# Koukyosyumei/MyZKP

Hardware: AMD Instinct MI355X
Metric: G1 MSM pairs/sec + NTT elems/sec at 2^20 and 2^24; bit-exact vs CPU (higher is better)
Workload: dtype u32x9 (29-bit limbs, 254-bit Montgomery); 1 GPU; KZG commit = BN254 G1 Pippenger MSM of 2^20 (scalar, point) pairs per GPU against a device-resident SRS (commit_kzg, kzg.rs:57-59); 17-bit signed windows (library default at this size), 15 window tables built once at upload; N GPUs = one MSM of N*2^20 pairs (BASELINE configs[2]/[3]); pairs_per_gpu=1048576, seed=332211571536, window_bits=17

## Files before the change

myzkp_amd/csrc/mzk_api.hip:

```cpp
#include <stdarg.h>
#include <stdlib.h>
#include <atomic>
#include "mzk_common.h"
#include "mzk_gl.h"

namespace mzk {

static thread_local char g_err[512] = "";
void set_error(const char* fmt, ...) {
  va_list ap;
  va_start(ap, fmt);
  vsnprintf(g_err, sizeof g_err, fmt, ap);
  va_end(ap);
}
void clear_error() { g_err[0] = 0; }
int hip_fail(hipError_t e, const char* what, const char* file, int line) {
  set_error("HIP error %d (%s) in %s at %s:%d", (int)e, hipGetErrorString(e), what, file, line);
  return MZK_E_HIP;
}

static std::atomic<uint64_t> g_owner{0};
static thread_local int t_depth = 0;
static thread_local char t_marker;
static uint64_t g_call_epoch = 1;
static size_t g_ws_budget = 0;
EntryGuard::EntryGuard() : ok(true), nested(false) {
  if (t_depth > 0) { t_depth++; nested = true; return; }
  uint64_t expected = 0;
  if (!g_owner.compare_exchange_strong(expected, (uint64_t)(uintptr_t)&t_marker, std::memory_order_acquire)) {
    ok = false;
    set_error("another host thread is inside the library: calls must come from one thread at a time (MZK_E_BUSY)");
    return;
  }
  t_depth = 1;
  g_call_epoch++;
}
EntryGuard::~EntryGuard() {
  if (!ok) return;
  if (--t_depth == 0) g_owner.store(0, std::memory_order_release);
}

static Context g_ctxs[MZK_MAX_CTX];
static int g_nctx = 0, g_cur = 0;
static int g_last_ordinal = 0;
static signed char g_peer[MZK_MAX_CTX][MZK_MAX_CTX];
int ctx_peer_enabled(int a, int b) { return (a >= 0 && b >= 0 && a < g_nctx && b < g_nctx) ? g_peer[a][b] : 0; }
static uint64_t g_gen_counter = 1;
Context& ctx() { return g_ctxs[g_cur]; }
int ctx_count() { return g_nctx; }
static std::atomic<int> g_ctx0_current_on{-1};
static void publish_ctx0() {
  g_ctx0_current_on.store((g_nctx > 0 && g_cur == 0 && g_ctxs[0].ready) ? g_ctxs[0].device : -1, std::memory_order_release);
}
int ctx_select(int index) {
  if (index < 0 || index >= g_nctx || !g_ctxs[index].ready) { set_error("context %d does not exist (%d initialised)", index, g_nctx); return MZK_E_ARG; }
  MZK_HIP(hipSetDevice(g_ctxs[index].device));
  g_cur = index;
  publish_ctx0();
  return MZK_OK;
}
CtxScope::CtxScope(int index) : prev_ctx(g_cur), prev_dev(-1), ok(false) {
  if (hipGetDevice(&prev_dev) != hipSuccess) prev_dev = -1;
  ok = ctx_select(index) == MZK_OK;
}
CtxScope::~CtxScope() {
  g_cur = prev_ctx;
  publish_ctx0();
  if (prev_dev >= 0) (void)hipSetDevice(prev_dev);
}

size_t ws_bytes_held() {
  size_t t = poly_bytes_held();
  for (const auto& b : ctx().ws) t += b.cap;
  return t;
}
size_t ws_trim_idle() {
  Context& c = ctx();
  const size_t poly_idle = poly_trim_idle();
  size_t idle = 0;
  for (const auto& b : c.ws) if (b.p && b.epoch != g_call_epoch) idle += b.cap;
  if (!idle) return poly_idle;
  (void)hipDeviceSynchronize();
  bool table_slot_freed = false;
  for (int k = 0; k < WS_COUNT; k++) {
    WsBuf& b = c.ws[k];
    if (b.p && b.epoch != g_call_epoch) {
      (void)hipFree(b.p);
      b.p = nullptr; b.cap = 0;
      table_slot_freed = table_slot_freed || k == WS_FB_TABLE16 || k == WS_FB_TABLE8 || k == WS_NTT_PRE || k == WS_NTT_PRE_M128;
    }
  }
  if (table_slot_freed) c.ws_gen = ++g_gen_counter;
  return idle + poly_idle;
}
int dev_alloc(void** out, size_t bytes, const char* what) {
  *out = nullptr;
  hipError_t e = hipMalloc(out, bytes);
  if (e == hipErrorOutOfMemory || e == hipErrorMemoryAllocation) {
    (void)hipGetLastError();
    if (ws_trim_idle()) e = hipMalloc(out, bytes);
  }
  if (e == hipSuccess) return MZK_OK;
  (void)hipGetLastError();
  *out = nullptr;
  if (e == hipErrorOutOfMemory || e == hipErrorMemoryAllocation) {
    set_error("%s: the device has no %zu bytes left (idle workspace already released)", what, bytes);
    return MZK_E_NOMEM;
  }
  return hip_fail(e, what, __FILE__, __LINE__);
}
int ws_get(WsSlot slot, size_t bytes, void** out) {
  WsBuf& b = ctx().ws[slot];
  b.epoch = g_call_epoch;
  if (bytes > b.cap) {
    if (b.p) {
      MZK_HIP(hipDeviceSynchronize());
      MZK_HIP(hipFree(b.p));
      b.p = nullptr; b.cap = 0;
    }
    size_t cap = bytes < 4096 ? 4096 : bytes;
    if (g_ws_budget && ws_bytes_held() + cap > g_ws_budget) (void)ws_trim_idle();
    MZK_TRY(dev_alloc(&b.p, cap, "workspace"));
    b.cap = cap;
  }
  *out = b.p;
  return MZK_OK;
}
uint64_t ws_generation() { return ctx().ws_gen; }
int d2h_sync(void* host, const void* dev, size_t bytes, hipStream_t s) {
  if (bytes == 0 || bytes > SMALL_D2H_MAX) {
    if (bytes) MZK_HIP(hipMemcpyAsync(host, dev, bytes, hipMemcpyDeviceToHost, s));
    MZK_HIP(hipStreamSynchronize(s));
    return MZK_OK;
  }
  Context& c = ctx();
  if (!c.bounce) MZK_HIP(hipHostMalloc(&c.bounce, SMALL_D2H_MAX, hipHostMallocPortable));
  MZK_HIP(hipMemcpyAsync(c.bounce, dev, bytes, hipMemcpyDeviceToHost, s));
  MZK_HIP(hipStreamSynchronize(s));
  memcpy(host, c.bounce, bytes);
  return MZK_OK;
}
void ws_release_all() {
  Context& c = ctx();
  c.ws_gen = ++g_gen_counter;
  for (auto& b : c.ws) {
    if (b.p) (void)hipFree(b.p);
    b.p = nullptr; b.cap = 0;
  }
}
WsGuard::WsGuard(hipStream_t s_) : s(s_) {
  Context& c = ctx();
  if (!c.ready) return;
  if (c.ws_used && c.ws_last != s) {
    if (!c.ws_event && hipEventCreateWithFlags(&c.ws_event, hipEventDisableTiming) != hipSuccess) c.ws_event = nullptr;
    if (c.ws_event && hipEventRecord(c.ws_event, c.ws_last) == hipSuccess) (void)hipStreamWaitEvent(s, c.ws_event, 0);
    else { (void)hipGetLastError(); (void)hipDeviceSynchronize(); }
  }
}
WsGuard::~WsGuard() {
  Context& c = ctx();
  if (!c.ready) return;
  c.ws_last = s;
  c.ws_used = true;
}

static bool g_prof_on = false;
static uint32_t g_prof_mask = 0xffffffffu;
struct ProfPair { hipEvent_t a, b; int phase; };
static std::vector<ProfPair> g_prof_pending;
static std::vector<hipEvent_t> g_prof_pool;
static hipEvent_t g_prof_open[MZK_PH_COUNT];
static double g_prof_ms[MZK_PH_COUNT];
static uint64_t g_prof_cnt[MZK_PH_COUNT];
static hipEvent_t prof_event() {
  if (!g_prof_pool.empty()) { hipEvent_t e = g_prof_pool.back(); g_prof_pool.pop_back(); return e; }
  hipEvent_t e = nullptr;
  (void)hipEventCreate(&e);
  return e;
}
void prof_begin(hipStream_t s, int phase) {
  if (!g_prof_on || !((g_prof_mask >> phase) & 1u) || ctx().index != 0) return;
  hipEvent_t e = prof_event();
  (void)hipEventRecord(e, s);
  g_prof_open[phase] = e;
}
void prof_end(hipStream_t s, int phase) {
  if (!g_prof_on || !g_prof_open[phase] || ctx().index != 0) return;
  hipEvent_t e = prof_event();
  (void)hipEventRecord(e, s);
  g_prof_pending.push_back({g_prof_open[phase], e, phase});
  g_prof_open[phase] = nullptr;
}
static void prof_drain() {
  (void)hipDeviceSynchronize();
  for (auto& pr : g_prof_pending) {
    float ms = 0.f;
    if (hipEventElapsedTime(&ms, pr.a, pr.b) == hipSuccess) { g_prof_ms[pr.phase] += ms; g_prof_cnt[pr.phase]++; }
    g_prof_pool.push_back(pr.a);
    g_prof_pool.push_back(pr.b);
  }
  g_prof_pending.clear();
}

int ensure_init() {
  if (g_nctx > 0 && ctx().ready) {
    int cur = -1;
    if (hipGetDevice(&cur) != hipSuccess || cur != ctx().device) MZK_HIP(hipSetDevice(ctx().device));
    return MZK_OK;
  }
  return mzk_init(g_last_ordinal);
}

static const HostField HF_FR = {4, {0x43e1f593f0000001ULL, 0x2833e84879b97091ULL, 0xb85045b68181585dULL, 0x30644e72e131a029ULL}, 29 * FrParams::L};
static const HostField HF_FQ = {4, {0x3c208c16d87cfd47ULL, 0x97816a916871ca8dULL, 0xb85045b68181585dULL, 0x30644e72e131a029ULL}, 29 * FqParams::L};
static const HostField HF_M128 = {2, {1ULL, 407ULL << 55, 0, 0}, 29 * M128Params::L};
const HostField* host_field(int fid) {
  switch (fid) {
    case MZK_FIELD_FR: return &HF_FR;
    case MZK_FIELD_M128: return &HF_M128;
    case MZK_FIELD_FQ: return &HF_FQ;
    default: return nullptr;
  }
}
int field_check(int fid, const char* who, bool fq_too) {
  if (fid == MZK_FIELD_FR || fid == MZK_FIELD_M128 || (fq_too && fid == MZK_FIELD_FQ)) return MZK_OK;
  set_error("%s: bad field id %d", who, fid);
  return MZK_E_ARG;
}
int field_check_ntt(int fid, const char* who) {
  if (fid == MZK_FIELD_FR || fid == MZK_FIELD_M128) return MZK_OK;
  set_error("%s: field id %d has no NTT on this path", who, fid);
  return MZK_E_ARG;
}
static int h_cmp(const uint64_t* a, const uint64_t* b, int n) {
  for (int i = n - 1; i >= 0; i--) if (a[i] != b[i]) return a[i] > b[i] ? 1 : -1;
  return 0;
}
bool h_is_canonical(const HostField* f, const uint64_t* a) { return h_cmp(a, f->p, f->nl) < 0; }
bool h_is_one(const HostField* f, const uint64_t* a) {
  if (a[0] != 1) return false;
  for (int i = 1; i < f->nl; i++) if (a[i]) return false;
  return true;
}
static void h_addmod(const HostField* f, uint64_t* r, const uint64_t* a, const uint64_t* b) {
  uint64_t t[4] = {0, 0, 0, 0};
  unsigned __int128 c = 0;
  for (int i = 0; i < f->nl; i++) { c += (unsigned __int128)a[i] + b[i]; t[i] = (uint64_t)c; c >>= 64; }
  if (c || h_cmp(t, f->p, f->nl) >= 0) {
    unsigned __int128 br = 0;
    for (int i = 0; i < f->nl; i++) {
      unsigned __int128 d = (unsigned __int128)t[i] - f->p[i] - (uint64_t)br;
      t[i] = (uint64_t)d; br = (d >> 64) & 1;
    }
  }
  for (int i = 0; i < f->nl; i++) r[i] = t[i];
}
static void h_mulmod_slow(const HostField* f, uint64_t* r, const uint64_t* a, const uint64_t* b) {
  uint64_t acc[4] = {0, 0, 0, 0}, aa[4] = {0, 0, 0, 0}, bb[4] = {0, 0, 0, 0};
  for (int i = 0; i < f->nl; i++) { aa[i] = a[i]; bb[i] = b[i]; }
  for (int bit = 64 * f->nl - 1; bit >= 0; bit--) {
    h_addmod(f, acc, acc, acc);
    if ((bb[bit / 64] >> (bit % 64)) & 1) h_addmod(f, acc, acc, aa);
  }
  for (int i = 0; i < f->nl; i++) r[i] = acc[i];
}
struct HostMont { bool ready; uint64_t n0; uint64_t r2[4]; };
static HostMont g_hmont[3];
static const HostMont* host_mont(const HostField* f) {
  HostMont* m = &g_hmont[f == &HF_FR ? 0 : (f == &HF_FQ ? 1 : 2)];
  if (!m->ready) {
    uint64_t inv = f->p[0];
    for (int i = 0; i < 6; i++) inv *= 2 - f->p[0] * inv;
    m->n0 = (uint64_t)0 - inv;
    uint64_t x[4] = {1, 0, 0, 0};
    for (int i = 0; i < 128 * f->nl; i++) h_addmod(f, x, x, x);
    for (int i = 0; i < 4; i++) m->r2[i] = x[i];
    m->ready = true;
  }
  return m;
}
static void h_montmul(const HostField* f, const HostMont* m, uint64_t* r, const uint64_t* a, const uint64_t* b) {
  const int n = f->nl;
  uint64_t t[6] = {0, 0, 0, 0, 0, 0};
  for (int i = 0; i < n; i++) {
    unsigned __int128 c = 0;
    for (int j = 0; j < n; j++) { c += (unsigned __int128)a[j] * b[i] + t[j]; t[j] = (uint64_t)c; c >>= 64; }
    c += t[n]; t[n] = (uint64_t)c; t[n + 1] = (uint64_t)(c >> 64);
    const uint64_t q = t[0] * m->n0;
    c = (unsigned __int128)q * f->p[0] + t[0];
    c >>= 64;
    for (int j = 1; j < n; j++) { c += (unsigned __int128)q * f->p[j] + t[j]; t[j - 1] = (uint64_t)c; c >>= 64; }
    c += t[n]; t[n - 1] = (uint64_t)c;
    t[n] = t[n + 1] + (uint64_t)(c >> 64);
  }
  if (t[n] || h_cmp(t, f->p, n) >= 0) {
    unsigned __int128 br = 0;
    for (int i = 0; i < n; i++) { unsigned __int128 d = (unsigned __int128)t[i] - f->p[i] - (uint64_t)br; t[i] = (uint64_t)d; br = (d >> 64) & 1; }
  }
  for (int i = 0; i < n; i++) r[i] = t[i];
}
void h_mulmod(const HostField* f, uint64_t* r, const uint64_t* a, const uint64_t* b) {
  const HostMont* m = host_mont(f);
  uint64_t t[4] = {0, 0, 0, 0};
  h_montmul(f, m, t, a, b);
  h_montmul(f, m, r, t, m->r2);
}
void h_powmod_u64(const HostField* f, uint64_t* r, const uint64_t* a, uint64_t e) {
  uint64_t res[4] = {1, 0, 0, 0}, base[4] = {0, 0, 0, 0};
  for (int i = 0; i < f->nl; i++) base[i] = a[i];
  while (e) {
    if (e & 1) h_mulmod(f, res, res, base);
    h_mulmod(f, base, base, base);
    e >>= 1;
  }
  for (int i = 0; i < f->nl; i++) r[i] = res[i];
}
void h_invmod(const HostField* f, uint64_t* r, const uint64_t* a) {
  uint64_t e[4] = {0, 0, 0, 0}, res[4] = {1, 0, 0, 0}, base[4] = {0, 0, 0, 0};
  for (int i = 0; i < f->nl; i++) { e[i] = f->p[i]; base[i] = a[i]; }
  {
    uint64_t borrow = 2;
    for (int i = 0; i < f->nl && borrow; i++) {
      const uint64_t old = e[i];
      e[i] = old - borrow;
      borrow = (old < borrow) ? 1 : 0;
    }
  }
  for (int bit = 0; bit < 64 * f->nl; bit++) {
    if ((e[bit / 64] >> (bit % 64)) & 1) h_mulmod(f, res, res, base);
    h_mulmod(f, base, base, base);
  }
  for (int i = 0; i < f->nl; i++) r[i] = res[i];
}
void h_ninv_pow2(const HostField* f, unsigned k, uint64_t* out) {
  uint64_t q[4] = {0, 0, 0, 0};
  for (int i = 0; i < f->nl; i++) q[i] = f->p[i];
  q[0] -= 1;
  for (unsigned s = 0; s < k; s++) {
    for (int i = 0; i < f->nl; i++) q[i] = (q[i] >> 1) | ((i + 1 < f->nl) ? (q[i + 1] << 63) : 0);
  }
  unsigned __int128 br = 0;
  for (int i = 0; i < f->nl; i++) {
    unsigned __int128 d = (unsigned __int128)f->p[i] - q[i] - (uint64_t)br;
    out[i] = (uint64_t)d; br = (d >> 64) & 1;
  }
}
void h_rmod(const HostField* f, uint64_t* out) {
  const uint64_t two[4] = {2, 0, 0, 0};
  h_powmod_u64(f, out, two, (uint64_t)f->mont_bits);
}

}

using namespace mzk;

extern "C" {

int mzk_abi_version(void) { return 2; }
const char* mzk_last_error(void) { return g_err; }

static int check_device(int device_ordinal, int* num_cu) {
  int count = 0;
  hipError_t e = hipGetDeviceCount(&count);
  if (e != hipSuccess || count <= 0) {
    set_error("no HIP device visible (hipGetDeviceCount: %s); this library has no CPU fallback",
              e == hipSuccess ? "0 devices" : hipGetErrorString(e));
    return MZK_E_NOGPU;
  }
  if (device_ordinal < 0 || device_ordinal >= count) { set_error("mzk_init: device %d out of range (%d visible)", device_ordinal, count); return MZK_E_ARG; }
  hipDeviceProp_t prop;
  MZK_HIP(hipGetDeviceProperties(&prop, device_ordinal));
  if (strncmp(prop.gcnArchName, "gfx950", 6) != 0) {
    set_error("device %d is %s; this library is built for gfx950 (MI355X) only", device_ordinal, prop.gcnArchName);
    return MZK_E_NOGPU;
  }
  *num_cu = prop.multiProcessorCount;
  return MZK_OK;
}

int mzk_init_devices(const int* device_ordinals, int n_devices) {
  mzk::EntryGuard entry;
  if (!entry.ok) return MZK_E_BUSY;
  if (!device_ordinals || n_devices < 1 || n_devices > MZK_MAX_CTX) { set_error("mzk_init_devices: need 1..%d device ordinals", MZK_MAX_CTX); return MZK_E_ARG; }
  bool same = g_nctx == n_devices;
  for (int i = 0; same && i < n_devices; i++) same = g_ctxs[i].ready && g_ctxs[i].device == device_ordinals[i];
  if (same) return ctx_select(0);
  int ncu[MZK_MAX_CTX];
  for (int i = 0; i < n_devices; i++) MZK_TRY(check_device(device_ordinals[i], &ncu[i]));
  if (g_nctx) mzk_shutdown();
  for (int i = 0; i < n_devices; i++) {
    Context& c = g_ctxs[i];
    c = Context();
    c.index = i;
    c.device = device_ordinals[i];
    c.num_cu = ncu[i];
    c.ws_gen = ++g_gen_counter;
    MZK_HIP(hipSetDevice(c.device));
    int dup = 0;
    for (int j = 0; j < i; j++) dup += g_ctxs[j].device == c.device;
    int prio_least = 0, prio_greatest = 0;
    (void)hipDeviceGetStreamPriorityRange(&prio_least, &prio_greatest);
    int prio = prio_least - dup;
    if (prio < prio_greatest) prio = prio_greatest;
    if (dup == 0) MZK_HIP(hipStreamCreateWithFlags(&c.stream, hipStreamNonBlocking));
    else MZK_HIP(hipStreamCreateWithPriority(&c.stream, hipStreamNonBlocking, prio));
    c.ready = true;
    g_nctx = i + 1;
  }
  g_last_ordinal = device_ordinals[0];
  for (int a = 0; a < n_devices; a++)
    for (int b = 0; b < n_devices; b++) {
      g_peer[a][b] = 1;
      const int da = g_ctxs[a].device, db = g_ctxs[b].device;
      if (da == db) continue;
      int can = 0;
      if (hipDeviceCanAccessPeer(&can, da, db) != hipSuccess) { (void)hipGetLastError(); can = 0; }
      if (can) {
        MZK_HIP(hipSetDevice(da));
        hipError_t e = hipDeviceEnablePeerAccess(db, 0);
        if (e == hipErrorPeerAccessAlreadyEnabled) (void)hipGetLastError();
        else if (e != hipSuccess) { (void)hipGetLastError(); can = 0; }
      }
      g_peer[a][b] = (signed char)can;
    }
  return ctx_select(0);
}
int mzk_init(int device_ordinal) {
  if (g_ctx0_current_on.load(std::memory_order_acquire) == device_ordinal) {
    int dev = -1;
    if (hipGetDevice(&dev) == hipSuccess && (dev == device_ordinal || hipSetDevice(device_ordinal) == hipSuccess)) return MZK_OK;
    (void)hipGetLastError();
  }
  mzk::EntryGuard entry;
  if (!entry.ok) return MZK_E_BUSY;
  if (g_nctx > 0 && g_ctxs[0].ready && g_ctxs[0].device == device_ordinal) return entry.nested ? MZK_OK : ctx_select(0);
  return mzk_init_devices(&device_ordinal, 1);
}
int mzk_ctx_count(void) { return g_nctx; }
int mzk_ctx_select(int index) {
  mzk::EntryGuard entry;
  if (!entry.ok) return MZK_E_BUSY;
  return ctx_select(index);
}
int mzk_ctx_peer_enabled(int a, int b) { return ctx_peer_enabled(a, b); }
int mzk_ctx_device(int index) { return (index >= 0 && index < g_nctx) ? g_ctxs[index].device : -1; }
void* mzk_ctx_stream(int index) { return (index >= 0 && index < g_nctx) ? (void*)g_ctxs[index].stream : nullptr; }

// ... 1141 lines not shown
```

myzkp_amd/csrc/mzk_common.h:

```cpp
#pragma once
#include <hip/hip_runtime.h>
#include <stdint.h>
#include <stddef.h>
#include <stdio.h>
#include <string.h>
#include <functional>
#include <string>
#include <vector>
#include "../../include/mzk.h"
#include "mzk_field.h"
#include "mzk_msm_plan.h"

namespace mzk {

#ifdef MZK_TUNING
#include <stdlib.h>
static inline int tune_int(const char* name, int dflt) { const char* v = getenv(name); return v ? atoi(v) : dflt; } static inline const char* tune_str(const char* name) { return getenv(name); }
#else
static inline constexpr int tune_int(const char*, int dflt) { return dflt; }
static inline constexpr const char* tune_str(const char*) { return nullptr; }
#endif

void set_error(const char* fmt, ...);
void clear_error();
size_t table_budget_bytes();
int hip_fail(hipError_t e, const char* what, const char* file, int line);
#define MZK_HIP(x)                                                        \
  do {                                                                    \
    hipError_t _e = (x);                                                  \
    if (_e != hipSuccess) return mzk::hip_fail(_e, #x, __FILE__, __LINE__); \
  } while (0)
#define MZK_TRY(x)        \
  do {                    \
    int _rc = (x);        \
    if (_rc != MZK_OK) return _rc; \
  } while (0)

constexpr int MZK_MAX_CTX = 16;
struct WsBuf { void* p = nullptr; size_t cap = 0; uint64_t epoch = 0; };
enum WsSlot { WS_NTT_TMP = 0, WS_NTT_IO_A, WS_NTT_IO_B, WS_MSM_POINTS, WS_MSM_SCALARS, WS_MSM_COUNTS, WS_MSM_OFFSETS,
              WS_MSM_CURSOR, WS_MSM_ENTRIES, WS_MSM_BUCKETS, WS_MSM_RED_A, WS_MSM_RED_B, WS_MSM_SCAN, WS_MSM_OUT, WS_MSM_SLOTS, WS_MSM_WGHIST, WS_BATCHINV, WS_XYZZ_TMP, WS_MERKLE_NODES, WS_FB_TABLE16, WS_FB_TABLE8, WS_NTT_PRE, WS_NTT_PRE_M128,
              WS_MISC_A, WS_MISC_B, WS_MISC_C, WS_MISC_D, WS_MISC_E, WS_MISC_F, WS_COUNT };
enum AttrFlag { ATTR_FINE_SCATTER4 = 0, ATTR_FINE_SCATTER8, ATTR_DIGITS_LDS, ATTR_SMALL_MSM, ATTR_NTT_LARGE_FR, ATTR_NTT_LARGE_M128, ATTR_NTT_LARGE_M128_2WG, ATTR_MANY_SORT1, ATTR_TAIL_ROW, ATTR_COARSE_STAGED4, ATTR_COARSE_STAGED8, ATTR_COUNT };
struct Context {
  bool ready = false;
  int index = 0;
  int device = -1;
  int num_cu = 256;
  hipStream_t stream = nullptr;
  WsBuf ws[WS_COUNT];
  uint64_t ws_gen = 1;
  hipEvent_t ws_event = nullptr;
  hipEvent_t fork_event = nullptr, join_event = nullptr;
  hipStream_t ws_last = nullptr;
  bool ws_used = false;
  bool attr_done[ATTR_COUNT] = {};
  hipStream_t xstream[MZK_MAX_CTX] = {};
  hipEvent_t xdone[MZK_MAX_CTX] = {};
  hipEvent_t xready = nullptr;
  void* bounce = nullptr;
};
constexpr size_t SMALL_D2H_MAX = 4096;
int d2h_sync(void* host, const void* dev, size_t bytes, hipStream_t s);
int ctx_peer_enabled(int a, int b);
struct EntryGuard {
  bool ok;
  bool nested;
  EntryGuard();
  ~EntryGuard();
};
#define MZK_ENTER()                        \
  mzk::EntryGuard _mzk_entry;              \
  if (!_mzk_entry.ok) return MZK_E_BUSY;   \
  MZK_TRY(mzk::ensure_init())
Context& ctx();
int ctx_count();
int ctx_select(int index);
int ensure_init();
struct CtxScope {
  int prev_ctx, prev_dev; bool ok;
  explicit CtxScope(int index);
  ~CtxScope();
};

int ws_get(WsSlot slot, size_t bytes, void** out);
void ws_release_all();
size_t ws_trim_idle();
size_t ws_bytes_held();
int dev_alloc(void** out, size_t bytes, const char* what);
size_t poly_bytes_held();
size_t poly_trim_idle();
uint64_t ws_generation();
struct WsGuard {
  hipStream_t s;
  explicit WsGuard(hipStream_t s_);
  ~WsGuard();
};

void prof_begin(hipStream_t s, int phase);
void prof_end(hipStream_t s, int phase);
struct ProfScope {
  hipStream_t s; int ph;
  ProfScope(hipStream_t s_, int ph_) : s(s_), ph(ph_) { prof_begin(s, ph); }
  ~ProfScope() { prof_end(s, ph); }
};

struct HostField {
  int nl;
  uint64_t p[4];
  int mont_bits;
};
const HostField* host_field(int fid);
bool h_is_canonical(const HostField* f, const uint64_t* a);
void h_mulmod(const HostField* f, uint64_t* r, const uint64_t* a, const uint64_t* b);
void h_powmod_u64(const HostField* f, uint64_t* r, const uint64_t* a, uint64_t e);
void h_invmod(const HostField* f, uint64_t* r, const uint64_t* a);
void h_ninv_pow2(const HostField* f, unsigned log2n, uint64_t* out);
bool h_is_one(const HostField* f, const uint64_t* a);
void h_rmod(const HostField* f, uint64_t* out);

static inline bool field_is_gl(int fid) { return fid == MZK_FIELD_M64 || fid == MZK_FIELD_M64X3; }
static inline int field_gl_comps(int fid) { return fid == MZK_FIELD_M64X3 ? 3 : 1; }
static inline int field_words(int fid) { return field_is_gl(fid) ? 2 * field_gl_comps(fid) : (fid == MZK_FIELD_M128 ? 4 : 8); }
static inline int field_limbs64(int fid) { return field_is_gl(fid) ? field_gl_comps(fid) : (fid == MZK_FIELD_M128 ? 2 : 4); }
static inline size_t field_bytes(int fid) { return 8 * (size_t)field_limbs64(fid); }
static inline unsigned field_max_log(int fid) { return fid == MZK_FIELD_FR ? 28 : 32; }

int field_check(int fid, const char* who, bool fq_too = false);
int field_check_ntt(int fid, const char* who);
template <class P_> struct FieldTag { typedef P_ P; };
template <class F> static inline int with_field(int fid, F&& f) {
  if (fid == MZK_FIELD_M128) return f(FieldTag<M128Params>());
  if (fid == MZK_FIELD_FR) return f(FieldTag<FrParams>());
  return field_check(fid, "with_field");
}
template <int NC_> struct GlTag { static constexpr int NC = NC_; };
template <class F> static inline int with_gl(int fid, F&& f) {
  if (fid == MZK_FIELD_M64) return f(GlTag<1>());
  if (fid == MZK_FIELD_M64X3) return f(GlTag<3>());
  return field_check(fid, "with_gl");
}
static inline int field_check_gl(int fid, const char* who) { return field_is_gl(fid) ? MZK_OK : field_check(fid, who); }
template <class F> static inline int with_field3(int fid, F&& f) {
  if (fid == MZK_FIELD_FR) return f(FieldTag<FrParams>());
  if (fid == MZK_FIELD_FQ) return f(FieldTag<FqParams>());
  if (fid == MZK_FIELD_M128) return f(FieldTag<M128Params>());
  return field_check(fid, "with_field", true);
}
#define MZK_FIELD_LAUNCH(fid, kernel, ...) \
  mzk::with_field(fid, [&](auto tag_) { typedef typename decltype(tag_)::P P; hipLaunchKernelGGL((kernel), __VA_ARGS__); return MZK_OK; })

int ntt_dev_impl(int fid, const uint64_t* root_host, const void* d_in, void* d_out, size_t n, int inverse,
                 const uint64_t* extra_scale_host, hipStream_t s);
int ntt_batch_dev_impl(int fid, const uint64_t* root_host, const void* d_in, void* d_out, size_t n, size_t batch, int inverse, hipStream_t s);
int coset_lde_dev_impl(int fid, const void* d_coef, size_t n_coef, const uint64_t* offset_host,
                       const uint64_t* generator_host, void* d_out, size_t order, hipStream_t s, size_t batch = 1);
int ntt_columns_dev_impl(int fid, const uint64_t* root_host, const void* d_in, void* d_out, size_t n_points, size_t cols, int inverse, hipStream_t s);
int transpose_elems_dev_impl(int fid, const void* d_in, void* d_out, size_t rows, size_t cols, hipStream_t s);
int poly_scale_dev_impl(int fid, const void* d_in, size_t n, const uint64_t* ratio_host, const uint64_t* lead_host, void* d_out, hipStream_t s);
int coset_divide_dev_impl(int fid, const void* d_lhs, size_t tl, const void* d_rhs, size_t tr, const uint64_t* offset_host,
                          const uint64_t* root_host, size_t order, void* d_out, hipStream_t s);
int rows_trimmed_len_dev(int fid, void* d_rows, size_t stride, const size_t* lens, size_t count, size_t clear_to, const void* d_extra, size_t extra_len,
                         WsSlot slot, size_t* out_lens, hipStream_t s);
struct CdRow { size_t row, tl; };
int coset_divide_rows_dev_impl(int fid, const void* d_lhs, size_t lhs_stride, const CdRow* rows, size_t nrows, const void* d_rhs, size_t tr,
                               const uint64_t* offset_host, const uint64_t* root_host, size_t order, void* d_out, size_t out_stride, hipStream_t s);
int pointwise_div_dev(int fid, const void* d_a, const void* d_b, void* d_out, size_t n, hipStream_t s);
int pointwise_div_shared_dev(int fid, const void* d_a, size_t a_stride, const void* d_b, void* d_out, size_t out_stride, size_t n, size_t regs, hipStream_t s);
int pointwise_mul_shared_dev(int fid, const void* d_a, size_t a_stride, const void* d_b, void* d_out, size_t out_stride, size_t n, size_t regs, hipStream_t s);
int pointwise_mul_dev(int fid, const void* d_a, const void* d_b, void* d_out, size_t n, hipStream_t s);
void ntt_release_plans();
int gl_param_check(int fid, const uint64_t* x, const char* who, const char* what, bool base_only);
int gl_ntt_dev_impl(int fid, const uint64_t* root_host, const void* d_in, void* d_out, size_t n, size_t batch, int inverse, hipStream_t s);
int gl_coset_lde_dev_impl(int fid, const void* d_coef, size_t n_coef, const uint64_t* offset_host, const uint64_t* generator_host, void* d_out,
                          size_t order, hipStream_t s, size_t batch);
int gl_fri_fold_dev(int fid, const void* d_cw, size_t n, const uint64_t* alpha, uint64_t half, uint64_t oinv, uint64_t winv, void* d_out, hipStream_t s);
void gl_release_plans();
void kzg_release_cache();
void poly_release_pool();
int fri_fold_dev_impl(int fid, const void* d_cw, size_t n, const uint64_t* alpha, const uint64_t* offset, const uint64_t* omega,
                      void* d_out, hipStream_t s);
struct FriFoldConsts { uint64_t half[4], oinv[4], winv[4], rmod[4]; };
int fri_fold_consts(int fid, const uint64_t* offset, const uint64_t* omega, FriFoldConsts* fc);
void fri_fold_consts_square(int fid, FriFoldConsts* fc);
int fri_fold_dev_consts(int fid, const void* d_cw, size_t n, const uint64_t* alpha, const FriFoldConsts& fc, void* d_out, hipStream_t s);
int fri_fold_dev_alpha(int fid, const void* d_cw, size_t n, const uint64_t* d_alpha, const FriFoldConsts& fc, void* d_out, hipStream_t s);
int kzg_batch_open_dev(const void* d_coef, size_t n, const uint64_t* us_host, size_t k, const void* d_points, int point_kind,
                       size_t table_stride, void* d_ys, void* d_w_xy, hipStream_t s);

static inline int msm_srs_window_bits(size_t n) {
  return n <= 1024 ? 8 : (n <= ((size_t)1 << 14) ? 10 : (n < ((size_t)1 << 19) ? 16 : (n < ((size_t)1 << 22) ? 17 : 20)));
}
static inline bool msm_srs_default_tables(size_t n) { return n > 0; }
struct MsmChunkCtx {
  int k, K;
  size_t i0;
  size_t n_total;
  size_t n_alloc;
};
struct MsmChunk { const void* d_scalars; size_t i0, n; hipEvent_t ready; };
int msm_chunked_impl(const MsmChunk* chunks, int K, const void* d_points, size_t n_total, int point_kind, size_t table_stride, void* d_out,
                     bool out_partial_xyzz, hipStream_t s, const std::function<int(int)>* before_chunk = nullptr);
bool msm_chunkable(size_t n_total, int point_kind, size_t table_stride);
int msm_dev_impl(const void* d_scalars, const void* d_points, size_t n, int point_kind, size_t table_stride, void* d_out,
                 bool out_partial_xyzz, hipStream_t s, const std::function<int()>* points_ready = nullptr, const MsmChunkCtx* cc = nullptr);

bool msm_many_supported(int window_bits);
int msm_generic_window_bits(size_t n);
int msm_many_dev_impl(const void* d_scalars, size_t n, size_t stride_elems, size_t count, const void* d_tables, int c, size_t table_stride, void* d_out,
                      hipStream_t s);
constexpr size_t MSM_DIRECT_MAX_N = (size_t)1 << 14;
size_t msm_direct_bytes(size_t n, int c);
int msm_build_direct(const void* d_points_mont, size_t n, int c, void* d_direct, hipStream_t s);
int msm_direct_many_dev_impl(const void* d_scalars, size_t n, size_t stride_elems, size_t count, const void* d_direct, int c, size_t table_stride, void* d_out,
                             hipStream_t s);

int xyzz_batch_to_affine(const void* d_xyzz, size_t count, void* d_out, bool out_mont, hipStream_t s);
int msm_build_tables(const void* d_points_mont, size_t n, void* d_tables, int window_bits, hipStream_t s);
int msm_fold_partials_impl(const void* d_partials, int count, void* d_out_xy, hipStream_t s);
int msm_prepare_points(const void* d_points_plain, size_t n, void* d_points_mont, void* d_phi, hipStream_t s);
int msm_phi_points(const void* d_points_mont, size_t n, void* d_phi, hipStream_t s);
int synth_field_impl(int fid, uint64_t seed, size_t n, void* d_out, hipStream_t s);
int synth_g1_impl(uint64_t seed, size_t n, void* d_out, hipStream_t s);
int selftest_inv_wave_impl(uint64_t seed, size_t n, uint64_t* mismatches_host, hipStream_t s);
int selftest_row_ec_impl(uint64_t seed, size_t n, int dbl_reps, uint64_t* mismatches_host, hipStream_t s);
int selftest_field_asm_impl(int fid, uint64_t seed, size_t n, uint64_t* mismatches_host, hipStream_t s);
int selftest_copy_impl(const void* d_src, void* d_dst, size_t bytes, hipStream_t s);
int selftest_field_probe_arity(int fid, int op, int form, int* limbs);
int selftest_field_probe_impl(int fid, int op, int form, size_t n, const uint32_t* in_host, uint32_t* out_host, hipStream_t s);
int selftest_g1_probe_check(int op, int form, int* a_words, int* b_words);
int selftest_g1_probe_impl(int op, int form, size_t n, const uint32_t* a_host, const uint32_t* b_host, const uint8_t* neg_host, uint32_t* out_host,
                           hipStream_t s);
int kzg_setup_g1_dev(const uint64_t* alpha_host, const uint64_t* g1_host, size_t first, size_t count, void* d_powers_xy, hipStream_t s);
int kzg_open_dev(const void* d_coef, size_t n, const uint64_t* u_host, const void* d_points, int point_kind, size_t table_stride,
                 void* d_y, void* d_w_xy, void* d_q, hipStream_t s);
struct SdJob { const void* src; size_t len; const uint64_t* u; const uint64_t* end; void* y; void* q; };
int synth_div_dev(const SdJob* jobs, const size_t* rounds, int nrounds, hipStream_t s);
int synth_div_field_dev(int fid, const SdJob* jobs, const size_t* rounds, int nrounds, hipStream_t s);
int poly_div_roots_check(int fid, const void* polys, size_t stride, const size_t* lens, size_t count, const uint64_t* roots, const size_t* root_offsets,
                         const void* out, const size_t* out_lens);
int poly_div_roots_dev_impl(int fid, const void* d_polys, size_t stride, const size_t* lens, size_t count, const uint64_t* roots, const size_t* root_offsets,
                            void* d_out, size_t* out_lens, hipStream_t s);

}

struct mzk_srs {
  void* d_points_mont;
  size_t n;
  bool has_tables;
  int window_bits;
  int ctx_index;
  int sets = 1;
  void* d_direct = nullptr;
  int direct_bits = 0;
  size_t direct_bytes = 0;
  mutable void* d_tables_wide = nullptr;
  mutable int wide_bits = 0;
  mutable size_t wide_bytes = 0;
  int kind() const { return has_tables ? (mzk::MSM_PTS_TABLES | (window_bits << 8) | (sets << 16)) : (int)mzk::MSM_PTS_MONT; }
  size_t table_rows() const { return has_tables ? (size_t)mzk::msm_table_rows(window_bits, sets) : 2; }
};

namespace mzk {
bool srs_many_capable(const mzk_srs* srs);
int msm_many_srs(const mzk_srs* srs, const void* d_scalars, size_t n, size_t stride_elems, size_t count, void* d_out, hipStream_t s,
                 size_t shift = 0);
bool kzg_open_many_supported(const mzk_srs* srs, size_t n);
int kzg_open_many_dev(const mzk_srs* srs, const void* d_coefs, size_t n, size_t count, const uint64_t* us_host, void* d_ys, void* d_ws_xy, hipStream_t s);
}
```

myzkp_amd/csrc/mzk_msm.hip:

```cpp
#include <stdlib.h>
#include <type_traits>
#include "mzk_common.h"
#include "mzk_ec.h"
#include "mzk_coop.h"
#include "mzk_row.h"
#include "mzk_glv.h"
#include "mzk_affine_wave.h"

namespace mzk {

static const MsmKnobs& msm_knobs() {
  static const MsmKnobs k = [] {
    const MsmKnobs d;
    return MsmKnobs{tune_int("MZK_GLV_C", d.glv_c), tune_int("MZK_SMALL_SCAN", d.small_scan), tune_int("MZK_SCAN_MAX_LOG", d.scan_max_log),
                    tune_int("MZK_ACC_SEG", d.acc_seg), tune_int("MZK_COARSE_LOG_20", d.coarse_log_20),
                    tune_int("MZK_COARSE_LOG_17", d.coarse_log_17), tune_int("MZK_PER_FINE", d.per_fine), tune_int("MZK_SORT_SCAN_FREE", d.sort_scan_free),
                    tune_int("MZK_COMBINE_WIDE_MIN_LOG", d.combine_wide_min_log)};
  }();
  return k;
}

int msm_generic_window_bits(size_t n) { return choose_shape_glv(n ? n : 1, msm_knobs().glv_c).c; }

__device__ __forceinline__ void load_words8(const u32* __restrict__ g, u32* w) {
  const uint4* p4 = reinterpret_cast<const uint4*>(g);
  uint4 a = p4[0], b = p4[1];
  w[0] = a.x; w[1] = a.y; w[2] = a.z; w[3] = a.w; w[4] = b.x; w[5] = b.y; w[6] = b.z; w[7] = b.w;
}
__device__ __forceinline__ void store_words8(u32* __restrict__ g, const u32* w) {
  uint4* p4 = reinterpret_cast<uint4*>(g);
  p4[0] = make_uint4(w[0], w[1], w[2], w[3]);
  p4[1] = make_uint4(w[4], w[5], w[6], w[7]);
}
__device__ __forceinline__ Xyzz xyzz_gload(const u32* __restrict__ g, size_t idx) {
  u32 w[32];
#pragma unroll
  for (int q = 0; q < 4; q++) load_words8(g + idx * 32 + 8 * q, w + 8 * q);
  return xyzz_load(w);
}
__device__ __forceinline__ void xyzz_gstore(u32* __restrict__ g, size_t idx, const Xyzz& p) {
  u32 w[32];
  xyzz_store(p, w);
#pragma unroll
  for (int q = 0; q < 4; q++) store_words8(g + idx * 32 + 8 * q, w + 8 * q);
}

static_assert(SLOT_WORDS == 4 * FqParams::L, "a slot is the four raw coordinates");
__device__ __forceinline__ void xyzz_gstore_raw(u32* __restrict__ g, size_t idx, const Xyzz& p) {
  u32 w[SLOT_WORDS];
  const bool inf = xyzz_is_inf(p);
#pragma unroll
  for (int i = 0; i < FqParams::L; i++) {
    w[i] = inf ? 0u : p.X.l[i]; w[9 + i] = inf ? 0u : p.Y.l[i]; w[18 + i] = inf ? 0u : p.ZZ.l[i]; w[27 + i] = inf ? 0u : p.ZZZ.l[i];
  }
  uint4* p4 = reinterpret_cast<uint4*>(g + idx * SLOT_WORDS);
#pragma unroll
  for (int q = 0; q < SLOT_WORDS / 4; q++) p4[q] = make_uint4(w[4 * q], w[4 * q + 1], w[4 * q + 2], w[4 * q + 3]);
}
__device__ __forceinline__ Xyzz xyzz_gload_raw(const u32* __restrict__ g, size_t idx) {
  u32 w[SLOT_WORDS];
  const uint4* p4 = reinterpret_cast<const uint4*>(g + idx * SLOT_WORDS);
#pragma unroll
  for (int q = 0; q < SLOT_WORDS / 4; q++) { const uint4 v = p4[q]; w[4 * q] = v.x; w[4 * q + 1] = v.y; w[4 * q + 2] = v.z; w[4 * q + 3] = v.w; }
  Xyzz p;
#pragma unroll
  for (int i = 0; i < FqParams::L; i++) { p.X.l[i] = w[i]; p.Y.l[i] = w[9 + i]; p.ZZ.l[i] = w[18 + i]; p.ZZZ.l[i] = w[27 + i]; }
  return p;
}
__device__ __forceinline__ Xyzz xyzz_gload_raw_quad(const u32* __restrict__ g, size_t idx, int lane) {
  Fq mine;
  const u32* src = g + idx * SLOT_WORDS + 9 * lane;
#pragma unroll
  for (int i = 0; i < FqParams::L; i++) mine.l[i] = src[i];
  Xyzz p;
  p.X = quad_bcast<0>(mine);
  p.Y = quad_bcast<1>(mine);
  p.ZZ = quad_bcast<2>(mine);
  p.ZZZ = quad_bcast<3>(mine);
  return p;
}

__global__ void k_prepare_points(const u32* __restrict__ in, u32* __restrict__ out, size_t n, u32* __restrict__ phi_out) {
  const size_t i = (size_t)blockIdx.x * blockDim.x + threadIdx.x;
  if (i >= n) return;
  u32 w[16];
  load_words8(in + i * 16, w);
  load_words8(in + i * 16 + 8, w + 8);
  Affine a;
  const bool inf = affine_words_is_inf(w);
  if (!inf) {
    a = affine_load_plain(w);
    affine_store_mont(a, w);
  }
  store_words8(out + i * 16, w);
  store_words8(out + i * 16 + 8, w + 8);
  if (phi_out) {
    if (!inf) {
      Fq beta;
#pragma unroll
      for (int k = 0; k < FqParams::L; k++) beta.l[k] = GlvParams::BETA_MONT[k];
      a.x = fe_reduce<FqParams>(fe_mul<FqParams>(a.x, beta));
      affine_store_mont(a, w);
    }
    store_words8(phi_out + i * 16, w);
    store_words8(phi_out + i * 16 + 8, w + 8);
  }
}
__global__ void k_phi_points(const u32* __restrict__ in_mont, size_t n, u32* __restrict__ phi_out) {
  const size_t i = (size_t)blockIdx.x * blockDim.x + threadIdx.x;
  if (i >= n) return;
  u32 w[16];
  load_words8(in_mont + i * 16, w);
  load_words8(in_mont + i * 16 + 8, w + 8);
  if (!affine_words_is_inf(w)) {
    Affine a = affine_load_mont(w);
    Fq beta;
#pragma unroll
    for (int k = 0; k < FqParams::L; k++) beta.l[k] = GlvParams::BETA_MONT[k];
    a.x = fe_reduce<FqParams>(fe_mul<FqParams>(a.x, beta));
    affine_store_mont(a, w);
  }
  store_words8(phi_out + i * 16, w);
  store_words8(phi_out + i * 16 + 8, w + 8);
}

__global__ void k_points_to_plain(const u32* __restrict__ in_mont, size_t n, u32* __restrict__ out) {
  const size_t i = (size_t)blockIdx.x * blockDim.x + threadIdx.x;
  if (i >= n) return;
  u32 w[16];
  load_words8(in_mont + i * 16, w);
  load_words8(in_mont + i * 16 + 8, w + 8);
  if (!affine_words_is_inf(w)) affine_store_plain(affine_load_mont(w), w);
  store_words8(out + i * 16, w);
  store_words8(out + i * 16 + 8, w + 8);
}

__device__ __forceinline__ void load_scalar_canonical(const u32* __restrict__ scalars, size_t i, u32* w) {
  load_words8(scalars + i * 8, w);
  if (w[7] >= 0x30644e72u) {
    Fe<FrParams> x = fe_reduce<FrParams>(fe_unpack<FrParams>(w));
    fe_pack<FrParams>(x, w);
  }
}
__device__ __forceinline__ u32 raw_window(const u32* w, int win, int c) {
  const int bit = win * c;
  if (bit >= 256) return 0;
  const int k = bit >> 5, s = bit & 31;
  u64 v = w[k];
  if (k + 1 < 8) v |= (u64)w[k + 1] << 32;
  return (u32)(v >> s) & ((1u << c) - 1u);
}
__device__ __forceinline__ int slots_per_scalar(const DigitLayout& L) { return L.glv ? 2 * L.nwin : L.nwin; }
template <class Emit>
__device__ __forceinline__ void walk_digits(const u32* w, const DigitLayout& L, size_t i, Emit emit) {
  const int c = L.c;
  const u32 half = 1u << (c - 1);
  if (!L.glv) {
    u32 carry = 0;
    for (int win = 0; win < L.nwin; win++) {
      u32 raw = raw_window(w, win, c) + carry;
      u32 neg = 0, mag = raw;
      carry = 0;
      if (raw > half) { mag = (1u << c) - raw; neg = 1; carry = 1; }
      if (mag != 0) {
        const u32 key = (L.merged ? ((u32)(win % L.sets) << (c - 1)) : ((u32)win << (c - 1))) + (mag - 1);
        const u32 payload = (L.merged ? (u32)((size_t)(win / L.sets) * L.table_stride + i) : (u32)i) | (neg << 31);
        emit(win, key, payload);
      }
    }
    return;
  }
  u32 m[2][8], sg[2];
#pragma unroll
  for (int h = 0; h < 2; h++)
#pragma unroll
    for (int j = 4; j < 8; j++) m[h][j] = 0;
  glv_split(w, m[0], &sg[0], m[1], &sg[1]);
#pragma unroll
  for (int h = 0; h < 2; h++) {
    u32 carry = 0;
    for (int win = 0; win < L.nwin; win++) {
      u32 raw = raw_window(m[h], win, c) + carry;
      u32 neg = 0, mag = raw;
      carry = 0;
      if (raw > half) { mag = (1u << c) - raw; neg = 1; carry = 1; }
      if (mag != 0) {
        const u32 key = ((u32)win << (c - 1)) + (mag - 1);
        const u32 payload = (u32)(i + (h ? L.phi_offset : 0)) | ((neg ^ sg[h]) << 31);
        emit(h * L.nwin + win, key, payload);
      }
    }
  }
}

constexpr u32 digit_bias_word(int C, int k) {
  const int nwin = 254 / C + 1;
  const unsigned long long hm1 = (1ull << (C - 1)) - 1;
  unsigned long long acc = 0;
  for (int w = 0; w < nwin; w++) {
    const int sh = w * C - 32 * k;
    if (sh >= 0 && sh < 32) acc |= (hm1 << sh) & 0xffffffffull;
    else if (sh < 0 && sh > -32) acc |= hm1 >> (-sh);
  }
  return (u32)acc;
}
template <int C, class Emit>
__device__ __forceinline__ void walk_digits_merged(const u32* w, size_t table_stride, size_t i, Emit emit) {
  constexpr int NWIN = 254 / C + 1;
  constexpr u32 HALF = 1u << (C - 1), MASKC = (1u << C) - 1u;
  u32 t[9];
  u64 cy = 0;
#pragma unroll
  for (int k = 0; k < 8; k++) { cy += (u64)w[k] + digit_bias_word(C, k); t[k] = (u32)cy; cy >>= 32; }
  t[8] = (u32)cy + digit_bias_word(C, 8);
#pragma unroll
  for (int win = 0; win < NWIN; win++) {
    const int bit = win * C, k = bit >> 5, sft = bit & 31;
    const u64 pair = (u64)t[k] | ((k + 1 < 9) ? ((u64)t[k + 1] << 32) : 0ull);
    const u32 v = (u32)(pair >> sft) & MASKC;
    if (v == HALF - 1u) continue;
    const bool neg = v < HALF - 1u;
    const u32 mag = neg ? (HALF - 1u) - v : v - (HALF - 1u);
    emit(win, mag - 1u, (u32)((size_t)win * table_stride + i) | ((u32)neg << 31));
  }
}

template <int NT>
__device__ __forceinline__ u32 block_excl_scan(u32 v, u32* sc, u32* total) {
  constexpr int NW = NT / 64;
  static_assert(NT % 64 == 0 && NW <= 64, "whole waves, at most 64 of them");
  const int lane = threadIdx.x & 63, wave = threadIdx.x >> 6;
  u32 incl = v;
#pragma unroll
  for (int off = 1; off < 64; off <<= 1) { const u32 t = (u32)__shfl_up((int)incl, off, 64); if (lane >= off) incl += t; }
  if (lane == 63) sc[wave] = incl;
  __syncthreads();
  if (wave == 0) {
    u32 t = (lane < NW) ? sc[lane] : 0u;
#pragma unroll
    for (int off = 1; off < NW; off <<= 1) { const u32 u = (u32)__shfl_up((int)t, off, 64); if (lane >= off) t += u; }
    if (lane < NW) sc[lane] = t;
  }
  __syncthreads();
  if (total) *total = sc[NW - 1];
  return (wave ? sc[wave - 1] : 0u) + incl - v;
}

__device__ __forceinline__ u32 counter_inc_agg(u32* __restrict__ ctr, u32 key) {
  const u32 k0 = (u32)__builtin_amdgcn_readfirstlane((int)key);
  const u64 same = __builtin_amdgcn_ballot_w64(key == k0);
  if (__builtin_popcountll(same) >= 16) {
    u32 r;
    if (key == k0) {
      const u32 lane_id = __builtin_amdgcn_mbcnt_hi(~0u, __builtin_amdgcn_mbcnt_lo(~0u, 0u));
      const u32 rank = (u32)__builtin_popcountll(same & (((u64)1 << lane_id) - 1));
      u32 base = 0;
      if (rank == 0) base = atomicAdd(&ctr[k0], (u32)__builtin_popcountll(same));
      base = (u32)__builtin_amdgcn_readlane((int)base, __builtin_ctzll(same));
      r = base + rank;
    } else {
      r = atomicAdd(&ctr[key], 1u);
    }
    return r;
  }
  return atomicAdd(&ctr[key], 1u);
}
constexpr u32 NO_RANK = 0xffffffffu;

__global__ __launch_bounds__(256) void k_digits_count(const u32* __restrict__ scalars, size_t n, DigitLayout L, u32* __restrict__ counts,
                                                       u32* __restrict__ ranks) {
  const size_t i = (size_t)blockIdx.x * blockDim.x + threadIdx.x;
  if (i >= n) return;
  u32 w[8];
  load_scalar_canonical(scalars, i, w);
  walk_digits(w, L, i, [&](int slot, u32 key, u32) { ranks[(size_t)slot * n + i] = counter_inc_agg(counts, key); });
}
__global__ __launch_bounds__(256) void k_digits_scatter(const u32* __restrict__ scalars, size_t n, DigitLayout L, const u32* __restrict__ offsets,
                                                         const u32* __restrict__ ranks, u32* __restrict__ entries) {
  const size_t i = (size_t)blockIdx.x * blockDim.x + threadIdx.x;
  if (i >= n) return;
  u32 w[8];
  load_scalar_canonical(scalars, i, w);
  walk_digits(w, L, i, [&](int slot, u32 key, u32 payload) { entries[offsets[key] + ranks[(size_t)slot * n + i]] = payload; });
}

constexpr int LDS_SORT_THREADS = 1024;
__global__ __launch_bounds__(LDS_SORT_THREADS) void k_digits_count_lds(const u32* __restrict__ scalars, size_t n, size_t per_wg, DigitLayout L,
                                                                      u32* __restrict__ wg_hist, u32* __restrict__ ranks) {
  extern __shared__ u32 hist[];
  const int NBK = 1 << (L.c - 1);
  for (int b = threadIdx.x; b < NBK; b += LDS_SORT_THREADS) hist[b] = 0;
  __syncthreads();
  const size_t lo = (size_t)blockIdx.x * per_wg;
  const size_t hi = (lo + per_wg < n) ? lo + per_wg : n;
  const int c = L.c;
  const u32 half = 1u << (c - 1);
  for (size_t i = lo + threadIdx.x; i < hi; i += LDS_SORT_THREADS) {
    u32 w[8];
    load_scalar_canonical(scalars, i, w);
    u32 carry = 0;
    for (int win = 0; win < L.nwin; win++) {
      u32 raw = raw_window(w, win, c) + carry;
      u32 mag = raw;
      carry = 0;
      if (raw > half) { mag = (1u << c) - raw; carry = 1; }
      u32 rank = NO_RANK;
      if (mag != 0) rank = atomicAdd(&hist[mag - 1], 1u);
      ranks[(size_t)win * n + i] = rank;
    }
  }
  __syncthreads();
  u32* row = wg_hist + (size_t)blockIdx.x * NBK;
  for (int b = threadIdx.x; b < NBK; b += LDS_SORT_THREADS) row[b] = hist[b];
}
__global__ __launch_bounds__(256) void k_wg_hist_prefix(u32* __restrict__ wg_hist, int nwg, int nbk, u32* __restrict__ counts) {
  const int b = blockIdx.x * blockDim.x + threadIdx.x;
  if (b >= nbk) return;
  u32 run = 0;
  for (int g = 0; g < nwg; g++) {
    const u32 v = wg_hist[(size_t)g * nbk + b];
    wg_hist[(size_t)g * nbk + b] = run;
    run += v;
  }
  counts[b] = run;
}
__global__ __launch_bounds__(LDS_SORT_THREADS) void k_digits_scatter_lds(const u32* __restrict__ scalars, size_t n, size_t per_wg, DigitLayout L,
                                                                        const u32* __restrict__ offsets, const u32* __restrict__ wg_hist,
                                                                        const u32* __restrict__ ranks, u32* __restrict__ entries) {
  extern __shared__ u32 base[];
  const int NBK = 1 << (L.c - 1);
  const u32* row = wg_hist + (size_t)blockIdx.x * NBK;
  for (int b = threadIdx.x; b < NBK; b += LDS_SORT_THREADS) base[b] = offsets[b] + row[b];
  __syncthreads();
  const size_t lo = (size_t)blockIdx.x * per_wg;
  const size_t hi = (lo + per_wg < n) ? lo + per_wg : n;
  const int c = L.c;
  const u32 half = 1u << (c - 1);
  for (size_t i = lo + threadIdx.x; i < hi; i += LDS_SORT_THREADS) {
    u32 w[8];
    load_scalar_canonical(scalars, i, w);
    u32 carry = 0;
    for (int win = 0; win < L.nwin; win++) {
      u32 raw = raw_window(w, win, c) + carry;
      u32 neg = 0, mag = raw;
      carry = 0;
      if (raw > half) { mag = (1u << c) - raw; neg = 1; carry = 1; }
      if (mag != 0) {
        const u32 rank = ranks[(size_t)win * n + i];
        const u32 ref = (u32)((size_t)win * L.table_stride + i);
        entries[base[mag - 1] + rank] = ref | (neg << 31);
      }
    }
  }
}

constexpr int SORT2_THREADS = 1024;
template <int C, int CL = COARSE_LOG>
__global__ __launch_bounds__(SORT2_THREADS) void k_coarse_count(const u32* __restrict__ scalars, size_t n, DigitLayout L, int key_shift,
                                                                 u32* __restrict__ binhist, int nwg, u32* __restrict__ bin_tot, u32* __restrict__ zero_ptr,
                                                                 size_t zero_words) {
  constexpr int BINS = 1 << CL;
  static_assert(BINS <= SORT2_THREADS, "one lane per bin");
  __shared__ u32 hist[BINS];
  if (threadIdx.x < BINS) hist[threadIdx.x] = 0;
  if (zero_ptr) {
    const size_t per = (zero_words + gridDim.x - 1) / gridDim.x;
    const size_t z0 = (size_t)blockIdx.x * per, z1 = (z0 + per < zero_words) ? z0 + per : zero_words;
    for (size_t z = z0 + threadIdx.x; z < z1; z += SORT2_THREADS) zero_ptr[z] = 0;
  }
  __syncthreads();
  const size_t lo = (size_t)blockIdx.x * COARSE_PER_WG;
  const size_t hi = (lo + COARSE_PER_WG < n) ? lo + COARSE_PER_WG : n;
  u32 w[COARSE_PER_WG / SORT2_THREADS][8];
#pragma unroll
  for (int k = 0; k < COARSE_PER_WG / SORT2_THREADS; k++) {
    const size_t i = lo + threadIdx.x + (size_t)k * SORT2_THREADS;
    if (i < hi) load_scalar_canonical(scalars, i, w[k]);
  }
#pragma unroll
  for (int k = 0; k < COARSE_PER_WG / SORT2_THREADS; k++) {
    const size_t i = lo + threadIdx.x + (size_t)k * SORT2_THREADS;
    if (i < hi) {
      auto emit = [&](int, u32 key, u32) { counter_inc_agg(hist, key >> key_shift); };
      if constexpr (C != 0) walk_digits_merged<C>(w[k], L.table_stride, i, emit);
      else walk_digits(w[k], L, i, emit);
    }
  }
  __syncthreads();
  if (threadIdx.x < BINS) {
    const u32 v = hist[threadIdx.x];
    binhist[(size_t)threadIdx.x * nwg + blockIdx.x] = v;
    if (bin_tot && v) atomicAdd(&bin_tot[threadIdx.x], v);
  }
}
template <int BINS>
__device__ __forceinline__ void bin_starts(const u32* __restrict__ bin_tot, u32* start, u32* __restrict__ start_out) {
  constexpr int PER = BINS / 64;
  static_assert(BINS % 64 == 0, "whole lanes");
  const int tid = threadIdx.x;
  if (tid < 64) {
    u32 c[PER], sum = 0;
#pragma unroll
    for (int q = 0; q < PER; q++) { c[q] = bin_tot[PER * tid + q]; sum += c[q]; }
    u32 incl = sum;
#pragma unroll
    for (int d = 1; d < 64; d <<= 1) {
      const u32 up = (u32)__shfl_up((int)incl, d, 64);
      if (tid >= d) incl += up;
    }
    u32 run = incl - sum;
#pragma unroll
    for (int q = 0; q < PER; q++) { start[PER * tid + q] = run; run += c[q]; }
    if (tid == 63) start[BINS] = incl;
  }
  __syncthreads();
  if (start_out && blockIdx.x == 0) for (int b = tid; b <= BINS; b += blockDim.x) start_out[b] = start[b];
}
struct Rec8 {
  typedef uint2 T;
  static __device__ __forceinline__ T make(u32 payload, u32 fine, int) { return make_uint2(payload, fine); }
  static __device__ __forceinline__ u32 fine(const T& r, u32, int) { return r.y; }
  static __device__ __forceinline__ u32 payload(const T& r, int) { return r.x; }
};
struct Rec4 {
  typedef u32 T;
  static __device__ __forceinline__ T make(u32 payload, u32 fine, int fb) { return ((payload & 0x7fffffffu) << (fb + 1)) | (fine << 1) | (payload >> 31); }
  static __device__ __forceinline__ u32 fine(const T& r, u32 fmask, int) { return (r >> 1) & fmask; }
  static __device__ __forceinline__ u32 payload(const T& r, int fb) { return (r >> (fb + 1)) | ((r & 1u) << 31); }
};
template <class REC, int C, int CL = COARSE_LOG>
__global__ __launch_bounds__(SORT2_THREADS) void k_coarse_scatter(const u32* __restrict__ scalars, size_t n, DigitLayout L, int key_shift,
                                                                   u32 fine_mask, int fb, const u32* __restrict__ binbase, int nwg,
                                                                   typename REC::T* __restrict__ tmp, const u32* __restrict__ bin_tot,
                                                                   u32* __restrict__ bin_cur, u32* __restrict__ bin_start_out) {
  constexpr int COARSE_BINS = 1 << CL;
  static_assert(COARSE_BINS <= SORT2_THREADS, "one lane per bin");
  __shared__ u32 cursor[COARSE_BINS];
  __shared__ u32 bscan[COARSE_BINS + 1];
  if (bin_tot) {
    bin_starts<COARSE_BINS>(bin_tot, bscan, bin_start_out);
    if (threadIdx.x < COARSE_BINS) {
      const u32 mine = binbase[(size_t)threadIdx.x * nwg + blockIdx.x];
      cursor[threadIdx.x] = bscan[threadIdx.x] + (mine ? atomicAdd(&bin_cur[threadIdx.x], mine) : 0u);
    }
  } else if (threadIdx.x < COARSE_BINS) {
    cursor[threadIdx.x] = binbase[(size_t)threadIdx.x * nwg + blockIdx.x];
  }
  __syncthreads();
  const size_t lo = (size_t)blockIdx.x * COARSE_PER_WG;
  const size_t hi = (lo + COARSE_PER_WG < n) ? lo + COARSE_PER_WG : n;
  u32 w[COARSE_PER_WG / SORT2_THREADS][8];
#pragma unroll
  for (int k = 0; k < COARSE_PER_WG / SORT2_THREADS; k++) {
    const size_t i = lo + threadIdx.x + (size_t)k * SORT2_THREADS;
    if (i < hi) load_scalar_canonical(scalars, i, w[k]);
  }
#pragma unroll
  for (int k = 0; k < COARSE_PER_WG / SORT2_THREADS; k++) {
    const size_t i = lo + threadIdx.x + (size_t)k * SORT2_THREADS;
    if (i < hi) {
      auto emit = [&](int, u32 key, u32 payload) {
        const u32 pos = counter_inc_agg(cursor, key >> key_shift);
        tmp[pos] = REC::make(payload, key & fine_mask, fb);
      };
      if constexpr (C != 0) walk_digits_merged<C>(w[k], L.table_stride, i, emit);
      else walk_digits(w[k], L, i, emit);
    }
  }
}
constexpr int stage_records(int C, int CL) { return (CL > 8 ? (254 / C + 1) : 16) * SORT2_THREADS; }
constexpr size_t stage_lds_bytes(int C, int CL, size_t rec_bytes) {
  return (size_t)stage_records(C, CL) * (rec_bytes + (CL > 8 ? 2 : 1)) + (size_t)(4 * (1 << CL) + 1) * 4;
}
template <class REC, int C, int CL = COARSE_LOG>
__global__ __launch_bounds__(SORT2_THREADS) void k_coarse_scatter_staged(const u32* __restrict__ scalars, size_t n, size_t table_stride, int key_shift,
                                                                          u32 fine_mask, int fb, const u32* __restrict__ binbase, int nwg,
                                                                          typename REC::T* __restrict__ tmp, const u32* __restrict__ bin_tot,
                                                                          u32* __restrict__ bin_cur, u32* __restrict__ bin_start_out) {
  typedef typename REC::T R;
  constexpr int COARSE_BINS = 1 << CL;
  constexpr int STAGE_RECORDS = stage_records(C, CL);
  constexpr int PER_LANE = COARSE_BINS / 64;
  typedef typename std::conditional<(CL > 8), unsigned short, unsigned char>::type BinTag;
  static_assert(stage_lds_bytes(C, CL, sizeof(R)) <= (size_t)160 * 1024, "staging must fit the LDS");
  extern __shared__ __attribute__((aligned(16))) u32 lds_stage[];
  R* stage = reinterpret_cast<R*>(lds_stage);
  BinTag* stage_bin = reinterpret_cast<BinTag*>(stage + STAGE_RECORDS);
  u32* cursor = reinterpret_cast<u32*>(stage_bin + STAGE_RECORDS);
  u32* hist = cursor + COARSE_BINS;
  u32* loff = hist + COARSE_BINS;
  u32* gpos = loff + COARSE_BINS + 1;
  static_assert(COARSE_BINS % 64 == 0 && COARSE_BINS <= SORT2_THREADS, "one wave scans PER_LANE bins per lane; one lane per bin elsewhere");
  const int tid = threadIdx.x;
  if (bin_tot) bin_starts<COARSE_BINS>(bin_tot, loff, bin_start_out);
  if (tid < COARSE_BINS) cursor[tid] = bin_tot ? loff[tid] : binbase[(size_t)tid * nwg + blockIdx.x];
  const size_t lo = (size_t)blockIdx.x * COARSE_PER_WG;
  const size_t hi = (lo + COARSE_PER_WG < n) ? lo + COARSE_PER_WG : n;
  u32 w[COARSE_PER_WG / SORT2_THREADS][8];
#pragma unroll
  for (int k = 0; k < COARSE_PER_WG / SORT2_THREADS; k++) {
    const size_t i = lo + tid + (size_t)k * SORT2_THREADS;
    if (i < hi) load_scalar_canonical(scalars, i, w[k]);
  }
#pragma unroll 1
  for (int k = 0; k < COARSE_PER_WG / SORT2_THREADS; k++) {
    const size_t i = lo + tid + (size_t)k * SORT2_THREADS;
    if (tid < COARSE_BINS) hist[tid] = 0;
    __syncthreads();
    if (i < hi) walk_digits_merged<C>(w[k], table_stride, i, [&](int, u32 key, u32) { counter_inc_agg(hist, key >> key_shift); });
    __syncthreads();
    if (tid < 64) {
      u32 c[PER_LANE], sum = 0;
#pragma unroll
      for (int q = 0; q < PER_LANE; q++) { c[q] = hist[PER_LANE * tid + q]; sum += c[q]; }
      u32 incl = sum;
#pragma unroll
      for (int d = 1; d < 64; d <<= 1) {
        const u32 up = (u32)__shfl_up((int)incl, d, 64);
        if (tid >= d) incl += up;
      }
      u32 run = incl - sum;
#pragma unroll
      for (int q = 0; q < PER_LANE; q++) { loff[PER_LANE * tid + q] = run; run += c[q]; }
      if (tid == 63) loff[COARSE_BINS] = incl;
    }
    __syncthreads();
    if (tid < COARSE_BINS) {
      const u32 cnt = hist[tid];
      if (bin_tot) {
        gpos[tid] = cursor[tid] + (cnt ? atomicAdd(&bin_cur[tid], cnt) : 0u);
      } else {
        gpos[tid] = cursor[tid];
        cursor[tid] += cnt;
      }
      hist[tid] = loff[tid];
    }
    __syncthreads();
    if (i < hi) walk_digits_merged<C>(w[k], table_stride, i, [&](int, u32 key, u32 payload) {
      const u32 bin = key >> key_shift;
      const u32 pos = counter_inc_agg(hist, bin);
      stage[pos] = REC::make(payload, key & fine_mask, fb);
      stage_bin[pos] = (BinTag)bin;
    });
    __syncthreads();
    const u32 total = loff[COARSE_BINS];
    for (u32 p = tid; p < total; p += SORT2_THREADS) {
      const u32 b = stage_bin[p];
      tmp[gpos[b] + (p - loff[b])] = stage[p];
    }
    __syncthreads();
  }
}
struct FineSlice { int bin, s, Sb; u32 lo, hi, start; bool active; };
__device__ __forceinline__ FineSlice fine_plan(const u32* __restrict__ binbase, int nwg, int bins, int S, u32 cap, u32* sc, u32* res) {
  const int tid = threadIdx.x;
  u32 start = 0, len = 0, Sb = 0;
  if (tid < bins) {
    start = binbase[(size_t)tid * nwg];
    len = binbase[(size_t)(tid + 1) * nwg] - start;
    Sb = (len + cap - 1) / cap;
    if (Sb < (u32)S) Sb = (u32)S;
  }
  if (tid == 0) res[0] = 0xffffffffu;
  const int lane = tid & 63, wave = tid >> 6;
  u32 v = Sb;
#pragma unroll
  for (int off = 1; off < 64; off <<= 1) { const u32 t = __shfl_up(v, off, 64); if (lane >= off) v += t; }
  if (lane == 63) sc[wave] = v;
  __syncthreads();
  if (wave == 0) {
    u32 t = (lane < SORT2_THREADS / 64) ? sc[lane] : 0u;
#pragma unroll
    for (int off = 1; off < SORT2_THREADS / 64; off <<= 1) { const u32 u = __shfl_up(t, off, 64); if (lane >= off) t += u; }
    if (lane < SORT2_THREADS / 64) sc[lane] = t;
  }
  __syncthreads();
  const u32 w = blockIdx.x, incl = v + (wave ? sc[wave - 1] : 0u), excl = incl - Sb;
  if (tid < bins && excl <= w && w < incl) { res[0] = (u32)tid; res[1] = w - excl; res[2] = Sb; res[3] = start; res[4] = len; res[5] = excl; }
  __syncthreads();
  FineSlice r;
  r.active = res[0] != 0xffffffffu;
  r.bin = (int)res[0]; r.s = (int)res[1]; r.Sb = (int)res[2];
  const u64 L = res[4];
  r.start = res[3];
  r.lo = res[3] + (u32)(L * (u64)r.s / (u64)r.Sb);
  r.hi = res[3] + (u32)(L * (u64)(r.s + 1) / (u64)r.Sb);
  return r;
}
constexpr int FINE_UNROLL = 8;
template <class REC>
__global__ __launch_bounds__(SORT2_THREADS) void k_fine_count(const typename REC::T* __restrict__ tmp, const u32* __restrict__ binbase, int nwg, int F,
                                                               int S, int fb, u32* __restrict__ finehist, int bins, u32 cap, u32* __restrict__ bucket_tot) {
  __shared__ u32 hist[FINE_MAX];
  __shared__ u32 sc[SORT2_THREADS];
  const FineSlice p = fine_plan(binbase, nwg, bins, S, cap, sc, hist);
  __syncthreads();
  if (!p.active) {
    for (int f = threadIdx.x; f < F; f += SORT2_THREADS) finehist[(size_t)blockIdx.x * F + f] = 0;
    return;
  }
  for (int f = threadIdx.x; f < F; f += SORT2_THREADS) hist[f] = 0;
  __syncthreads();
  const u32 lo = p.lo, hi = p.hi;
  for (u32 base = lo + threadIdx.x; base < hi; base += FINE_UNROLL * SORT2_THREADS) {
    u32 f[FINE_UNROLL];
#pragma unroll
    for (int k = 0; k < FINE_UNROLL; k++) {
      const u32 e = base + k * SORT2_THREADS;
      f[k] = (e < hi) ? REC::fine(tmp[e], (u32)F - 1u, fb) : 0xffffffffu;
    }
#pragma unroll
    for (int k = 0; k < FINE_UNROLL; k++) if (f[k] != 0xffffffffu) counter_inc_agg(hist, f[k]);
  }
  __syncthreads();
  const size_t hbase = (size_t)F * (blockIdx.x - (u32)p.s);
  for (int f = threadIdx.x; f < F; f += SORT2_THREADS) {
    const u32 v = hist[f];
    finehist[hbase + (size_t)f * p.Sb + p.s] = v;
    if (bucket_tot && v) atomicAdd(&bucket_tot[(size_t)p.bin * F + f], v);
  }
}
template <class REC>
__global__ __launch_bounds__(SORT2_THREADS) void k_fine_scatter_direct(const typename REC::T* __restrict__ tmp, const u32* __restrict__ binbase, int nwg, int F,
                                                                 int S, int fb, const u32* __restrict__ finebase, u32* __restrict__ offsets,
                                                                 u32* __restrict__ entries, size_t nbuckets, int bins, u32 cap) {
  __shared__ u32 cursor[FINE_MAX];
  __shared__ u32 sc[SORT2_THREADS];
  const FineSlice p = fine_plan(binbase, nwg, bins, S, cap, sc, cursor);
  __syncthreads();
  if (blockIdx.x == 0 && threadIdx.x == 0) offsets[nbuckets] = finebase[(size_t)F * gridDim.x];
  if (!p.active) return;
  const size_t hbase = (size_t)F * (blockIdx.x - (u32)p.s);
  for (int f = threadIdx.x; f < F; f += SORT2_THREADS) {
    const u32 base = finebase[hbase + (size_t)f * p.Sb + p.s];
    cursor[f] = base;
    if (p.s == 0) offsets[(size_t)p.bin * F + f] = base;
  }
  __syncthreads();
  const u32 lo = p.lo, hi = p.hi;
  for (u32 base = lo + threadIdx.x; base < hi; base += FINE_UNROLL * SORT2_THREADS) {
    typename REC::T r[FINE_UNROLL];
#pragma unroll
    for (int k = 0; k < FINE_UNROLL; k++) {
      const u32 e = base + k * SORT2_THREADS;
      if (e < hi) r[k] = tmp[e];
    }
#pragma unroll
    for (int k = 0; k < FINE_UNROLL; k++)
      if (base + k * SORT2_THREADS < hi) entries[counter_inc_agg(cursor, REC::fine(r[k], (u32)F - 1u, fb))] = REC::payload(r[k], fb);
  }
}

#ifndef MZK_STAGE_CAP
#define MZK_STAGE_CAP 8192
#endif
constexpr int STAGE_CAP = MZK_STAGE_CAP;
constexpr int STAGE_PER_LANE = STAGE_CAP / SORT2_THREADS;
template <class REC>
__global__ __launch_bounds__(SORT2_THREADS) void k_fine_scatter(const typename REC::T* __restrict__ tmp, const u32* __restrict__ binbase, int nwg, int F,
                                                                 int S, int fb, const u32* __restrict__ finebase, u32* __restrict__ offsets,
                                                                 u32* __restrict__ entries, size_t nbuckets, int bins, u32 cap, const u32* __restrict__ bucket_tot,
                                                                 u32* __restrict__ bucket_cur) {
  extern __shared__ u32 lds_fs[];
  u32* gbase = lds_fs;
  u32* cnt = gbase + F;
  u32* lpre = cnt + F;
  u32* scan = lpre + F;
  u32* spay = scan + SORT2_THREADS;
  unsigned short* skey = reinterpret_cast<unsigned short*>(spay + STAGE_CAP);
  const int tid = threadIdx.x;
  const FineSlice p = fine_plan(binbase, nwg, bins, S, cap, scan, gbase);
  __syncthreads();
  if (blockIdx.x == 0 && tid == 0) offsets[nbuckets] = bucket_tot ? binbase[(size_t)bins * nwg] : finebase[(size_t)F * gridDim.x];
  if (!p.active) return;
  const size_t hbase = (size_t)F * (blockIdx.x - (u32)p.s);
  if (bucket_tot) {
    const int per2 = (F + SORT2_THREADS - 1) / SORT2_THREADS;
    u32 local = 0;
    for (int q = 0; q < per2; q++) { const int f = tid * per2 + q; if (f < F) { const u32 v = bucket_tot[(size_t)p.bin * F + f]; cnt[f] = v; local += v; } }
    u32 run = p.start + block_excl_scan<SORT2_THREADS>(local, scan, nullptr);
    for (int q = 0; q < per2; q++) {
      const int f = tid * per2 + q;
      if (f < F) {
        const u32 v = cnt[f];
        const u32 mine = finebase[hbase + (size_t)f * p.Sb + p.s];
        gbase[f] = run + (mine ? atomicAdd(&bucket_cur[(size_t)p.bin * F + f], mine) : 0u);
        if (p.s == 0) offsets[(size_t)p.bin * F + f] = run;
        run += v;
      }
    }
    __syncthreads();
  } else {
    for (int f = tid; f < F; f += SORT2_THREADS) {
      const u32 base = finebase[hbase + (size_t)f * p.Sb + p.s];
      gbase[f] = base;
      if (p.s == 0) offsets[(size_t)p.bin * F + f] = base;
    }
  }
  const u32 lo = p.lo, hi = p.hi;
  const int per = (F + SORT2_THREADS - 1) / SORT2_THREADS;
  for (u32 chunk = lo; chunk < hi; chunk += STAGE_CAP) {
    const u32 cend = (hi - chunk > (u32)STAGE_CAP) ? chunk + STAGE_CAP : hi;
    for (int f = tid; f < F; f += SORT2_THREADS) cnt[f] = 0;
    __syncthreads();
    typename REC::T r[STAGE_PER_LANE];
    u32 rk[STAGE_PER_LANE];
    const u32 fmask = (u32)F - 1u;
#pragma unroll
    for (int k = 0; k < STAGE_PER_LANE; k++) {
      const u32 e = chunk + tid + k * SORT2_THREADS;
      if (e < cend) r[k] = tmp[e];
    }
#pragma unroll
    for (int k = 0; k < STAGE_PER_LANE; k++) rk[k] = (chunk + tid + k * SORT2_THREADS < cend) ? counter_inc_agg(cnt, REC::fine(r[k], fmask, fb)) : 0u;
    __syncthreads();
    u32 local = 0;
    for (int q = 0; q < per; q++) { const int f = tid * per + q; if (f < F) local += cnt[f]; }
    u32 run = block_excl_scan<SORT2_THREADS>(local, scan, nullptr);
    for (int q = 0; q < per; q++) { const int f = tid * per + q; if (f < F) { lpre[f] = run; run += cnt[f]; } }
    __syncthreads();
#pragma unroll
    for (int k = 0; k < STAGE_PER_LANE; k++) {
      if (chunk + tid + k * SORT2_THREADS < cend) {
        const u32 fk = REC::fine(r[k], fmask, fb);
        const u32 pos = lpre[fk] + rk[k];
        spay[pos] = REC::payload(r[k], fb);
        skey[pos] = (unsigned short)fk;
      }
    }
    __syncthreads();
    const u32 m = cend - chunk;
    for (u32 j = tid; j < m; j += SORT2_THREADS) {
      const u32 f = skey[j];
      entries[gbase[f] + (j - lpre[f])] = spay[j];
    }
    __syncthreads();
    for (int f = tid; f < F; f += SORT2_THREADS) gbase[f] += cnt[f];
    __syncthreads();
  }
}

__global__ __launch_bounds__(256) void k_scan_local(const u32* __restrict__ in, u32* __restrict__ out, u32* __restrict__ block_sums, size_t n) {
  __shared__ u32 sh[256];
  const size_t base = (size_t)blockIdx.x * SCAN_BLOCK + (size_t)threadIdx.x * SCAN_ITEMS;
  u32 v[SCAN_ITEMS], sum = 0;
#pragma unroll
  for (int k = 0; k < SCAN_ITEMS; k++) {
    v[k] = (base + k < n) ? in[base + k] : 0u;
    sum += v[k];
  }
  u32 block_total;
  u32 excl = block_excl_scan<256>(sum, sh, &block_total);
  if (threadIdx.x == 255) block_sums[blockIdx.x] = block_total;
#pragma unroll
  for (int k = 0; k < SCAN_ITEMS; k++) {
    if (base + k < n) out[base + k] = excl;
    excl += v[k];
  }
}
__global__ __launch_bounds__(256) void k_scan_finish(u32* __restrict__ offsets, const u32* __restrict__ block_sums, size_t nblocks, size_t n) {
  __shared__ u32 part[4];
  static_assert(SCAN_BLOCK % 256 == 0, "one block index per workgroup");
  const size_t i = (size_t)blockIdx.x * blockDim.x + threadIdx.x;
  const size_t first = (size_t)blockIdx.x * blockDim.x;
  const bool total_wg = first >= n;
  const size_t blk = total_wg ? nblocks : first / SCAN_BLOCK;
  u32 acc = 0;
  for (size_t j = threadIdx.x; j < blk; j += 256) acc += block_sums[j];
#pragma unroll
  for (int d = 32; d >= 1; d >>= 1) acc += (u32)__shfl_xor((int)acc, d, 64);
  if ((threadIdx.x & 63) == 0) part[threadIdx.x >> 6] = acc;
  __syncthreads();
  const u32 pre = part[0] + part[1] + part[2] + part[3];
  if (total_wg) { if (threadIdx.x == 0) offsets[n] = pre; }
  else if (i < n) offsets[i] = offsets[i] + pre;
}

__global__ __launch_bounds__(256) void k_scan_add(u32* __restrict__ offsets, const u32* __restrict__ prefix, size_t nblocks, size_t n) {
  const size_t i = (size_t)blockIdx.x * blockDim.x + threadIdx.x;
  if (i < n) offsets[i] += prefix[i / SCAN_BLOCK];
  else if (i == n) offsets[n] = prefix[nblocks];
}
static int launch_exclusive_scan(const u32* in, u32* out, size_t n, u32* scratch, hipStream_t s) {
  const size_t sb = (n + SCAN_BLOCK - 1) / SCAN_BLOCK;
  hipLaunchKernelGGL(k_scan_local, dim3((unsigned)sb), dim3(256), 0, s, in, out, scratch, n);
  if (sb <= SCAN_DIRECT_BLOCKS) {
    hipLaunchKernelGGL(k_scan_finish, dim3((unsigned)((n + 255) / 256 + 1)), dim3(256), 0, s, out, (const u32*)scratch, sb, n);
  } else {
    MZK_TRY(launch_exclusive_scan((const u32*)scratch, scratch, sb, scratch + sb + 2, s));
    hipLaunchKernelGGL(k_scan_add, dim3((unsigned)(n / 256 + 1)), dim3(256), 0, s, out, (const u32*)scratch, sb, n);
  }
  MZK_HIP(hipGetLastError());
  return MZK_OK;
}

constexpr u32 SEG_MIN = 8;
__device__ __forceinline__ u32 segment_length(u32 seg_host, u32 t_max, u32 total_entries) {
  if (t_max == 0) return seg_host;
  const u32 v = (total_entries + t_max - 1) / t_max;
  return v < SEG_MIN ? SEG_MIN : v;
}
template <bool SENT = false>
__global__ __launch_bounds__(256, 3) void k_seg_accumulate(const u32* __restrict__ points_mont, const u32* __restrict__ offsets,
                                                         const u32* __restrict__ entries, u32* __restrict__ slots, size_t nbuckets,
                                                         u32 seg_host, u32 t_max) {
  const size_t t = (size_t)blockIdx.x * blockDim.x + threadIdx.x;
  const u32 total_entries = offsets[nbuckets];
  u32 e0, e1;
  if (!seg_span(t, segment_length(seg_host, t_max, total_entries), total_entries, &e0, &e1)) return;
  const auto offset_at = [&](size_t b) __attribute__((always_inline)) { return offsets[b]; };
  Xyzz acc = xyzz_inf();
  u32 w[16];
  Affine pt;
  bool skip = false;
  seg_walk<SENT>(
      e0, e1, seg_first_bucket(offset_at, nbuckets, e0), nbuckets, [&](u32 e) __attribute__((always_inline)) { return entries[e]; }, offset_at,
      [&](u32 ref) __attribute__((always_inline)) {
        const size_t idx = ref & 0x7fffffffu;
        load_words8(points_mont + idx * 16, w);
        load_words8(points_mont + idx * 16 + 8, w + 8);
      },
      [&](u32 ent) __attribute__((always_inline)) {
#pragma unroll
        for (int k = 0; k < 16; k++) asm volatile("" : "+v"(w[k]));
        skip = affine_words_is_inf(w) || (SENT && ent == MANY_SENTINEL);
        pt = affine_load_mont(w);
      },
      [&](size_t b) __attribute__((always_inline)) {
        xyzz_gstore_raw(slots, t + b, acc);
        acc = xyzz_inf();
      },
      [&](u32, u32 ent, size_t) __attribute__((always_inline)) {
        if (!skip) acc = xyzz_madd_signed_with<FeAsm>(acc, pt, (ent >> 31) != 0);
      });
}
constexpr u32 HEAVY_SLOTS_SORT1 = 16;
__device__ __forceinline__ u32 bucket_end(const u32* __restrict__ offsets, const u32* __restrict__ tails, int lg_nb, size_t b) {
  if (tails && (b & (((size_t)1 << lg_nb) - 1)) == (((size_t)1 << lg_nb) - 1)) return tails[b >> lg_nb];
  return offsets[b + 1];
}
__device__ __forceinline__ bool defer_heavy(size_t b, size_t s0, size_t s1, u32 o1, u32* __restrict__ heavy, bool leader, u32 threshold = HEAVY_SLOTS) {
  if (s1 - s0 + 1 <= threshold) return false;
  if (leader) { const u32 i = atomicAdd(&heavy[0], 1u); heavy[HEAVY_HDR + 2 * i] = (u32)b; heavy[HEAVY_HDR + 2 * i + 1] = o1; }
  return true;
}
__global__ __launch_bounds__(128) void k_seg_combine_wide(const u32* __restrict__ slots, const u32* __restrict__ offsets,
                                                           u32* __restrict__ buckets, size_t nbuckets, u32 seg_host, u32* __restrict__ heavy, u32 t_max) {
  const size_t b = (size_t)blockIdx.x * blockDim.x + threadIdx.x;
  if (b >= nbuckets) return;
  const u32 seg = segment_length(seg_host, t_max, offsets[nbuckets]);
  if (b == 0) heavy[1] = seg;
  const u32 o0 = offsets[b], o1 = offsets[b + 1];
  Xyzz acc = xyzz_inf();
  if (o1 > o0) {
    const size_t s0 = (size_t)(o0 / seg) + b, s1 = (size_t)((o1 - 1) / seg) + b;
    if (defer_heavy(b, s0, s1, o1, heavy, true)) return;
    for (size_t sl = s0; sl <= s1; sl++) acc = xyzz_add_with<FeAsm>(acc, xyzz_gload_raw(slots, sl));
  }
  xyzz_gstore(buckets, b, acc);
}
__global__ __launch_bounds__(128) void k_seg_combine(const u32* __restrict__ slots, const u32* __restrict__ offsets, u32* __restrict__ buckets,
                                                      size_t nbuckets, u32 seg_host, u32* __restrict__ heavy, const u32* __restrict__ tails, int lg_nb, u32 t_max) {
  const size_t tid = (size_t)blockIdx.x * blockDim.x + threadIdx.x;
  const size_t b = tid / 4;
  const int lane = (int)(tid & 3);
  if (b >= nbuckets) return;
  const u32 seg = segment_length(seg_host, t_max, offsets[nbuckets]);
  if (tid == 0) heavy[1] = seg;
  const u32 o0 = offsets[b], o1 = bucket_end(offsets, tails, lg_nb, b);
  Xyzz acc = xyzz_inf();
  if (o1 > o0) {
    const size_t s0 = (size_t)(o0 / seg) + b, s1 = (size_t)((o1 - 1) / seg) + b;
    if (defer_heavy(b, s0, s1, o1, heavy, lane == 0, tails ? HEAVY_SLOTS_SORT1 : HEAVY_SLOTS)) return;
    acc = xyzz_gload_raw_quad(slots, s0, lane);
    for (size_t sl = s0 + 1; sl <= s1; sl++) acc = xyzz_add_quad(acc, xyzz_gload_raw_quad(slots, sl, lane), lane);
  }
  xyzz_gstore_quad(buckets, b, acc, lane);
}
constexpr int HEAVY_THREADS = 256;
constexpr int HEAVY_QUADS = HEAVY_THREADS / 4;
__device__ __forceinline__ void heavy_tree(u32* sh, const Xyzz& acc, int quad, int lane) {
  xyzz_gstore_quad(sh, quad, acc, lane);
  __syncthreads();
  for (int off = HEAVY_QUADS / 2; off >= 1; off >>= 1) {
    if (quad < off) {
      const Xyzz x = xyzz_gload_quad(sh, quad, lane), y = xyzz_gload_quad(sh, quad + off, lane);
      xyzz_gstore_quad(sh, quad, xyzz_add_quad(x, y, lane), lane);
    }
    __syncthreads();
  }
}
__global__ __launch_bounds__(HEAVY_THREADS) void k_seg_combine_heavy(const u32* __restrict__ slots, const u32* __restrict__ offsets,
                                                                      u32* __restrict__ buckets, u32* __restrict__ heavy, size_t max_heavy) {
  __shared__ __attribute__((aligned(16))) u32 sh[HEAVY_QUADS * 32];
  __shared__ u32 last_arrival;
  const u32 count = heavy[0];
  if (count == 0) return;
  const u32 seg = heavy[1];
  const int lane = threadIdx.x & 3, quad = threadIdx.x >> 2;
  const u32* list = heavy + HEAVY_HDR;
  if (2 * count > gridDim.x) {
    for (u32 h = blockIdx.x; h < count; h += gridDim.x) {
      const size_t b = list[2 * h];
      const u32 o0 = offsets[b], o1 = list[2 * h + 1];
      const size_t s0 = (size_t)(o0 / seg) + b, s1 = (size_t)((o1 - 1) / seg) + b;
      Xyzz acc = xyzz_inf();
      for (size_t sl = s0 + quad; sl <= s1; sl += HEAVY_QUADS) acc = xyzz_add_quad(acc, xyzz_gload_raw_quad(slots, sl, lane), lane);
      heavy_tree(sh, acc, quad, lane);
      if (quad == 0) xyzz_gstore_quad(buckets, b, xyzz_gload_quad(sh, 0, lane), lane);
      __syncthreads();
    }
    return;
  }
  const u32 G = gridDim.x / count;
  const u32 h = blockIdx.x / G, part = blockIdx.x % G;
  if (h >= count) return;
  u32* scratch = heavy + heavy_list_words(max_heavy);
  const size_t b = list[2 * h];
  const u32 o0 = offsets[b], o1 = list[2 * h + 1];
  const size_t s0 = (size_t)(o0 / seg) + b, s1 = (size_t)((o1 - 1) / seg) + b;
  if (s1 - s0 + 1 <= 16 * HEAVY_QUADS) {
    if (part != 0) return;
    Xyzz acc = xyzz_inf();
    for (size_t sl = s0 + quad; sl <= s1; sl += HEAVY_QUADS) acc = xyzz_add_quad(acc, xyzz_gload_raw_quad(slots, sl, lane), lane);
    heavy_tree(sh, acc, quad, lane);
    if (quad == 0) xyzz_gstore_quad(buckets, b, xyzz_gload_quad(sh, 0, lane), lane);
    return;
  }
  const size_t per = (s1 - s0 + G) / G;
  const size_t lo = s0 + (size_t)part * per;
  size_t hi = lo + per - 1;
  if (hi > s1) hi = s1;
  Xyzz acc = xyzz_inf();
  for (size_t sl = lo + quad; sl <= hi; sl += HEAVY_QUADS) acc = xyzz_add_quad(acc, xyzz_gload_raw_quad(slots, sl, lane), lane);
  heavy_tree(sh, acc, quad, lane);
  if (quad == 0) xyzz_gstore_quad(scratch, (size_t)h * G + part, xyzz_gload_quad(sh, 0, lane), lane);
  __threadfence();
  __syncthreads();
  if (threadIdx.x == 0) last_arrival = (atomicAdd(&heavy[2 + h], 1u) == G - 1) ? 1u : 0u;
  __syncthreads();
  if (!last_arrival) return;
  __threadfence();
  acc = xyzz_inf();
  for (u32 q = quad; q < G; q += HEAVY_QUADS) acc = xyzz_add_quad(acc, xyzz_gload_quad(scratch, (size_t)h * G + q, lane), lane);
  heavy_tree(sh, acc, quad, lane);
  if (quad == 0) xyzz_gstore_quad(buckets, b, xyzz_gload_quad(sh, 0, lane), lane);
}

__device__ __forceinline__ void halve_op(u32* __restrict__ buf, int lgB, int t, size_t id, int lane) {
  const int lgh = lgB - t - 1;
  const size_t a = id >> lgh, j = id & (((size_t)1 << lgh) - 1);
  const size_t base = (a == 0) ? 0 : ((size_t)1 << (lgB - a));
  const size_t idx = base + j;
  const Xyzz x = xyzz_gload_quad(buf, idx, lane), y = xyzz_gload_quad(buf, idx + ((size_t)1 << lgh), lane);
  xyzz_gstore_quad(buf, idx, xyzz_add_quad(x, y, lane), lane);
}
__global__ __launch_bounds__(128) void k_halve_step_wide(u32* __restrict__ buckets, int lgB, int t) {
  const size_t id = (size_t)blockIdx.x * blockDim.x + threadIdx.x;
  const size_t total = (size_t)(t + 1) << (lgB - t - 1);
  if (id >= total) return;
  u32* buf = buckets + ((size_t)blockIdx.y << lgB) * 32;
  const int lgh = lgB - t - 1;
  const size_t a = id >> lgh, j = id & (((size_t)1 << lgh) - 1);
  const size_t idx = ((a == 0) ? 0 : ((size_t)1 << (lgB - a))) + j;
  xyzz_gstore(buf, idx, xyzz_add_with<FeAsm>(xyzz_gload(buf, idx), xyzz_gload(buf, idx + ((size_t)1 << lgh))));
}
__global__ __launch_bounds__(128) void k_halve_step(u32* __restrict__ buckets, int lgB, int t) {
  const size_t tid = (size_t)blockIdx.x * blockDim.x + threadIdx.x;
  const size_t id = tid >> 2;
  const size_t total = (size_t)(t + 1) << (lgB - t - 1);
  if (id >= total) return;
  halve_op(buckets + ((size_t)blockIdx.y << lgB) * 32, lgB, t, id, (int)(tid & 3));
}
constexpr int HMULTI_THREADS = 512;
constexpr int HMULTI_QUADS = HMULTI_THREADS / 4;
constexpr int HMULTI_MAX_S = 8;
__global__ __launch_bounds__(HMULTI_THREADS) void k_halve_multi(u32* __restrict__ buckets, int lgB, int t0, int s) {
  extern __shared__ __attribute__((aligned(16))) u32 lds_hm[];
  const int lgs = lgB - t0 - s;
  const int a = (int)(blockIdx.x >> lgs);
  const size_t j0 = blockIdx.x & (((size_t)1 << lgs) - 1);
  u32* buf = buckets + ((size_t)blockIdx.y << lgB) * 32;
  const size_t base = ((a == 0) ? 0 : ((size_t)1 << (lgB - a))) + j0;
  const int ql = threadIdx.x & 3, quad = threadIdx.x >> 2;
  uint4* l4 = reinterpret_cast<uint4*>(lds_hm);
  uint4* g4 = reinterpret_cast<uint4*>(buf);
  for (int i = threadIdx.x; i < (8 << s); i += HMULTI_THREADS) l4[i] = g4[(base + ((size_t)(i >> 3) << lgs)) * 8 + (i & 7)];
  __syncthreads();
  for (int tl = 0; tl < s; tl++) {
    const int lgh = s - tl - 1;
    const int total = ((a == 0) ? (tl + 1) : 1) << lgh;
    for (int id = quad; id < total; id += HMULTI_QUADS) {
      const int aa = id >> lgh, j = id & ((1 << lgh) - 1);
      const int lo = ((aa == 0) ? 0 : (1 << (s - aa))) + j;
      const Xyzz x = xyzz_gload_quad(lds_hm, (size_t)lo, ql), y = xyzz_gload_quad(lds_hm, (size_t)(lo + (1 << lgh)), ql);
      xyzz_gstore_quad(lds_hm, (size_t)lo, xyzz_add_quad(x, y, ql), ql);
    }
    __syncthreads();
  }
  const int nlive = (a == 0) ? s + 1 : 1;
  for (int i = threadIdx.x; i < 8 * nlive; i += HMULTI_THREADS) {
    const int e = i >> 3, k = (e == 0) ? 0 : (1 << (e - 1));
    g4[(base + ((size_t)k << lgs)) * 8 + (i & 7)] = l4[k * 8 + (i & 7)];
  }
}

constexpr int SMALL_SORT_THREADS = 1024;
__global__ __launch_bounds__(SMALL_SORT_THREADS) void k_small_sort(const u32* __restrict__ scalars, size_t n, DigitLayout L, int NB,
                                                                    u32* __restrict__ offsets, u32* __restrict__ entries) {
  extern __shared__ u32 sh_small[];
  u32* hist = sh_small;
  u32* scan = sh_small + NB;
  const int tid = threadIdx.x;
  for (int b = tid; b < NB; b += SMALL_SORT_THREADS) hist[b] = 0;
  __syncthreads();
  for (size_t i = tid; i < n; i += SMALL_SORT_THREADS) {
    u32 w[8];
    load_scalar_canonical(scalars, i, w);
    walk_digits(w, L, i, [&](int, u32 key, u32) { atomicAdd(&hist[key], 1u); });
  }
  __syncthreads();
  const int per = (NB + SMALL_SORT_THREADS - 1) / SMALL_SORT_THREADS;
  u32 local = 0;
  for (int q = 0; q < per; q++) { const int b = tid * per + q; if (b < NB) local += hist[b]; }
  u32 all_entries;
  u32 run = block_excl_scan<SMALL_SORT_THREADS>(local, scan, &all_entries);
  for (int q = 0; q < per; q++) {
    const int b = tid * per + q;
    if (b < NB) { const u32 c = hist[b]; hist[b] = run; offsets[b] = run; run += c; }
  }
  if (tid == SMALL_SORT_THREADS - 1) offsets[NB] = all_entries;
  __syncthreads();
  for (size_t i = tid; i < n; i += SMALL_SORT_THREADS) {
    u32 w[8];
    load_scalar_canonical(scalars, i, w);
    walk_digits(w, L, i, [&](int, u32 key, u32 payload) { entries[atomicAdd(&hist[key], 1u)] = payload; });
  }
}
template <int T>
__device__ __forceinline__ void small_tree_store(u32* sh, const Xyzz& acc, u32 cnt, size_t b, u32* __restrict__ buckets) {
  const int lane = threadIdx.x;
  if (cnt > T) cnt = T;
  if (cnt <= 1) {
    if (lane == 0) xyzz_gstore(buckets, b, acc);
    return;
  }
  u32 width = 2;
  while (width < cnt) width <<= 1;
  if ((u32)lane < width) xyzz_gstore(sh, lane, acc);
  __syncthreads();
  const int quad = lane >> 2, ql = lane & 3;
  const rowop::Lane ln = rowop::lane_init();
  for (u32 m = width; m > 1; m >>= 1) {
    if (m / 2 <= (u32)(T / 64)) {
      for (u32 i = (u32)(lane >> 6); i < m / 2; i += T / 64) {
        const rowop::Pt x = rowop::load(sh + i * 32, ln), y = rowop::load(sh + (i + m / 2) * 32, ln);
        rowop::store(sh + i * 32, rowop::add(x, y, ln), ln);
      }
    } else {
      for (u32 i = quad; i < m / 2; i += T / 4) {
        const Xyzz x = xyzz_gload_quad(sh, i, ql), y = xyzz_gload_quad(sh, i + m / 2, ql);
        xyzz_gstore_quad(sh, i, xyzz_add_quad(x, y, ql), ql);
      }
    }
    __syncthreads();
  }
  if (lane < 32) buckets[b * 32 + lane] = sh[lane];
}

template <int T>
__global__ __launch_bounds__(T) void k_small_accumulate(const u32* __restrict__ points_mont, const u32* __restrict__ offsets,
                                                         const u32* __restrict__ entries, u32* __restrict__ buckets) {
  __shared__ __attribute__((aligned(16))) u32 sh[T * 32];
  const size_t b = blockIdx.x;
  const int lane = threadIdx.x;
  const u32 o0 = offsets[b], o1 = offsets[b + 1];
  Xyzz acc = xyzz_inf();
  for (u32 e = o0 + lane; e < o1; e += T) {
    const u32 ent = entries[e];
    u32 w[16];
    const size_t idx = ent & 0x7fffffffu;
    load_words8(points_mont + idx * 16, w);
    load_words8(points_mont + idx * 16 + 8, w + 8);
    if (affine_words_is_inf(w)) continue;
    acc = xyzz_madd_signed_with<FeCpp>(acc, affine_load_mont(w), (ent >> 31) != 0);
  }
  small_tree_store<T>(sh, acc, o1 - o0, b, buckets);
}
constexpr int SMALL_LIST_CAP = 4096;
template <int T, int C>
__global__ __launch_bounds__(T) void k_small_accumulate_scan(const u32* __restrict__ scalars, size_t n, size_t table_stride, const u32* __restrict__ points_mont,
                                                              u32* __restrict__ buckets) {
  constexpr int NWIN = 254 / C + 1;
  constexpr u32 HALF = 1u << (C - 1), MASKC = (1u << C) - 1u;
  __shared__ __attribute__((aligned(16))) u32 sh[T * 32];
  __shared__ u32 list[SMALL_LIST_CAP];
  __shared__ u32 count;
  const size_t b = blockIdx.x;
  const int lane = threadIdx.x;
  if (lane == 0) count = 0;
  __syncthreads();
  Xyzz acc = xyzz_inf();
  auto add_entry = [&](u32 ent) {
    u32 w[16];
    const size_t idx = ent & 0x7fffffffu;
    load_words8(points_mont + idx * 16, w);
    load_words8(points_mont + idx * 16 + 8, w + 8);
    if (affine_words_is_inf(w)) return;
    acc = xyzz_madd_signed_with<FeCpp>(acc, affine_load_mont(w), (ent >> 31) != 0);
  };
  const u32 vpos = (u32)b + HALF, vneg = HALF - 2u - (u32)b;
  for (size_t i = lane; i < n; i += T) {
    u32 w[8], t[9];
    load_scalar_canonical(scalars, i, w);
    u64 cy = 0;
#pragma unroll
    for (int k = 0; k < 8; k++) { cy += (u64)w[k] + digit_bias_word(C, k); t[k] = (u32)cy; cy >>= 32; }
    t[8] = (u32)cy + digit_bias_word(C, 8);
    u32 hits = 0;
    u32 negs = 0;
#pragma unroll
    for (int win = 0; win < NWIN; win++) {
      const int bit = win * C, k = bit >> 5, sft = bit & 31;
      const u64 pair = (u64)t[k] | ((k + 1 < 9) ? ((u64)t[k + 1] << 32) : 0ull);
      const u32 v = (u32)(pair >> sft) & MASKC;
      hits |= (v == vpos || v == vneg) ? (1u << win) : 0u;
      negs |= (v == vneg) ? (1u << win) : 0u;
    }
    while (hits) {
      const int win = __builtin_ctz(hits);
      hits &= hits - 1;
      const u32 payload = (u32)((size_t)win * table_stride + i) | (((negs >> win) & 1u) << 31);
      const u32 pos = atomicAdd(&count, 1u);
      if (pos < (u32)SMALL_LIST_CAP) list[pos] = payload;
      else add_entry(payload);
    }
  }
  __syncthreads();
  const u32 total = count;
  const u32 listed = total < (u32)SMALL_LIST_CAP ? total : (u32)SMALL_LIST_CAP;
  for (u32 e = lane; e < listed; e += T) add_entry(list[e]);
  small_tree_store<T>(sh, acc, total > (u32)SMALL_LIST_CAP ? (u32)T : total, b, buckets);
}
static_assert(254 / 8 + 1 <= 32, "window hit masks are 32 bits");

int launch_reduce_tail_row(u32* buckets, int lgB, int t_start, int sets, u32* out, int finish_affine, hipStream_t s);
int launch_window_combine_row(const u32* wsum, int nwin, int c, int out_xyzz, u32* out, hipStream_t s);
int launch_fold_partials_row(const u32* partials, int count, u32* out, hipStream_t s);
static size_t row_tail_max_ops() {
  static const size_t v = (size_t)tune_int("MZK_TAIL_MAX_OPS", 64);
  return v < 1 ? 1 : v;
}

static int launch_halving_steps(u32* buckets, int lgB, int sets, size_t tail_max, int* t_next, hipStream_t s) {
  int t = 0;
  while (t < lgB && ((size_t)(t + 1) << (lgB - t - 1)) > tail_max) {
    const size_t total = (size_t)(t + 1) << (lgB - t - 1);
    if (total * (size_t)sets >= ((size_t)1 << 16)) {
      hipLaunchKernelGGL(k_halve_step_wide, dim3((unsigned)((total + 127) / 128), (unsigned)sets), dim3(128), 0, s, buckets, lgB, t);
      t++;
      continue;
    }
    const int st = (lgB - t < HMULTI_MAX_S) ? lgB - t : HMULTI_MAX_S;
    const size_t multi_wgs = ((size_t)(t + 1) << (lgB - t - st)) * (size_t)sets;
    if (multi_wgs > (size_t)ctx().num_cu) {
      hipLaunchKernelGGL(k_halve_step, dim3((unsigned)((4 * total + 127) / 128), (unsigned)sets), dim3(128), 0, s, buckets, lgB, t);
      t++;
    } else {
      hipLaunchKernelGGL(k_halve_multi, dim3((unsigned)((size_t)(t + 1) << (lgB - t - st)), (unsigned)sets), dim3(HMULTI_THREADS), ((size_t)128 << st), s, buckets, lgB, t, st);
      t += st;
    }
  }
  MZK_HIP(hipGetLastError());
  *t_next = t;
  return MZK_OK;
}

static int reduce_bucket_sets(u32* buckets, int lgB, int sets, bool merged, int horner_c, u32* wsum, u32* d_out, bool out_partial_xyzz, hipStream_t s) {
  prof_begin(s, MZK_PH_MSM_REDUCE);
  int t_start = 0;
  MZK_TRY(launch_halving_steps(buckets, lgB, sets, row_tail_max_ops(), &t_start, s));
  if (merged) {
    MZK_TRY(launch_reduce_tail_row(buckets, lgB, t_start, 1, d_out, out_partial_xyzz ? 0 : 1, s));
    MZK_HIP(hipGetLastError());
    prof_end(s, MZK_PH_MSM_REDUCE);
    return MZK_OK;
  }
  MZK_TRY(launch_reduce_tail_row(buckets, lgB, t_start, sets, wsum, 0, s));
  MZK_HIP(hipGetLastError());
  prof_end(s, MZK_PH_MSM_REDUCE);
  prof_begin(s, MZK_PH_MSM_COMBINE);
  MZK_TRY(launch_window_combine_row((const u32*)wsum, sets, horner_c, out_partial_xyzz ? 1 : 0, d_out, s));
  prof_end(s, MZK_PH_MSM_COMBINE);
  return MZK_OK;
}

int msm_prepare_points(const void* d_points_plain, size_t n, void* d_points_mont, void* d_phi, hipStream_t s) {
  if (n == 0) return MZK_OK;
  hipLaunchKernelGGL(k_prepare_points, dim3((unsigned)((n + 255) / 256)), dim3(256), 0, s, (const u32*)d_points_plain,
                     (u32*)d_points_mont, n, (u32*)d_phi);
  MZK_HIP(hipGetLastError());
  return MZK_OK;
}
int msm_points_to_plain(const void* d_points_mont, size_t n, void* d_points_plain, hipStream_t s) {
  if (n == 0) return MZK_OK;
  hipLaunchKernelGGL(k_points_to_plain, dim3((unsigned)((n + 255) / 256)), dim3(256), 0, s, (const u32*)d_points_mont, n, (u32*)d_points_plain);
  MZK_HIP(hipGetLastError());
  return MZK_OK;
}
int msm_phi_points(const void* d_points_mont, size_t n, void* d_phi, hipStream_t s) {
  if (n == 0) return MZK_OK;
  hipLaunchKernelGGL(k_phi_points, dim3((unsigned)((n + 255) / 256)), dim3(256), 0, s, (const u32*)d_points_mont, n, (u32*)d_phi);
  MZK_HIP(hipGetLastError());
  return MZK_OK;
}

__global__ __launch_bounds__(128) void k_srs_state_init(const u32* __restrict__ pts_mont, size_t n, u32* __restrict__ state) {
  const size_t i = (size_t)blockIdx.x * blockDim.x + threadIdx.x;
  if (i >= n) return;
  u32 w[16];
  load_words8(pts_mont + i * 16, w);
  load_words8(pts_mont + i * 16 + 8, w + 8);
  Xyzz p = affine_words_is_inf(w) ? xyzz_inf() : xyzz_from_affine(affine_load_mont(w));
  xyzz_gstore(state, i, p);
}
__global__ __launch_bounds__(128) void k_srs_window_step(u32* __restrict__ state, size_t n, int c) {
  const size_t i = (size_t)blockIdx.x * blockDim.x + threadIdx.x;
  if (i >= n) return;
  Xyzz p = xyzz_gload(state, i);
  for (int d = 0; d < c; d++) p = xyzz_dbl_with<FeAsm>(p);
  xyzz_gstore(state, i, p);
}
int msm_build_tables(const void* d_points_mont, size_t n, void* d_tables, int window_bits, hipStream_t s) {
  if (n == 0) return MZK_OK;
  u32* state;
  MZK_TRY(ws_get(WS_XYZZ_TMP, n * 128, (void**)&state));
  const unsigned blocks = (unsigned)((n + 127) / 128);
  MZK_HIP(hipMemcpyAsync(d_tables, d_points_mont, n * 64, hipMemcpyDeviceToDevice, s));
  hipLaunchKernelGGL(k_srs_state_init, dim3(blocks), dim3(128), 0, s, (const u32*)d_points_mont, n, state);
  for (int win = 1; win < msm_table_windows(window_bits); win++) {
    hipLaunchKernelGGL(k_srs_window_step, dim3(blocks), dim3(128), 0, s, state, n, window_bits);
    MZK_TRY(xyzz_batch_to_affine(state, n, (u32*)d_tables + (size_t)win * n * 16, true, s));
  }
  MZK_HIP(hipGetLastError());
  return MZK_OK;
}

struct SortBufs {
  const u32* scalars; u32* binhist; void* tmp; u32* finehist; u32* scan3; u32* offsets; u32* entries;
  u32 *bin_tot, *bin_cur, *bin_start, *bucket_tot, *bucket_cur;
};
template <class REC>
static int sort_records(const MsmPlan& P, const SortBufs& a, hipStream_t s) {
  typedef typename REC::T R;
  const unsigned bins = 1u << P.cl;
#define MZK_STAGED(C, CLOG) hipLaunchKernelGGL((k_coarse_scatter_staged<REC, C, CLOG>), dim3(P.nwg), dim3(SORT2_THREADS), lds, s, a.scalars, P.n, P.L.table_stride, \
                                               P.key_shift, P.fine_mask, P.fb, (const u32*)a.binhist, P.nwg, (R*)a.tmp, (const u32*)a.bin_tot, a.bin_cur, a.bin_start)
#define MZK_DIRECT(C, CLOG) hipLaunchKernelGGL((k_coarse_scatter<REC, C, CLOG>), dim3(P.nwg), dim3(SORT2_THREADS), 0, s, a.scalars, P.n, P.L, P.key_shift, P.fine_mask, \
                                               P.fb, (const u32*)a.binhist, P.nwg, (R*)a.tmp, (const u32*)a.bin_tot, a.bin_cur, a.bin_start)
  if (P.scatter_staged) {
    const size_t lds = stage_lds_bytes(P.coarse_c, P.cl, sizeof(R));
    bool& attr = ctx().attr_done[sizeof(R) == 4 ? ATTR_COARSE_STAGED4 : ATTR_COARSE_STAGED8];
    if (!attr) {
      MZK_HIP(hipFuncSetAttribute((const void*)k_coarse_scatter_staged<REC, 16>, hipFuncAttributeMaxDynamicSharedMemorySize, 160 * 1024));
      MZK_HIP(hipFuncSetAttribute((const void*)k_coarse_scatter_staged<REC, 17>, hipFuncAttributeMaxDynamicSharedMemorySize, 160 * 1024));
      MZK_HIP(hipFuncSetAttribute((const void*)k_coarse_scatter_staged<REC, 20>, hipFuncAttributeMaxDynamicSharedMemorySize, 160 * 1024));
      MZK_HIP(hipFuncSetAttribute((const void*)k_coarse_scatter_staged<REC, 20, 10>, hipFuncAttributeMaxDynamicSharedMemorySize, 160 * 1024));
      MZK_HIP(hipFuncSetAttribute((const void*)k_coarse_scatter_staged<REC, 17, 9>, hipFuncAttributeMaxDynamicSharedMemorySize, 160 * 1024));
      attr = true;
    }
    if (P.coarse_c == 17 && P.cl == 9) MZK_STAGED(17, 9);
    else if (P.coarse_c == 20 && P.cl == 10) MZK_STAGED(20, 10);
    else if (P.coarse_c == 20) MZK_STAGED(20, COARSE_LOG);
    else if (P.coarse_c == 17) MZK_STAGED(17, COARSE_LOG);
    else MZK_STAGED(16, COARSE_LOG);
  }
  else if (P.cl == 10) MZK_DIRECT(0, 10);
  else MZK_DIRECT(0, COARSE_LOG);
#undef MZK_STAGED
#undef MZK_DIRECT
  const u32* bounds = a.bin_tot ? (const u32*)a.bin_start : (const u32*)a.binhist;
  const int bstride = a.bin_tot ? 1 : P.nwg;
  hipLaunchKernelGGL((k_fine_count<REC>), dim3(P.fine_wgs), dim3(SORT2_THREADS), 0, s, (const R*)a.tmp, bounds, bstride, P.F, P.S,
                     P.fb, a.finehist, (int)bins, P.slice_cap, a.bucket_tot);
  if (!P.fine_free) MZK_TRY(launch_exclusive_scan((const u32*)a.finehist, a.finehist, P.own.n_fine, a.scan3, s));
  if (P.F <= STAGE_F_MAX) {
    const size_t lds = ((size_t)3 * P.F + SORT2_THREADS + STAGE_CAP) * 4 + (size_t)STAGE_CAP * 2;
    bool& staged_attr = ctx().attr_done[sizeof(R) == 4 ? ATTR_FINE_SCATTER4 : ATTR_FINE_SCATTER8];
    if (!staged_attr) {
      MZK_HIP(hipFuncSetAttribute((const void*)k_fine_scatter<REC>, hipFuncAttributeMaxDynamicSharedMemorySize, 160 * 1024));
      staged_attr = true;
    }
    hipLaunchKernelGGL((k_fine_scatter<REC>), dim3(P.fine_wgs), dim3(SORT2_THREADS), lds, s, (const R*)a.tmp, bounds, bstride, P.F,
                       P.S, P.fb, (const u32*)a.finehist, a.offsets, a.entries, P.NBtot, (int)bins, P.slice_cap, (const u32*)a.bucket_tot, a.bucket_cur);
  } else {
    hipLaunchKernelGGL((k_fine_scatter_direct<REC>), dim3(P.fine_wgs), dim3(SORT2_THREADS), 0, s, (const R*)a.tmp, bounds, bstride,
                       P.F, P.S, P.fb, (const u32*)a.finehist, a.offsets, a.entries, P.NBtot, (int)bins, P.slice_cap);
  }
  MZK_HIP(hipGetLastError());
  return MZK_OK;
}

int msm_dev_impl(const void* d_scalars, const void* d_points, size_t n, int point_kind, size_t table_stride, void* d_out,
                 bool out_partial_xyzz, hipStream_t s, const std::function<int()>* points_ready, const MsmChunkCtx* cc) {
  if (!d_out || ((!d_scalars || !d_points) && n)) { set_error("msm: null pointer"); return MZK_E_ARG; }
  if (cc && (n < SMALL_MAX_N || n > cc->n_alloc)) { set_error("msm: chunk of %zu pairs (chunks hold 4097 .. %zu)", n, cc->n_alloc); return MZK_E_ARG; }
  if (n == 0) {
    if (points_ready) MZK_TRY((*points_ready)());
    MZK_HIP(hipMemsetAsync(d_out, 0, out_partial_xyzz ? 128 : 64, s));
    return MZK_OK;
  }
  const size_t n_shape = cc ? cc->n_total : n, i0 = cc ? cc->i0 : 0;
  const MsmPlan P = msm_plan(n, n_shape, cc ? cc->n_alloc : n, point_kind, table_stride, ctx().num_cu, cc ? cc->K : 0, msm_knobs());
  if (P.err != MZK_OK) { set_error("%s", P.msg); return P.err; }
  u32 *pm = nullptr, *counts = nullptr, *offsets = nullptr, *ranks = nullptr, *entries = nullptr, *scan = nullptr, *buckets = nullptr,
      *slots = nullptr, *wghist = nullptr, *wsum = nullptr;
  const struct { WsSlot slot; size_t bytes; u32** p; size_t words; } req[] = {
      {WS_MSM_POINTS, P.ws.points, &pm, 0}, {WS_MSM_COUNTS, P.ws.counts, &counts, 0}, {WS_MSM_OFFSETS, P.ws.offsets, &offsets, P.NBtot + 1},
      {WS_MSM_CURSOR, P.ws.cursor, &ranks, 0}, {WS_MSM_ENTRIES, P.ws.entries, &entries, P.alloc.E}, {WS_MSM_SCAN, P.ws.scan, &scan, 0},
      {WS_MSM_BUCKETS, P.ws.buckets, &buckets, P.NB * 32}, {WS_MSM_SLOTS, P.ws.slots, &slots, P.slot_region_words},
      {WS_MSM_WGHIST, P.ws.wghist, &wghist, 0}, {WS_MSM_OUT, P.ws.out, &wsum, 0}};
  for (const auto& r : req)
    if (r.bytes) { MZK_TRY(ws_get(r.slot, r.bytes, (void**)r.p)); *r.p += (cc ? cc->k : 0) * r.words; }
  const u32* pts = (pm ? pm : (const u32*)d_points) + i0 * 16;
  bool prepared = false;
  auto prepare = [&]() -> int {
    if (prepared) return MZK_OK;
    prepared = true;
    if (points_ready) MZK_TRY((*points_ready)());
    if (!pm) return MZK_OK;
    prof_begin(s, MZK_PH_MSM_PREPARE);
    MZK_TRY(msm_prepare_points((const u32*)d_points + i0 * 16, n, pm + i0 * 16, pm + (n_shape + i0) * 16, s));
    prof_end(s, MZK_PH_MSM_PREPARE);
    return MZK_OK;
  };
  if (P.path == MsmPath::SmallScan) {
    MZK_TRY(prepare());
    prof_begin(s, MZK_PH_MSM_ACCUMULATE);
#define MZK_SCAN_CASE(C) case C: hipLaunchKernelGGL((k_small_accumulate_scan<256, C>), dim3((unsigned)P.NB), dim3(256), 0, s, (const u32*)d_scalars, n, P.L.table_stride, pts, buckets); break;
    switch (P.L.c) { MZK_SCAN_CASE(8) MZK_SCAN_CASE(10) MZK_SCAN_CASE(11) MZK_SCAN_CASE(12) MZK_SCAN_CASE(13) }
#undef MZK_SCAN_CASE
    prof_end(s, MZK_PH_MSM_ACCUMULATE);
  } else if (P.path == MsmPath::SmallSort) {
    MZK_TRY(prepare());
    prof_begin(s, MZK_PH_MSM_SORT);
    hipLaunchKernelGGL(k_small_sort, dim3(1), dim3(SMALL_SORT_THREADS), (P.NB + SMALL_SORT_THREADS) * 4, s, (const u32*)d_scalars, n, P.L, (int)P.NB, offsets, entries);
    prof_end(s, MZK_PH_MSM_SORT);
    prof_begin(s, MZK_PH_MSM_ACCUMULATE);
    if (P.small_wide)
      hipLaunchKernelGGL(k_small_accumulate<256>, dim3((unsigned)P.NB), dim3(256), 0, s, pts, (const u32*)offsets, (const u32*)entries, buckets);
    else
      hipLaunchKernelGGL(k_small_accumulate<64>, dim3((unsigned)P.NB), dim3(64), 0, s, pts, (const u32*)offsets, (const u32*)entries, buckets);
    prof_end(s, MZK_PH_MSM_ACCUMULATE);
  } else {
    u32* heavy = slots + P.nslots * SLOT_WORDS;
    prof_begin(s, MZK_PH_MSM_SORT);
    MZK_HIP(hipMemsetAsync(heavy, 0, (size_t)HEAVY_HDR * 4, s));
    if (P.path == MsmPath::TwoLevel) {
      u32* finehist = wghist + P.alloc.n_coarse + 1;
      const SortBufs sb{(const u32*)d_scalars, wghist, ranks, finehist, scan + scan_scratch_words(P.alloc.n_coarse) + 2, offsets, entries,
                        P.coarse_free ? heavy + SORT_CTR_AT : nullptr, P.coarse_free ? heavy + SORT_CTR_AT + SORT_CTR_BINS : nullptr,
                        P.coarse_free ? finehist + P.alloc.n_fine + 1 : nullptr, P.fine_free ? counts : nullptr, P.fine_free ? counts + P.NBtot : nullptr};
#define MZK_CCOUNT(C, CLOG) hipLaunchKernelGGL((k_coarse_count<C, CLOG>), dim3(P.nwg), dim3(SORT2_THREADS), 0, s, (const u32*)d_scalars, n, P.L, P.key_shift, wghist, \
                                               P.nwg, sb.bin_tot, sb.bucket_tot, P.fine_free ? 2 * P.NBtot : (size_t)0)
      if (P.coarse_c == 20 && P.cl == 10) MZK_CCOUNT(20, 10);
      else if (P.coarse_c == 17 && P.cl == 9) MZK_CCOUNT(17, 9);
      else if (P.cl == 10) MZK_CCOUNT(0, 10);
      else if (P.coarse_c == 20) MZK_CCOUNT(20, COARSE_LOG);
      else if (P.coarse_c == 17) MZK_CCOUNT(17, COARSE_LOG);
      else if (P.coarse_c == 16) MZK_CCOUNT(16, COARSE_LOG);
      else MZK_CCOUNT(0, COARSE_LOG);
#undef MZK_CCOUNT
      if (!P.coarse_free) MZK_TRY(launch_exclusive_scan((const u32*)wghist, wghist, P.own.n_coarse, scan, s));
      MZK_TRY(P.compact ? sort_records<Rec4>(P, sb, s) : sort_records<Rec8>(P, sb, s));
    } else if (P.path == MsmPath::LdsOnePass) {
      const size_t lds = P.NB * 4;
      bool& lds_attr_set = ctx().attr_done[ATTR_DIGITS_LDS];
      if (!lds_attr_set) {
        MZK_HIP(hipFuncSetAttribute((const void*)k_digits_count_lds, hipFuncAttributeMaxDynamicSharedMemorySize, 160 * 1024));
        MZK_HIP(hipFuncSetAttribute((const void*)k_digits_scatter_lds, hipFuncAttributeMaxDynamicSharedMemorySize, 160 * 1024));
        lds_attr_set = true;
      }
      hipLaunchKernelGGL(k_digits_count_lds, dim3(P.nwg), dim3(LDS_SORT_THREADS), lds, s, (const u32*)d_scalars, n, P.per_wg, P.L, wghist, ranks);
      hipLaunchKernelGGL(k_wg_hist_prefix, dim3((unsigned)((P.NB + 255) / 256)), dim3(256), 0, s, wghist, P.nwg, (int)P.NB, counts);
      MZK_TRY(launch_exclusive_scan((const u32*)counts, offsets, P.NB, scan, s));
      hipLaunchKernelGGL(k_digits_scatter_lds, dim3(P.nwg), dim3(LDS_SORT_THREADS), lds, s, (const u32*)d_scalars, n, P.per_wg, P.L, (const u32*)offsets,
                         (const u32*)wghist, (const u32*)ranks, entries);
    } else {
      const unsigned nblk = (unsigned)((n + 255) / 256);
      MZK_HIP(hipMemsetAsync(counts, 0, P.NB * 4, s));
      hipLaunchKernelGGL(k_digits_count, dim3(nblk), dim3(256), 0, s, (const u32*)d_scalars, n, P.L, counts, ranks);
      MZK_TRY(launch_exclusive_scan((const u32*)counts, offsets, P.NB, scan, s));
      hipLaunchKernelGGL(k_digits_scatter, dim3(nblk), dim3(256), 0, s, (const u32*)d_scalars, n, P.L, offsets, ranks, entries);
    }
    MZK_HIP(hipGetLastError());
    prof_end(s, MZK_PH_MSM_SORT);
    MZK_TRY(prepare());
    prof_begin(s, MZK_PH_MSM_ACCUMULATE);
    hipLaunchKernelGGL(k_seg_accumulate<false>, dim3((unsigned)((P.T + 255) / 256)), dim3(256), 0, s, pts, offsets, entries, slots, P.NB, P.seg, P.t_max);
    prof_end(s, MZK_PH_MSM_ACCUMULATE);
    prof_begin(s, MZK_PH_MSM_SEG_COMBINE);
    if (P.combine_wide)
      hipLaunchKernelGGL(k_seg_combine_wide, dim3((unsigned)((P.NB + 127) / 128)), dim3(128), 0, s, slots, offsets, buckets, P.NB, P.seg, heavy, P.t_max);
    else
      hipLaunchKernelGGL(k_seg_combine, dim3((unsigned)((4 * P.NB + 127) / 128)), dim3(128), 0, s, slots, offsets, buckets, P.NB, P.seg, heavy, (const u32*)nullptr, 0, P.t_max);
    hipLaunchKernelGGL(k_seg_combine_heavy, dim3(HEAVY_GRID), dim3(HEAVY_THREADS), 0, s, (const u32*)slots, (const u32*)offsets, buckets, heavy, P.max_heavy);
    MZK_HIP(hipGetLastError());
    prof_end(s, MZK_PH_MSM_SEG_COMBINE);
    if (cc) return MZK_OK;
  }
  MZK_TRY(reduce_bucket_sets(buckets, P.lgB, P.red_windows, P.one_set, P.horner_c, wsum, (u32*)d_out, out_partial_xyzz, s));
  MZK_HIP(hipGetLastError());
  return MZK_OK;
}

__global__ __launch_bounds__(128) void k_fold_bucket_sets(u32* __restrict__ buckets, size_t NB, int K) {
  const size_t b = (size_t)blockIdx.x * blockDim.x + threadIdx.x;
  if (b >= NB) return;
  Xyzz acc = xyzz_gload(buckets, b);
  for (int k = 1; k < K; k++) acc = xyzz_add_with<FeAsm>(acc, xyzz_gload(buckets, (size_t)k * NB + b));
  xyzz_gstore(buckets, b, acc);
}
bool msm_chunkable(size_t n_total, int point_kind, size_t table_stride) { return msm_chunkable(n_total, point_kind, table_stride, msm_knobs()); }
int msm_chunked_impl(const MsmChunk* chunks, int K, const void* d_points, size_t n_total, int point_kind, size_t table_stride, void* d_out,
                     bool out_partial_xyzz, hipStream_t s, const std::function<int(int)>* before_chunk) {
  if (!chunks || K < 1 || K > 8 || !d_out || !d_points) { set_error("msm_chunked: bad argument"); return MZK_E_ARG; }
  size_t n_alloc = 0, covered = 0;
  for (int k = 0; k < K; k++) {
    if (chunks[k].i0 != covered) { set_error("msm_chunked: chunks must be consecutive"); return MZK_E_ARG; }
    covered += chunks[k].n;
    n_alloc = chunks[k].n > n_alloc ? chunks[k].n : n_alloc;
  }
  if (covered != n_total || !msm_chunkable(n_total, point_kind, table_stride)) { set_error("msm_chunked: chunks do not cover a chunkable problem"); return MZK_E_ARG; }
  for (int k = 0; k < K; k++) {
    if (before_chunk) MZK_TRY((*before_chunk)(k));
    if (chunks[k].ready) MZK_HIP(hipStreamWaitEvent(s, chunks[k].ready, 0));
    const MsmChunkCtx cc{k, K, chunks[k].i0, n_total, n_alloc};
    MZK_TRY(msm_dev_impl(chunks[k].d_scalars, d_points, chunks[k].n, point_kind, table_stride, d_out, out_partial_xyzz, s, nullptr, &cc));
  }
  const MsmPlan P = msm_plan(n_alloc, n_total, n_alloc, point_kind, table_stride, ctx().num_cu, K, msm_knobs());
  u32 *buckets, *wsum;
  MZK_TRY(ws_get(WS_MSM_BUCKETS, P.ws.buckets, (void**)&buckets));
  MZK_TRY(ws_get(WS_MSM_OUT, (size_t)MAX_WINDOWS * 128, (void**)&wsum));
  if (K > 1) {
    prof_begin(s, MZK_PH_MSM_SEG_COMBINE);
    hipLaunchKernelGGL(k_fold_bucket_sets, dim3((unsigned)((P.NB + 127) / 128)), dim3(128), 0, s, buckets, P.NB, K);
    MZK_HIP(hipGetLastError());
    prof_end(s, MZK_PH_MSM_SEG_COMBINE);
  }
  MZK_TRY(reduce_bucket_sets(buckets, P.lgB, P.red_windows, P.one_set, P.horner_c, wsum, (u32*)d_out, out_partial_xyzz, s));
  MZK_HIP(hipGetLastError());
  return MZK_OK;
}

constexpr int MANY_CHUNK = 1024;
constexpr int MANY_THREADS = 256;
constexpr int MANY_PER_LANE = MANY_CHUNK / MANY_THREADS;
template <int C>
__global__ __launch_bounds__(MANY_THREADS) void k_many_count(const u32* __restrict__ scalars, size_t n, size_t stride_words, int nch, u32* __restrict__ cnt) {
  constexpr int NB = 1 << (C - 1);
  __shared__ u32 hist[NB];
  const size_t j = blockIdx.x / (unsigned)nch;
  const int ch = (int)(blockIdx.x % (unsigned)nch);
  for (int b = threadIdx.x; b < NB; b += MANY_THREADS) hist[b] = 0;
  __syncthreads();
  const u32* sc = scalars + j * stride_words;
  const size_t lo = (size_t)ch * MANY_CHUNK;
  const size_t hi = (lo + MANY_CHUNK < n) ? lo + MANY_CHUNK : n;
  u32 w[MANY_PER_LANE][8];
#pragma unroll
  for (int k = 0; k < MANY_PER_LANE; k++) {
    const size_t i = lo + threadIdx.x + (size_t)k * MANY_THREADS;
    if (i < hi) load_scalar_canonical(sc, i, w[k]);
  }
#pragma unroll
  for (int k = 0; k < MANY_PER_LANE; k++) {
    const size_t i = lo + threadIdx.x + (size_t)k * MANY_THREADS;
    if (i < hi) walk_digits_merged<C>(w[k], 0, i, [&](int, u32 key, u32) { counter_inc_agg(hist, key); });
  }
  __syncthreads();
  for (int b = threadIdx.x; b < NB; b += MANY_THREADS) cnt[(j * NB + b) * (size_t)nch + ch] = hist[b];
}
template <int C>
__global__ __launch_bounds__(MANY_THREADS) void k_many_scatter(const u32* __restrict__ scalars, size_t n, size_t stride_words, int nch, size_t table_stride,
                                                                const u32* __restrict__ offs, u32* __restrict__ compact, size_t nbuckets,
                                                                u32* __restrict__ entries) {
  constexpr int NB = 1 << (C - 1);
  __shared__ u32 cursor[NB];
  const size_t j = blockIdx.x / (unsigned)nch;
  const int ch = (int)(blockIdx.x % (unsigned)nch);
  for (int b = threadIdx.x; b < NB; b += MANY_THREADS) {
    const u32 o = offs[(j * NB + b) * (size_t)nch + ch];
    cursor[b] = o;
    if (compact != nullptr && ch == 0) compact[j * NB + b] = o;
  }
  if (compact != nullptr && blockIdx.x == 0 && threadIdx.x == 0) compact[nbuckets] = offs[nbuckets * (size_t)nch];
  __syncthreads();
  const u32* sc = scalars + j * stride_words;
  const size_t lo = (size_t)ch * MANY_CHUNK;
  const size_t hi = (lo + MANY_CHUNK < n) ? lo + MANY_CHUNK : n;
  u32 w[MANY_PER_LANE][8];
#pragma unroll
  for (int k = 0; k < MANY_PER_LANE; k++) {
    const size_t i = lo + threadIdx.x + (size_t)k * MANY_THREADS;
    if (i < hi) load_scalar_canonical(sc, i, w[k]);
  }
#pragma unroll
  for (int k = 0; k < MANY_PER_LANE; k++) {
    const size_t i = lo + threadIdx.x + (size_t)k * MANY_THREADS;
    if (i < hi) walk_digits_merged<C>(w[k], table_stride, i, [&](int, u32 key, u32 payload) { entries[counter_inc_agg(cursor, key)] = payload; });
  }
}

constexpr int SORT1_THREADS = 1024;
constexpr int SORT1_PER_LANE = MANY_CHUNK / SORT1_THREADS;
template <int C>
__global__ __launch_bounds__(SORT1_THREADS) void k_many_sort1(const u32* __restrict__ scalars, size_t n, size_t stride_words, size_t table_stride, u32 cap,
                                                              u32* __restrict__ offsets, size_t npoly, u32* __restrict__ entries, u32* __restrict__ tails) {
  constexpr int NB = 1 << (C - 1);
  constexpr int PER = (NB + SORT1_THREADS - 1) / SORT1_THREADS;
  __shared__ u32 hist[NB];
  __shared__ u32 scan[SORT1_THREADS];
  extern __shared__ u32 stage[];
  const size_t j = blockIdx.x;
  const int tid = threadIdx.x;
  for (int b = tid; b < NB; b += SORT1_THREADS) hist[b] = 0;
  __syncthreads();
  const u32* sc = scalars + j * stride_words;
  u32 w[SORT1_PER_LANE][8];
#pragma unroll
  for (int k = 0; k < SORT1_PER_LANE; k++) {
    const size_t i = tid + (size_t)k * SORT1_THREADS;
    if (i < n) load_scalar_canonical(sc, i, w[k]);
  }
#pragma unroll
  for (int k = 0; k < SORT1_PER_LANE; k++) {
    const size_t i = tid + (size_t)k * SORT1_THREADS;
    if (i < n) walk_digits_merged<C>(w[k], 0, i, [&](int, u32 key, u32) { counter_inc_agg(hist, key); });
  }
  __syncthreads();
  u32 local = 0;
#pragma unroll
  for (int q = 0; q < PER; q++) { const int b = tid * PER + q; if (b < NB) local += hist[b]; }
  u32 total;
  u32 run = block_excl_scan<SORT1_THREADS>(local, scan, &total);
  const u32 base = (u32)(j * cap);
#pragma unroll
  for (int q = 0; q < PER; q++) {
    const int b = tid * PER + q;
    if (b < NB) { const u32 c = hist[b]; hist[b] = run; offsets[j * NB + b] = base + run; run += c; }
  }
  if (j + 1 == npoly && tid == 0) offsets[npoly * NB] = (u32)(npoly * cap);
  if (tid == 0) tails[j] = base + total;
  __syncthreads();
#pragma unroll
  for (int k = 0; k < SORT1_PER_LANE; k++) {
    const size_t i = tid + (size_t)k * SORT1_THREADS;
    if (i < n) walk_digits_merged<C>(w[k], table_stride, i, [&](int, u32 key, u32 payload) { stage[counter_inc_agg(hist, key)] = payload; });
  }
  __syncthreads();
  for (u32 e = tid; e < cap; e += SORT1_THREADS) entries[base + e] = (e < total) ? stage[e] : MANY_SENTINEL;
}

bool msm_many_supported(int window_bits) { return window_bits == 8 || (window_bits >= 10 && window_bits <= 13); }

int msm_many_dev_impl(const void* d_scalars, size_t n, size_t stride_elems, size_t count, const void* d_tables, int c, size_t table_stride, void* d_out,
                      hipStream_t s) {
  if (count == 0) return MZK_OK;
  if (!d_out || ((!d_scalars || !d_tables) && n)) { set_error("msm_many: null pointer"); return MZK_E_ARG; }
  if (!msm_many_supported(c)) { set_error("msm_many: window width %d has no grid-batched path", c); return MZK_E_ARG; }
  if (n == 0) {
    MZK_HIP(hipMemsetAsync(d_out, 0, count * 64, s));
    return MZK_OK;
  }
  const int nwin = msm_table_windows(c), lgB = c - 1;
  const size_t NB = (size_t)1 << lgB;
  if ((size_t)nwin * table_stride > ((size_t)1 << 31)) { set_error("msm_many: table rows exceed the 31-bit point references"); return MZK_E_ARG; }
  const int nch = (int)((n + MANY_CHUNK - 1) / MANY_CHUNK);
  size_t per_pass = ((size_t)1 << 21) / NB;
  const size_t by_coefs = (((size_t)1 << 22) + n - 1) / n;
  if (by_coefs < per_pass) per_pass = by_coefs;
  if (per_pass < 1) per_pass = 1;
  for (size_t first = 0; first < count; first += per_pass) {
    const size_t cnt = (count - first < per_pass) ? count - first : per_pass;
    const u32* sc = (const u32*)d_scalars + first * stride_elems * 8;
    u32* out = (u32*)d_out + first * 16;
    const size_t NBtot = cnt * NB, ncnt = NBtot * (size_t)nch;
    const size_t E_max = cnt * n * (size_t)nwin;
    const size_t resident_lanes = (size_t)ctx().num_cu * 4 * 4 * 64;
    size_t seg_sz = (E_max + resident_lanes - 1) / resident_lanes;
    if (seg_sz < 16) seg_sz = 16;
    const u32 seg = (u32)seg_sz;
    const size_t T = (E_max + seg_sz - 1) / seg_sz;
    const size_t nslots = T + NBtot + 1;
    const size_t max_heavy = (T + NBtot) / HEAVY_SLOTS_SORT1 + 1;
    const size_t heavy_words = heavy_total_words(max_heavy);
    u32 *offs, *compact, *entries, *scan_tmp, *buckets, *slots;
    MZK_TRY(ws_get(WS_MSM_COUNTS, (ncnt + 1) * 4, (void**)&offs));
    MZK_TRY(ws_get(WS_MSM_ENTRIES, E_max * 4, (void**)&entries));
    MZK_TRY(ws_get(WS_MSM_SCAN, scan_scratch_words(ncnt) * 4, (void**)&scan_tmp));
    MZK_TRY(ws_get(WS_MSM_BUCKETS, NBtot * 128, (void**)&buckets));
    MZK_TRY(ws_get(WS_MSM_SLOTS, nslots * SLOT_WORDS * 4 + heavy_words * 4, (void**)&slots));
    compact = offs;
    u32* tails = nullptr;
    if (nch > 1) MZK_TRY(ws_get(WS_MSM_OFFSETS, (NBtot + 1) * 4, (void**)&compact));
    else MZK_TRY(ws_get(WS_MSM_OFFSETS, cnt * 4, (void**)&tails));
    u32* heavy = slots + nslots * SLOT_WORDS;
    prof_begin(s, MZK_PH_MSM_SORT);
    MZK_HIP(hipMemsetAsync(heavy, 0, (size_t)HEAVY_HDR * 4, s));
    const unsigned nwg = (unsigned)(cnt * (size_t)nch);
    const bool one_kernel_sort = nch == 1;
    if (one_kernel_sort) {
      bool& done = ctx().attr_done[ATTR_MANY_SORT1];
      if (!done) {
        MZK_HIP(hipFuncSetAttribute((const void*)k_many_sort1<8>, hipFuncAttributeMaxDynamicSharedMemorySize, 140 * 1024));
        MZK_HIP(hipFuncSetAttribute((const void*)k_many_sort1<10>, hipFuncAttributeMaxDynamicSharedMemorySize, 140 * 1024));
        MZK_HIP(hipFuncSetAttribute((const void*)k_many_sort1<11>, hipFuncAttributeMaxDynamicSharedMemorySize, 140 * 1024));
        MZK_HIP(hipFuncSetAttribute((const void*)k_many_sort1<12>, hipFuncAttributeMaxDynamicSharedMemorySize, 140 * 1024));
        MZK_HIP(hipFuncSetAttribute((const void*)k_many_sort1<13>, hipFuncAttributeMaxDynamicSharedMemorySize, 140 * 1024));
        done = true;
      }
    }
#define MZK_MANY_CASE(C) case C:                                                                                                                    \
      if (one_kernel_sort) {                                                                                                                         \
        hipLaunchKernelGGL((k_many_sort1<C>), dim3(nwg), dim3(SORT1_THREADS), n * (size_t)nwin * 4, s, sc, n, stride_elems * 8, table_stride,       \
                           (u32)(n * (size_t)nwin), offs, cnt, entries, tails);                                                                           \
        break;                                                                                                                                       \
      }                                                                                                                                              \
      hipLaunchKernelGGL((k_many_count<C>), dim3(nwg), dim3(MANY_THREADS), 0, s, sc, n, stride_elems * 8, nch, offs);                                \
      MZK_TRY(launch_exclusive_scan((const u32*)offs, offs, ncnt, scan_tmp, s));                                                                     \
      hipLaunchKernelGGL((k_many_scatter<C>), dim3(nwg), dim3(MANY_THREADS), 0, s, sc, n, stride_elems * 8, nch, table_stride, (const u32*)offs,     \
                         nch > 1 ? compact : (u32*)nullptr, NBtot, entries);                                                                         \
      break;
    switch (c) { MZK_MANY_CASE(8) MZK_MANY_CASE(10) MZK_MANY_CASE(11) MZK_MANY_CASE(12) MZK_MANY_CASE(13) }
#undef MZK_MANY_CASE
    MZK_HIP(hipGetLastError());
    prof_end(s, MZK_PH_MSM_SORT);
    prof_begin(s, MZK_PH_MSM_ACCUMULATE);
    const u32 t_max = one_kernel_sort ? 0u : (u32)T;
    if (one_kernel_sort)
      hipLaunchKernelGGL(k_seg_accumulate<true>, dim3((unsigned)((T + 255) / 256)), dim3(256), 0, s, (const u32*)d_tables, (const u32*)compact, (const u32*)entries,
                         slots, NBtot, seg, t_max);
    else
      hipLaunchKernelGGL(k_seg_accumulate<false>, dim3((unsigned)((T + 255) / 256)), dim3(256), 0, s, (const u32*)d_tables, (const u32*)compact, (const u32*)entries,
                         slots, NBtot, seg, t_max);
    prof_end(s, MZK_PH_MSM_ACCUMULATE);
    prof_begin(s, MZK_PH_MSM_SEG_COMBINE);
    const unsigned cgrid = (unsigned)((4 * NBtot + 127) / 128);
    hipLaunchKernelGGL(k_seg_combine, dim3(cgrid), dim3(128), 0, s, slots, (const u32*)compact, buckets, NBtot, seg, heavy, (const u32*)tails, lgB, t_max);
    hipLaunchKernelGGL(k_seg_combine_heavy, dim3(HEAVY_GRID), dim3(HEAVY_THREADS), 0, s, (const u32*)slots, (const u32*)compact, buckets, heavy, max_heavy);
    MZK_HIP(hipGetLastError());
    prof_end(s, MZK_PH_MSM_SEG_COMBINE);
    prof_begin(s, MZK_PH_MSM_REDUCE);
    int t_start = 0;
    MZK_TRY(launch_halving_steps(buckets, lgB, (int)cnt, row_tail_max_ops(), &t_start, s));
    MZK_TRY(launch_reduce_tail_row(buckets, lgB, t_start, (int)cnt, out, 1, s));
    MZK_HIP(hipGetLastError());
    prof_end(s, MZK_PH_MSM_REDUCE);
  }
  return MZK_OK;
}

constexpr int DIRECT_THREADS = 256;
size_t msm_direct_bytes(size_t n, int c) { return (size_t)msm_table_windows(c) * n * ((size_t)1 << (c - 1)) * 64; }
__global__ __launch_bounds__(64) void k_direct_chain(const u32* __restrict__ rows_mont, size_t rows, int M, u32* __restrict__ out_xyzz) {
  const size_t r = (size_t)blockIdx.x * blockDim.x + threadIdx.x;
  if (r >= rows) return;
  u32 w[16];
  load_words8(rows_mont + r * 16, w);
  load_words8(rows_mont + r * 16 + 8, w + 8);
  const bool inf = affine_words_is_inf(w);
  const Affine a = affine_load_mont(w);
  Xyzz acc = xyzz_inf();
  for (int m = 0; m < M; m++) {
    if (!inf) acc = xyzz_madd_signed_with<FeCpp>(acc, a, false);
    xyzz_gstore(out_xyzz, r * (size_t)M + m, acc);
  }
}
int msm_build_direct(const void* d_points_mont, size_t n, int c, void* d_direct, hipStream_t s) {
  if (n == 0) return MZK_OK;
  const int nwin = msm_table_windows(c), M = 1 << (c - 1);
  const size_t rows = (size_t)nwin * n;
  u32 *tables, *tmp;
  MZK_TRY(ws_get(WS_MISC_C, rows * 64, (void**)&tables));
  MZK_TRY(msm_build_tables(d_points_mont, n, tables, c, s));
  size_t slice = ((size_t)1 << 21) / (size_t)M;
  if (slice < 64) slice = 64;
  if (slice > rows) slice = rows;
  MZK_TRY(ws_get(WS_MISC_D, slice * (size_t)M * 128, (void**)&tmp));
  for (size_t r0 = 0; r0 < rows; r0 += slice) {
    const size_t cnt = (rows - r0 < slice) ? rows - r0 : slice;
    hipLaunchKernelGGL(k_direct_chain, dim3((unsigned)((cnt + 63) / 64)), dim3(64), 0, s, (const u32*)tables + r0 * 16, cnt, M, tmp);
    MZK_HIP(hipGetLastError());
    MZK_TRY(xyzz_batch_to_affine(tmp, cnt * (size_t)M, (u32*)d_direct + r0 * (size_t)M * 16, true, s));
  }
  return MZK_OK;
}
template <int C>
__device__ __forceinline__ bool direct_item(const u32* __restrict__ sc, size_t t, size_t table_stride, const u32* __restrict__ direct, const u32** rec, bool* neg) {
  constexpr int NWIN = 254 / C + 1;
  constexpr u32 HALF = 1u << (C - 1), MASKC = (1u << C) - 1u;
  const size_t i = t / NWIN;
  const int win = (int)(t - i * NWIN);
  u32 w[8], tw[10];
  load_scalar_canonical(sc, i, w);
  u64 cy = 0;
#pragma unroll
  for (int k = 0; k < 8; k++) { cy += (u64)w[k] + digit_bias_word(C, k); tw[k] = (u32)cy; cy >>= 32; }
  tw[8] = (u32)cy + digit_bias_word(C, 8);
  tw[9] = 0;
  const int bit = win * C, k = bit >> 5, sft = bit & 31;
  u32 lo = tw[0], hi = tw[1];
#pragma unroll
  for (int q = 1; q < 9; q++) { lo = (k == q) ? tw[q] : lo; hi = (k == q) ? tw[q + 1] : hi; }
  const u32 v = (u32)((((u64)hi << 32) | lo) >> sft) & MASKC;
  if (v == HALF - 1u) return false;
  *neg = v < HALF - 1u;
  const u32 mag = *neg ? (HALF - 1u) - v : v - (HALF - 1u);
  *rec = direct + (((size_t)win * table_stride + i) * HALF + (mag - 1u)) * 16;
  return true;
}
template <int C>
__global__ __launch_bounds__(DIRECT_THREADS) void k_direct_accumulate(const u32* __restrict__ scalars, size_t n, size_t stride_words, int parts, size_t table_stride,
                                                                       const u32* __restrict__ direct, u32* __restrict__ slots) {
  constexpr int NWIN = 254 / C + 1;
  const size_t j = blockIdx.x / (unsigned)parts;
  const int part = (int)(blockIdx.x % (unsigned)parts);
  const u32* sc = scalars + j * stride_words;
  const size_t items = n * NWIN;
  const size_t per = (items + parts - 1) / parts;
  const size_t first = (size_t)part * per;
  const size_t last = (first + per < items) ? first + per : items;
  Xyzz acc = xyzz_inf();
  u32 pw[16];
  const u32* rec = nullptr;
  bool neg = false;
  size_t t = first + threadIdx.x;
  bool have = (t < last) && direct_item<C>(sc, t, table_stride, direct, &rec, &neg);
  if (have) { load_words8(rec, pw); load_words8(rec + 8, pw + 8); }
  while (t < last) {
    const bool cur_have = have, cur_neg = neg;
    u32 cw[16];
#pragma unroll
    for (int q = 0; q < 16; q++) cw[q] = pw[q];
    t += DIRECT_THREADS;
    have = (t < last) && direct_item<C>(sc, t, table_stride, direct, &rec, &neg);
    if (have) { load_words8(rec, pw); load_words8(rec + 8, pw + 8); }
    if (cur_have && !affine_words_is_inf(cw)) acc = xyzz_madd_signed_with<FeAsm>(acc, affine_load_mont(cw), cur_neg);
  }
  xyzz_gstore_raw(slots, (size_t)blockIdx.x * DIRECT_THREADS + threadIdx.x, acc);
}
__global__ __launch_bounds__(DIRECT_THREADS) void k_direct_finish(const u32* __restrict__ slots, int parts, u32* __restrict__ scratch, u32* __restrict__ out) {
  __shared__ __attribute__((aligned(16))) u32 sh[DIRECT_THREADS * 32];
  const size_t j = blockIdx.x;
  Xyzz acc = xyzz_gload_raw(slots, (j * parts) * DIRECT_THREADS + threadIdx.x);
  for (int p = 1; p < parts; p++) acc = xyzz_add_with<FeAsm>(acc, xyzz_gload_raw(slots, (j * parts + p) * DIRECT_THREADS + threadIdx.x));
  small_tree_store<DIRECT_THREADS>(sh, acc, DIRECT_THREADS, j, scratch);
  __syncthreads();
  if (threadIdx.x < 64) wave_store_affine(sh, out + j * 16);
}
constexpr int DIRECT_FINISH_PARTS = 8;
__global__ __launch_bounds__(DIRECT_THREADS) void k_direct_fold(const u32* __restrict__ slots, int parts, int groups, u32* __restrict__ folded) {
  const size_t j = blockIdx.x / (unsigned)groups;
  const int g = (int)(blockIdx.x % (unsigned)groups);
  Xyzz acc = xyzz_gload_raw(slots, (j * parts + g) * DIRECT_THREADS + threadIdx.x);
  for (int p = g + groups; p < parts; p += groups) acc = xyzz_add_with<FeAsm>(acc, xyzz_gload_raw(slots, (j * parts + p) * DIRECT_THREADS + threadIdx.x));
  xyzz_gstore_raw(folded, (size_t)blockIdx.x * DIRECT_THREADS + threadIdx.x, acc);
}
int msm_direct_many_dev_impl(const void* d_scalars, size_t n, size_t stride_elems, size_t count, const void* d_direct, int c, size_t table_stride, void* d_out,
                             hipStream_t s) {
  if (count == 0) return MZK_OK;
  if (!d_out || ((!d_scalars || !d_direct) && n)) { set_error("msm_direct_many: null pointer"); return MZK_E_ARG; }
  if (n == 0) {
    MZK_HIP(hipMemsetAsync(d_out, 0, count * 64, s));
    return MZK_OK;
  }
  const size_t items = n * (size_t)msm_table_windows(c);
  const size_t per_pass = (size_t)1 << 12;
  for (size_t first = 0; first < count; first += per_pass) {
    const size_t cnt = (count - first < per_pass) ? count - first : per_pass;
    static const int parts_mul = tune_int("MZK_DIRECT_PARTS_MUL", 1);
    const size_t resident = (size_t)ctx().num_cu * 3 * (size_t)(parts_mul > 0 ? parts_mul : 1);
    size_t parts = (resident + cnt / 2) / cnt;
    const size_t max_parts = (items + DIRECT_THREADS - 1) / DIRECT_THREADS;
    if (parts > max_parts) parts = max_parts;
    if (parts > 64) parts = 64;
    if (parts < 1) parts = 1;
    size_t groups = 0;
    if (parts > (size_t)DIRECT_FINISH_PARTS) for (groups = 2; groups * groups < parts; groups++) {}
    u32 *slots, *scratch;
    MZK_TRY(ws_get(WS_MSM_SLOTS, cnt * (parts + groups) * DIRECT_THREADS * SLOT_WORDS * 4, (void**)&slots));
    MZK_TRY(ws_get(WS_MSM_BUCKETS, cnt * 128, (void**)&scratch));
    const u32* sc = (const u32*)d_scalars + first * stride_elems * 8;
    const unsigned nwg = (unsigned)(cnt * parts);
    prof_begin(s, MZK_PH_MSM_ACCUMULATE);
#define MZK_DIRECT_CASE(C) case C: hipLaunchKernelGGL((k_direct_accumulate<C>), dim3(nwg), dim3(DIRECT_THREADS), 0, s, sc, n, stride_elems * 8, (int)parts, table_stride, (const u32*)d_direct, slots); break;
    switch (c) { MZK_DIRECT_CASE(8) MZK_DIRECT_CASE(9) MZK_DIRECT_CASE(10) MZK_DIRECT_CASE(11) MZK_DIRECT_CASE(12)
      default: set_error("msm_direct_many: no kernel for %d-bit direct tables", c); return MZK_E_ARG; }
#undef MZK_DIRECT_CASE
    MZK_HIP(hipGetLastError());
    prof_end(s, MZK_PH_MSM_ACCUMULATE);
    prof_begin(s, MZK_PH_MSM_REDUCE);
    if (groups) {
      u32* folded = slots + cnt * parts * DIRECT_THREADS * SLOT_WORDS;
      hipLaunchKernelGGL(k_direct_fold, dim3((unsigned)(cnt * groups)), dim3(DIRECT_THREADS), 0, s, (const u32*)slots, (int)parts, (int)groups, folded);
      hipLaunchKernelGGL(k_direct_finish, dim3((unsigned)cnt), dim3(DIRECT_THREADS), 0, s, (const u32*)folded, (int)groups, scratch, (u32*)d_out + first * 16);
    } else {
      hipLaunchKernelGGL(k_direct_finish, dim3((unsigned)cnt), dim3(DIRECT_THREADS), 0, s, (const u32*)slots, (int)parts, scratch, (u32*)d_out + first * 16);
    }
    MZK_HIP(hipGetLastError());
    prof_end(s, MZK_PH_MSM_REDUCE);
  }
  return MZK_OK;
}
bool srs_many_capable(const mzk_srs* srs) { return srs->d_direct != nullptr || (srs->has_tables && srs->sets == 1 && msm_many_supported(srs->window_bits)); }
constexpr size_t MANY_WIDE_FROM = (size_t)1 << 13;
constexpr int MANY_WIDE_BITS = 12;
int msm_many_srs(const mzk_srs* srs, const void* d_scalars, size_t n, size_t stride_elems, size_t count, void* d_out, hipStream_t s,
                 size_t shift) {
  if (shift && shift + n > srs->n) { set_error("msm_many: points [%zu, %zu) past the handle's %zu", shift, shift + n, srs->n); return MZK_E_LENGTH; }
  if (srs->d_direct)
    return msm_direct_many_dev_impl(d_scalars, n, stride_elems, count, (const char*)srs->d_direct + shift * ((size_t)1 << (srs->direct_bits - 1)) * 64,
                                    srs->direct_bits, srs->n, d_out, s);
  if (n >= MANY_WIDE_FROM && srs->has_tables && srs->sets == 1 && srs->window_bits < MANY_WIDE_BITS) {
    if (!srs->d_tables_wide && srs->wide_bits == 0) {
      const size_t bytes = (size_t)msm_table_windows(MANY_WIDE_BITS) * srs->n * 64;
      const size_t own = (size_t)srs->n * 64 * srs->table_rows() + srs->direct_bytes;
      void* t = nullptr;
      const bool within_budget = table_budget_bytes() == 0 || own + bytes <= table_budget_bytes();
      if (within_budget && dev_alloc(&t, bytes, "wide window tables of the grid-batched pass") == MZK_OK) {
        const int rc = msm_build_tables(srs->d_points_mont, srs->n, t, MANY_WIDE_BITS, s);
        if (rc != MZK_OK) { (void)hipFree(t); return rc; }
        srs->d_tables_wide = t; srs->wide_bits = MANY_WIDE_BITS; srs->wide_bytes = bytes;
      } else {
        srs->wide_bits = -1;
        if (within_budget) clear_error();
      }
    }
    if (srs->d_tables_wide)
      return msm_many_dev_impl(d_scalars, n, stride_elems, count, (const char*)srs->d_tables_wide + shift * 64, srs->wide_bits, srs->n, d_out, s);
  }
  return msm_many_dev_impl(d_scalars, n, stride_elems, count, (const char*)srs->d_points_mont + shift * 64, srs->window_bits, srs->n, d_out, s);
}

int msm_fold_partials_impl(const void* d_partials, int count, void* d_out_xy, hipStream_t s) {
  if (!d_partials || !d_out_xy || count < 0) { set_error("fold_partials: bad argument"); return MZK_E_ARG; }
  MZK_TRY(launch_fold_partials_row((const u32*)d_partials, count, (u32*)d_out_xy, s));
  return MZK_OK;
}

}

namespace mzk {
__device__ __forceinline__ u64 splitmix64(u64& s) {
  u64 z = (s += 0x9e3779b97f4a7c15ULL);
  z = (z ^ (z >> 30)) * 0xbf58476d1ce4e5b9ULL;
  z = (z ^ (z >> 27)) * 0x94d049bb133111ebULL;
  return z ^ (z >> 31);
}
template <class P> __device__ void synth_words(u64 seed, u64 index, u32* w) {
  constexpr int NL = P::NW / 2;
  u32 pw[P::NW];
  {
    Fe<P> pm;
    for (int i = 0; i < P::L; i++) pm.l[i] = P::P[i];
    fe_pack<P>(pm, pw);
  }
  for (u64 attempt = 0;; attempt++) {
    u64 s = seed ^ (index * 0xd1342543de82ef95ULL) ^ (attempt * 0xa0761d6478bd642fULL);
    for (int i = 0; i < NL; i++) {
      u64 v = splitmix64(s);
      w[2 * i] = (u32)v;
      w[2 * i + 1] = (u32)(v >> 32);
    }
    constexpr int topbits = P::BITS - 64 * (NL - 1);
    if (topbits < 64) {
      const u64 mask = (((u64)1 << topbits) - 1);
      w[P::NW - 2] &= (u32)mask;
      w[P::NW - 1] &= (u32)(mask >> 32);
    }
    bool lt = false, decided = false;
    for (int i = P::NW - 1; i >= 0 && !decided; i--) {
      if (w[i] != pw[i]) { lt = w[i] < pw[i]; decided = true; }
    }
    if (decided && lt) return;
  }
}
template <class P> __global__ void k_synth_field(u64 seed, size_t n, u32* __restrict__ out) {
  const size_t i = (size_t)blockIdx.x * blockDim.x + threadIdx.x;
  if (i >= n) return;
  u32 w[P::NW];
  synth_words<P>(seed, i, w);
  for (int k = 0; k < P::NW; k++) out[i * P::NW + k] = w[k];
}
__global__ void k_synth_g1(u64 seed, size_t n, u32* __restrict__ out) {
  typedef FqParams P;
  const size_t i = (size_t)blockIdx.x * blockDim.x + threadIdx.x;
  if (i >= n) return;
  u32 w[8];
  synth_words<P>(seed, i, w);
  u32 e[8];
  {
    Fe<P> pm;
    for (int k = 0; k < P::L; k++) pm.l[k] = P::P[k];
    u32 qw[8];
    fe_pack<P>(pm, qw);
    for (int k = 0; k < 8; k++) e[k] = (qw[k] >> 2) | ((k + 1 < 8) ? (qw[k + 1] << 30) : 0u);
    u32 c = 1;
    for (int k = 0; k < 8 && c; k++) { e[k] += c; c = (e[k] == 0) ? 1u : 0u; }
  }
  Fe<P> b3;
  for (int k = 0; k < P::L; k++) b3.l[k] = FQ_B_MONT[k];
  Fe<P> x = fe_reduce<P>(fe_to_mont<P>(fe_unpack<P>(w)));
  Fe<P> one = fe_one<P>();
  for (;;) {
    Fe<P> rhs = fe_reduce<P>(fe_add<P>(fe_mul<P>(fe_sqr<P>(x), x), b3));
    Fe<P> y = fe_pow_words<P>(rhs, e, 8);
    Fe<P> y2 = fe_reduce<P>(fe_sqr<P>(y));
    if (fe_eq_canon<P>(y2, rhs) && !fe_is_zero_canon<P>(rhs)) {
      Affine a;
      a.x = x;
      a.y = fe_reduce<P>(y);
      u32 o[16];
      affine_store_plain(a, o);
      for (int k = 0; k < 16; k++) out[i * 16 + k] = o[k];
      return;
    }
    x = fe_reduce<P>(fe_add<P>(x, one));
  }
}
int synth_field_impl(int fid, u64 seed, size_t n, void* d_out, hipStream_t s) {
  if (n == 0) return MZK_OK;
  const unsigned blocks = (unsigned)((n + 255) / 256);
  MZK_TRY(field_check(fid, "synth", true));
  return with_field3(fid, [&](auto tag) -> int {
    hipLaunchKernelGGL((k_synth_field<typename decltype(tag)::P>), dim3(blocks), dim3(256), 0, s, seed, n, (u32*)d_out);
    MZK_HIP(hipGetLastError());
    return MZK_OK;
  });
}
int synth_g1_impl(u64 seed, size_t n, void* d_out, hipStream_t s) {
  if (n == 0) return MZK_OK;
  hipLaunchKernelGGL(k_synth_g1, dim3((unsigned)((n + 127) / 128)), dim3(128), 0, s, seed, n, (u32*)d_out);
  MZK_HIP(hipGetLastError());
  return MZK_OK;
}
}
```

myzkp_amd/csrc/mzk_msm_plan.h:

```cpp
#pragma once
#include <stddef.h>
#include <stdint.h>
#include <stdio.h>
#include "../../include/mzk.h"

namespace mzk {

enum { MSM_PTS_PLAIN = 0, MSM_PTS_MONT = 1, MSM_PTS_TABLES = 2 };
static inline int msm_table_windows(int c) { return 254 / c + 1; }
static inline int msm_table_rows(int c, int sets) { return 254 / (c * sets) + 1; }

constexpr int SCALAR_BITS = 254;
constexpr int MAX_WINDOWS = 32;
constexpr int GLV_MAG_BITS = 126;
constexpr int SLOT_WORDS = 36;
constexpr int ACC_RESIDENT_WAVES = 3;

struct DigitLayout {
  int c, nwin, merged;
  int sets;
  size_t table_stride;
  int glv;
  size_t phi_offset;
};

struct MsmShape { int c, nwin, lgB; size_t nbuckets; };
static MsmShape choose_shape_glv(size_t n, int force_c = 0) {
  int lg = 0;
  while (((size_t)1 << lg) < 2 * n) lg++;
  int c = lg - 3;
  if (c < 8) c = 8;
  if (c > 16) c = 16;
  if (c == 15) c = 16;
  if (n >= ((size_t)3 << 21)) c = 19;
  if (force_c > 0) c = force_c;
  for (; c > 8; c--) {
    const int nw = GLV_MAG_BITS / c + 1;
    if (GLV_MAG_BITS - c * (nw - 1) >= 5) break;
  }
  MsmShape s;
  s.c = c;
  s.nwin = GLV_MAG_BITS / c + 1;
  s.lgB = c - 1;
  s.nbuckets = (size_t)s.nwin << s.lgB;
  return s;
}

#ifndef MZK_COARSE_LOG
#define MZK_COARSE_LOG 8
#endif
constexpr int COARSE_LOG = MZK_COARSE_LOG;
constexpr int COARSE_PER_WG = 4096;
constexpr int FINE_MAX = 8192;
constexpr int STAGE_F_MAX = 2048;
constexpr size_t SMALL_MAX_N = 4097;
constexpr size_t SMALL_MAX_BUCKETS = 8192;
constexpr int SCAN_ITEMS = 8;
constexpr int SCAN_BLOCK = 256 * SCAN_ITEMS;
constexpr size_t SCAN_DIRECT_BLOCKS = 2048;
static inline size_t scan_scratch_words(size_t n) {
  const size_t sb = (n + SCAN_BLOCK - 1) / SCAN_BLOCK;
  return sb + 2 + (sb > SCAN_DIRECT_BLOCKS ? scan_scratch_words(sb) : 0);
}
constexpr uint32_t HEAVY_SLOTS = 32;
constexpr int HEAVY_GRID = 512;
constexpr int SORT_CTR_BINS = 1024;
constexpr int SORT_CTR_AT = 2 + HEAVY_GRID;
constexpr int HEAVY_HDR = SORT_CTR_AT + 2 * SORT_CTR_BINS;
constexpr size_t heavy_list_words(size_t max_heavy) { return (HEAVY_HDR + 2 * max_heavy + 2 + 3) & ~(size_t)3; }
constexpr size_t heavy_total_words(size_t max_heavy) { return heavy_list_words(max_heavy) + (size_t)HEAVY_GRID * 32 + 8; }

struct MsmKnobs {
  int glv_c = 0;
  int small_scan = 1;
  int scan_max_log = 14;
  int acc_seg = 0;
  int coarse_log_20 = 10;
  int coarse_log_17 = 9;
  int per_fine = 0;
  int sort_scan_free = 3;
  int combine_wide_min_log = 17;
};

enum class MsmPath { SmallScan, SmallSort, TwoLevel, LdsOnePass, Atomic };
struct MsmWsBytes { size_t points, counts, offsets, cursor, entries, buckets, scan, slots, wghist, out; };
struct MsmSizing { size_t E, T, n_coarse, n_fine; };

struct MsmPlan {
  int err = MZK_OK;
  char msg[192] = {};
  size_t n = 0;
  DigitLayout L{};
  int lgB = 0, red_windows = 0, horner_c = 0;
  size_t NB = 0, NBtot = 0;
  bool one_set = false, small_wide = false;
  MsmPath path = MsmPath::SmallSort;
  int cl = 0, F = 0, fb = 0, key_shift = 0, S = 0, nwg = 0;
  uint32_t fine_mask = 0, slice_cap = 0;
  unsigned fine_wgs = 0;
  size_t per_wg = 0;
  bool compact = false, coarse_free = false, fine_free = false, scatter_staged = false;
  int coarse_c = 0;
  uint32_t seg = 0, t_max = 0;
  size_t T = 0, nslots = 0, max_heavy = 0, slot_region_words = 0;
  bool combine_wide = false;
  MsmSizing own{}, alloc{};
  MsmWsBytes ws{}, ws_used{};
  MsmPlan& fail(const char* fmt, size_t a = 0, size_t b = 0, size_t c = 0) { err = MZK_E_ARG; snprintf(msg, sizeof msg, fmt, a, b, c); return *this; }
};

static inline size_t msm_slot_region_words(size_t T, size_t NB) {
  return ((T + NB + 1) * SLOT_WORDS + heavy_total_words((T + NB) / HEAVY_SLOTS + 1) + 3) & ~(size_t)3;
}
static inline MsmPlan& msm_sized(MsmPlan& P, size_t regions) {
  for (int u = 0; u < 2; u++) {
    const MsmSizing& z = u ? P.own : P.alloc;
    MsmWsBytes& w = u ? P.ws_used : P.ws;
    w.points = P.ws.points, w.out = P.ws.out;
    w.offsets = regions * (P.NBtot + 1) * 4;
    w.entries = regions * z.E * 4;
    w.buckets = regions * P.NB * 128;
    if (P.path == MsmPath::SmallScan || P.path == MsmPath::SmallSort) continue;
    const bool two = P.path == MsmPath::TwoLevel;
    w.counts = 2 * P.NBtot * 4;
    w.cursor = z.E * (two ? 8 : 4);
    w.slots = regions * msm_slot_region_words(z.T, P.NB) * 4;
    w.wghist = two ? (z.n_coarse + 1 + z.n_fine + 1 + ((size_t)1 << P.cl) + 1) * 4 : P.path == MsmPath::LdsOnePass ? (size_t)P.nwg * P.NB * 4 : 0;
    w.scan = two ? (scan_scratch_words(z.n_coarse) + scan_scratch_words(z.n_fine) + 4) * 4 : scan_scratch_words(P.NB) * 4;
  }
  return P;
}

static inline MsmPlan msm_plan(size_t n, size_t n_shape, size_t n_alloc, int point_kind, size_t table_stride, int num_cu, int chunks,
                               const MsmKnobs& kn) {
  MsmPlan P;
  P.n = n;
  if (n > ((size_t)1 << 27)) return P.fail("msm: n > 2^27 not supported");
  const int kind = point_kind & 0xff, table_c = (point_kind >> 8) & 0xff, table_sets = (point_kind >> 16) & 0xff;
  DigitLayout& L = P.L;
  L.merged = kind == MSM_PTS_TABLES;
  L.sets = (L.merged && table_sets) ? table_sets : 1;
  L.table_stride = table_stride;
  L.glv = !L.merged;
  L.phi_offset = kind == MSM_PTS_PLAIN ? n_shape : table_stride;
  const MsmShape sh = choose_shape_glv(n_shape, kn.glv_c);
  L.c = L.merged ? (table_c ? table_c : 16) : sh.c;
  L.nwin = L.merged ? msm_table_windows(L.c) : sh.nwin;
  P.NB = L.merged ? (size_t)L.sets << (L.c - 1) : sh.nbuckets;
  P.lgB = L.c - 1, P.red_windows = L.merged ? L.sets : L.nwin;
  P.one_set = L.merged && L.sets == 1, P.horner_c = P.one_set ? 0 : L.c;
  const size_t windows_per_pair = L.glv ? 2 * L.nwin : L.nwin, regions = chunks ? chunks : 1;
  const size_t E_max = P.own.E = n * windows_per_pair, E_alloc = P.alloc.E = n_alloc * windows_per_pair;
  P.ws.points = kind == MSM_PTS_PLAIN ? 2 * n_shape * 64 : 0;
  P.ws.out = chunks ? 0 : (size_t)MAX_WINDOWS * 128;
  P.NBtot = P.NB;
  if (L.glv && (P.NB & (P.NB - 1)) != 0 && L.c >= 17) { P.NBtot = 1; while (P.NBtot < P.NB) P.NBtot <<= 1; }

  const bool scan_ok = P.one_set && kn.small_scan != 0 && n <= ((size_t)1 << kn.scan_max_log) && (L.c == 8 || (L.c >= 10 && L.c <= 13));
  if (!chunks && (scan_ok || n < (L.merged ? SMALL_MAX_N : SMALL_MAX_N - 1)) && P.NB <= SMALL_MAX_BUCKETS) {
    P.path = scan_ok ? MsmPath::SmallScan : MsmPath::SmallSort;
    P.small_wide = E_max / P.NB > 64;
    return msm_sized(P, 1);
  }
  const size_t ref_max = L.merged ? (size_t)msm_table_rows(L.c, L.sets) * table_stride : L.phi_offset + n;
  if (ref_max > ((size_t)1 << 31) || E_max >= ((size_t)1 << 32))
    return P.fail("msm: %zu pairs x %zu windows (table stride %zu) exceed the 31-bit point references / 32-bit entry offsets", n, (size_t)L.nwin, table_stride);

  const size_t resident_lanes = (size_t)num_cu * 4 * ACC_RESIDENT_WAVES * 64;
  size_t seg = (E_max + resident_lanes - 1) / resident_lanes;
  seg = kn.acc_seg > 0 ? (size_t)kn.acc_seg : seg < 16 ? 16 : seg;
  P.seg = (uint32_t)seg;
  P.T = P.own.T = (E_max + seg - 1) / seg;
  P.t_max = kn.acc_seg > 0 ? 0u : (uint32_t)P.T;
  P.nslots = P.T + P.NB + 1;
  P.max_heavy = (P.T + P.NB) / HEAVY_SLOTS + 1;
  P.combine_wide = P.NB >= ((size_t)1 << kn.combine_wide_min_log);
  const size_t T_seg = E_alloc / (kn.acc_seg > 0 ? (size_t)kn.acc_seg : 16) + 1;
  P.alloc.T = !chunks ? P.T : kn.acc_seg > 0 ? T_seg : (resident_lanes + 1 < T_seg ? resident_lanes + 1 : T_seg);
  P.slot_region_words = msm_slot_region_words(P.alloc.T, P.NB);

  const bool plain_merged = L.merged && L.sets == 1;
  P.cl = (plain_merged && L.c == 20 && kn.coarse_log_20 == 10) ? 10 : COARSE_LOG;
  if (plain_merged && L.c == 17 && kn.coarse_log_17 == 9 && COARSE_LOG == 8 && ref_max > ((size_t)1 << (31 - 8)) && ref_max <= ((size_t)1 << (31 - 7)))
    P.cl = 9;
  if (L.glv && P.NBtot > ((size_t)STAGE_F_MAX << COARSE_LOG)) P.cl = 10;
  const size_t cbins = (size_t)1 << P.cl;
  const bool two_level = (P.NBtot & (P.NBtot - 1)) == 0 && P.NBtot >= 4096 && (P.NBtot / cbins) <= (size_t)FINE_MAX &&
                         (n >= 4096 || (L.merged && P.NBtot > ((size_t)1 << 15)));
  if (chunks && !two_level) return P.fail("msm: chunk mode needs the two-level sort (layout %zu bits, %zu buckets)", (size_t)L.c, P.NB);
  P.path = two_level ? MsmPath::TwoLevel : L.merged ? MsmPath::LdsOnePass : MsmPath::Atomic;
  if (P.path == MsmPath::LdsOnePass) {
    const size_t nwg = (n + 4095) / 4096;
    P.nwg = nwg < 1 ? 1 : nwg > (size_t)num_cu ? num_cu : (int)nwg;
    P.per_wg = (n + P.nwg - 1) / P.nwg;
  }
  if (!two_level) return msm_sized(P, regions);
  while (((size_t)1 << P.key_shift) < P.NBtot) P.key_shift++;
  P.key_shift -= P.cl;
  P.F = (int)(P.NBtot / cbins);
  P.fine_mask = (uint32_t)P.F - 1u;
  while ((1 << P.fb) < P.F) P.fb++;
  P.nwg = (int)((n + COARSE_PER_WG - 1) / COARSE_PER_WG);
  const size_t per_fine = kn.per_fine > 0 ? (size_t)kn.per_fine : (P.F >= 4096 ? 131072 : P.F >= 2048 ? 65536 : (L.glv ? 16384 : 32768));
  const size_t S = (E_max / cbins + per_fine - 1) / per_fine;
  P.S = S < 2 ? 2 : S > 64 ? 64 : (int)S;
  const size_t slice_nom = (E_max + cbins * (size_t)P.S - 1) / (cbins * (size_t)P.S);
  P.slice_cap = (uint32_t)(slice_nom + slice_nom / 2 + 1);
  P.fine_wgs = (unsigned)(cbins * (size_t)P.S + (E_max + P.slice_cap - 1) / P.slice_cap + 1);
  P.own.n_coarse = cbins * P.nwg;
  P.own.n_fine = (size_t)P.F * P.fine_wgs;
  const size_t slice_nom_a = (E_alloc + cbins * (size_t)64 - 1) / (cbins * (size_t)64);
  P.alloc.n_coarse = chunks ? cbins * ((n_alloc + COARSE_PER_WG - 1) / COARSE_PER_WG) : P.own.n_coarse;
  P.alloc.n_fine = chunks ? (size_t)P.F * (cbins * 64 + (E_alloc + slice_nom_a) / (slice_nom_a + slice_nom_a / 2 + 1) + 2) : P.own.n_fine;
  P.compact = ref_max <= ((size_t)1 << (31 - P.fb));
  P.coarse_free = (kn.sort_scan_free & 1) != 0 && cbins <= (size_t)SORT_CTR_BINS;
  P.fine_free = (kn.sort_scan_free & 2) != 0 && P.F <= STAGE_F_MAX;
  P.coarse_c = (plain_merged && (L.c == 16 || L.c == 17 || L.c == 20)) ? L.c : 0;
  P.scatter_staged = P.coarse_c != 0;
  return msm_sized(P, regions);
}

#if defined(__HIPCC__)
#define MZK_HD __host__ __device__ __forceinline__
#else
#define MZK_HD inline
#endif
constexpr uint32_t MANY_SENTINEL = 0xffffffffu;

MZK_HD bool seg_span(uint64_t t, uint32_t seg, uint32_t total, uint32_t* e0, uint32_t* e1) {
  const uint64_t e0w = t * seg;
  if (e0w >= total) return false;
  *e0 = (uint32_t)e0w;
  *e1 = (e0w + seg < total) ? (uint32_t)e0w + seg : total;
  return true;
}

template <int K, class Offset>
MZK_HD size_t seg_bucket_search(Offset offset_at, size_t nbuckets, uint32_t e) {
  size_t lo = 0, hi = nbuckets;
  while (hi - lo > 1) {
    const size_t step = (hi - lo + K - 1) / K;
    uint32_t v[K];
#if defined(__HIPCC__)
#pragma unroll
#endif
    for (int j = 1; j < K; j++) v[j] = offset_at(lo + j * step < hi ? lo + j * step : hi);
    size_t below = 0;
#if defined(__HIPCC__)
#pragma unroll
#endif
    for (int j = 1; j < K; j++) below += v[j] <= e ? 1 : 0;
    lo += below * step;
    if (lo + step < hi) hi = lo + step;
  }
  return lo;
}
template <class Offset>
MZK_HD size_t seg_first_bucket(Offset offset_at, size_t nbuckets, uint32_t e) {
  return nbuckets <= ((size_t)1 << 20) ? seg_bucket_search<16>(offset_at, nbuckets, e) : seg_bucket_search<32>(offset_at, nbuckets, e);
}

template <bool SENT, class Entry, class Offset, class IssueRow, class TakeRow, class Flush, class Add>
MZK_HD void seg_walk(uint32_t e0, uint32_t e1, size_t b, size_t nbuckets, Entry entry_at, Offset offset_at, IssueRow issue_row, TakeRow take_row,
                     Flush flush, Add add) {
  const auto row_ref = [](uint32_t ent) { return (SENT && ent == MANY_SENTINEL) ? 0u : ent; };
  const auto end_after_next = [&](size_t bb) { return offset_at(bb + 2 <= nbuckets ? bb + 2 : nbuckets); };
  uint32_t ent = entry_at(e0);
  uint32_t ent1 = entry_at(e1 - e0 > 1 ? e0 + 1 : e0);
  issue_row(row_ref(ent));
  uint32_t bend = offset_at(b + 1), bend1 = end_after_next(b);
  for (uint32_t e = e0; e < e1; e++) {
    take_row(ent);
    const uint32_t ent2 = entry_at(e1 - e > 2 ? e + 2 : e1 - 1);
    issue_row(row_ref(ent1));
    if (e >= bend) {
      flush(b);
      b++, bend = bend1;
      while (e >= bend) b++, bend = offset_at(b + 1);
      bend1 = end_after_next(b);
    }
    add(e, ent, b);
    ent = ent1, ent1 = ent2;
  }
  flush(b);
}

static inline bool msm_chunkable(size_t n_total, int point_kind, size_t table_stride, const MsmKnobs& kn) {
  if (n_total < ((size_t)1 << 18)) return false;
  const MsmPlan P = msm_plan(n_total, n_total, n_total, point_kind, table_stride, 256, 1, kn);
  return P.err == MZK_OK && P.L.sets == 1 && P.path == MsmPath::TwoLevel;
}

}
```

Measured before the change: 766.5 million pairs/s.

## Fuse fine count and scatter into one-pass kernel with over-cap fallback

Adds a k_fine_one kernel for the two-level bucket sort. When a coarse bin fits in one slice, a single workgroup builds its histogram, computes offsets and scatters entries directly, which removes the separate fine-count launch, the global fine scan and one extra read of the temp records. Bins that exceed the slice cap fall back to a histogram-only pass and are scattered by an over_only k_fine_scatter launch. The change also skips the heavy-header memset when the previous call left it clean, tracked by a workspace allocation generation counter. In exchange it adds more code paths and stateful cross-call bookkeeping that could go wrong if a buffer is reused stale.

```diff
diff --git a/myzkp_amd/csrc/mzk_api.hip b/myzkp_amd/csrc/mzk_api.hip
--- a/myzkp_amd/csrc/mzk_api.hip
+++ b/myzkp_amd/csrc/mzk_api.hip
@@ -81,6 +81,7 @@
   for (const auto& b : c.ws) if (b.p && b.epoch != g_call_epoch) idle += b.cap;
   if (!idle) return poly_idle;
   (void)hipDeviceSynchronize();
+  c.ws_alloc_gen++;
   bool table_slot_freed = false;
   for (int k = 0; k < WS_COUNT; k++) {
     WsBuf& b = c.ws[k];
@@ -113,6 +114,7 @@
   WsBuf& b = ctx().ws[slot];
   b.epoch = g_call_epoch;
   if (bytes > b.cap) {
+    ctx().ws_alloc_gen++;
     if (b.p) {
       MZK_HIP(hipDeviceSynchronize());
       MZK_HIP(hipFree(b.p));
@@ -143,6 +145,7 @@
 void ws_release_all() {
   Context& c = ctx();
   c.ws_gen = ++g_gen_counter;
+  c.ws_alloc_gen++;
   for (auto& b : c.ws) {
     if (b.p) (void)hipFree(b.p);
     b.p = nullptr; b.cap = 0;
diff --git a/myzkp_amd/csrc/mzk_common.h b/myzkp_amd/csrc/mzk_common.h
--- a/myzkp_amd/csrc/mzk_common.h
+++ b/myzkp_amd/csrc/mzk_common.h
@@ -55,6 +55,8 @@
   hipStream_t ws_last = nullptr;
   bool ws_used = false;
   bool attr_done[ATTR_COUNT] = {};
+  const uint32_t* msm_hdr_clean = nullptr;
+  uint64_t msm_hdr_gen = 0, ws_alloc_gen = 1;
   hipStream_t xstream[MZK_MAX_CTX] = {};
   hipEvent_t xdone[MZK_MAX_CTX] = {};
   hipEvent_t xready = nullptr;
diff --git a/myzkp_amd/csrc/mzk_msm.hip b/myzkp_amd/csrc/mzk_msm.hip
--- a/myzkp_amd/csrc/mzk_msm.hip
+++ b/myzkp_amd/csrc/mzk_msm.hip
@@ -15,7 +15,7 @@
     return MsmKnobs{tune_int("MZK_GLV_C", d.glv_c), tune_int("MZK_SMALL_SCAN", d.small_scan), tune_int("MZK_SCAN_MAX_LOG", d.scan_max_log),
                     tune_int("MZK_ACC_SEG", d.acc_seg), tune_int("MZK_COARSE_LOG_20", d.coarse_log_20),
                     tune_int("MZK_COARSE_LOG_17", d.coarse_log_17), tune_int("MZK_PER_FINE", d.per_fine), tune_int("MZK_SORT_SCAN_FREE", d.sort_scan_free),
-                    tune_int("MZK_COMBINE_WIDE_MIN_LOG", d.combine_wide_min_log)};
+                    tune_int("MZK_COMBINE_WIDE_MIN_LOG", d.combine_wide_min_log), tune_int("MZK_FINE_ONE", d.fine_one)};
   }();
   return k;
 }
@@ -551,43 +551,61 @@
     __syncthreads();
   }
 }
-struct FineSlice { int bin, s, Sb; u32 lo, hi, start; bool active; };
-__device__ __forceinline__ FineSlice fine_plan(const u32* __restrict__ binbase, int nwg, int bins, int S, u32 cap, u32* sc, u32* res) {
+__device__ __forceinline__ u32 plan_incl_scan(u32 v, u32* sc) {
+  const int tid = threadIdx.x, lane = tid & 63, wave = tid >> 6;
+#pragma unroll
+  for (int off = 1; off < 64; off <<= 1) { const u32 t = __shfl_up(v, off, 64); if (lane >= off) v += t; }
+  if (lane == 63) sc[wave] = v;
+  __syncthreads();
+  if (wave == 0) {
+    u32 t = (lane < SORT2_THREADS / 64) ? sc[lane] : 0u;
+#pragma unroll
+    for (int off = 1; off < SORT2_THREADS / 64; off <<= 1) { const u32 u = __shfl_up(t, off, 64); if (lane >= off) t += u; }
+    if (lane < SORT2_THREADS / 64) sc[lane] = t;
+  }
+  __syncthreads();
+  return v + (wave ? sc[wave - 1] : 0u);
+}
+__device__ __forceinline__ FineSlice fine_plan(const u32* __restrict__ binbase, int nwg, int bins, int S, u32 cap, u32* sc, u32* res, bool over_only = false) {
   const int tid = threadIdx.x;
   u32 start = 0, len = 0, Sb = 0;
   if (tid < bins) {
     start = binbase[(size_t)tid * nwg];
     len = binbase[(size_t)(tid + 1) * nwg] - start;
-    Sb = (len + cap - 1) / cap;
-    if (Sb < (u32)S) Sb = (u32)S;
+    Sb = fine_bin_slices(len, cap, (u32)S);
   }
   if (tid == 0) res[0] = 0xffffffffu;
-  const int lane = tid & 63, wave = tid >> 6;
-  u32 v = Sb;
-#pragma unroll
-  for (int off = 1; off < 64; off <<= 1) { const u32 t = __shfl_up(v, off, 64); if (lane >= off) v += t; }
-  if (lane == 63) sc[wave] = v;
-  __syncthreads();
-  if (wave == 0) {
-    u32 t = (lane < SORT2_THREADS / 64) ? sc[lane] : 0u;
-#pragma unroll
-    for (int off = 1; off < SORT2_THREADS / 64; off <<= 1) { const u32 u = __shfl_up(t, off, 64); if (lane >= off) t += u; }
-    if (lane < SORT2_THREADS / 64) sc[lane] = t;
-  }
-  __syncthreads();
-  const u32 w = blockIdx.x, incl = v + (wave ? sc[wave - 1] : 0u), excl = incl - Sb;
-  if (tid < bins && excl <= w && w < incl) { res[0] = (u32)tid; res[1] = w - excl; res[2] = Sb; res[3] = start; res[4] = len; res[5] = excl; }
-  __syncthreads();
-  FineSlice r;
-  r.active = res[0] != 0xffffffffu;
-  r.bin = (int)res[0]; r.s = (int)res[1]; r.Sb = (int)res[2];
-  const u64 L = res[4];
-  r.start = res[3];
-  r.lo = res[3] + (u32)(L * (u64)r.s / (u64)r.Sb);
-  r.hi = res[3] + (u32)(L * (u64)(r.s + 1) / (u64)r.Sb);
-  return r;
+  const u32 first = plan_incl_scan(Sb, sc) - Sb;
+  u32 before = first, mine = Sb;
+  if (over_only) {
+    __syncthreads();
+    mine = fine_over_slices(Sb);
+    before = plan_incl_scan(mine, sc) - mine;
+  }
+  if (tid < bins && fine_slice_is_mine(blockIdx.x, before, mine)) {
+    res[0] = (u32)tid; res[1] = blockIdx.x - before; res[2] = Sb; res[3] = start; res[4] = len; res[5] = first;
+  }
+  __syncthreads();
+  if (res[0] == 0xffffffffu) { FineSlice none{}; none.active = false; return none; }
+  return fine_slice_make(res[0], res[1], res[2], res[3], res[4], res[5]);
 }
 constexpr int FINE_UNROLL = 8;
+template <class REC>
+__device__ __forceinline__ void fine_histogram(const typename REC::T* __restrict__ tmp, u32 lo, u32 hi, int F, int fb, u32* hist) {
+  for (int f = threadIdx.x; f < F; f += SORT2_THREADS) hist[f] = 0;
+  __syncthreads();
+  for (u32 base = lo + threadIdx.x; base < hi; base += FINE_UNROLL * SORT2_THREADS) {
+    u32 f[FINE_UNROLL];
+#pragma unroll
+    for (int k = 0; k < FINE_UNROLL; k++) {
+      const u32 e = base + k * SORT2_THREADS;
+      f[k] = (e < hi) ? REC::fine(tmp[e], (u32)F - 1u, fb) : 0xffffffffu;
+    }
+#pragma unroll
+    for (int k = 0; k < FINE_UNROLL; k++) if (f[k] != 0xffffffffu) counter_inc_agg(hist, f[k]);
+  }
+  __syncthreads();
+}
 template <class REC>
 __global__ __launch_bounds__(SORT2_THREADS) void k_fine_count(const typename REC::T* __restrict__ tmp, const u32* __restrict__ binbase, int nwg, int F,
                                                                int S, int fb, u32* __restrict__ finehist, int bins, u32 cap, u32* __restrict__ bucket_tot) {
@@ -599,20 +617,7 @@
     for (int f = threadIdx.x; f < F; f += SORT2_THREADS) finehist[(size_t)blockIdx.x * F + f] = 0;
     return;
   }
-  for (int f = threadIdx.x; f < F; f += SORT2_THREADS) hist[f] = 0;
-  __syncthreads();
-  const u32 lo = p.lo, hi = p.hi;
-  for (u32 base = lo + threadIdx.x; base < hi; base += FINE_UNROLL * SORT2_THREADS) {
-    u32 f[FINE_UNROLL];
-#pragma unroll
-    for (int k = 0; k < FINE_UNROLL; k++) {
-      const u32 e = base + k * SORT2_THREADS;
-      f[k] = (e < hi) ? REC::fine(tmp[e], (u32)F - 1u, fb) : 0xffffffffu;
-    }
-#pragma unroll
-    for (int k = 0; k < FINE_UNROLL; k++) if (f[k] != 0xffffffffu) counter_inc_agg(hist, f[k]);
-  }
-  __syncthreads();
+  fine_histogram<REC>(tmp, p.lo, p.hi, F, fb, hist);
   const size_t hbase = (size_t)F * (blockIdx.x - (u32)p.s);
   for (int f = threadIdx.x; f < F; f += SORT2_THREADS) {
     const u32 v = hist[f];
@@ -657,10 +662,55 @@
 constexpr int STAGE_CAP = MZK_STAGE_CAP;
 constexpr int STAGE_PER_LANE = STAGE_CAP / SORT2_THREADS;
 template <class REC>
+__device__ __forceinline__ void fine_rounds(const typename REC::T* __restrict__ tmp, u32 lo, u32 hi, int F, int fb, u32* gbase, u32* cnt, u32* lpre, u32* scan,
+                                            u32* spay, unsigned short* skey, u32* __restrict__ entries) {
+  const int tid = threadIdx.x;
+  const int per = (F + SORT2_THREADS - 1) / SORT2_THREADS;
+  for (u32 chunk = lo; chunk < hi; chunk += STAGE_CAP) {
+    const u32 cend = (hi - chunk > (u32)STAGE_CAP) ? chunk + STAGE_CAP : hi;
+    for (int f = tid; f < F; f += SORT2_THREADS) cnt[f] = 0;
+    __syncthreads();
+    typename REC::T r[STAGE_PER_LANE];
+    u32 rk[STAGE_PER_LANE];
+    const u32 fmask = (u32)F - 1u;
+#pragma unroll
+    for (int k = 0; k < STAGE_PER_LANE; k++) {
+      const u32 e = chunk + tid + k * SORT2_THREADS;
+      if (e < cend) r[k] = tmp[e];
+    }
+#pragma unroll
+    for (int k = 0; k < STAGE_PER_LANE; k++) rk[k] = (chunk + tid + k * SORT2_THREADS < cend) ? counter_inc_agg(cnt, REC::fine(r[k], fmask, fb)) : 0u;
+    __syncthreads();
+    u32 local = 0;
+    for (int q = 0; q < per; q++) { const int f = tid * per + q; if (f < F) local += cnt[f]; }
+    u32 run = block_excl_scan<SORT2_THREADS>(local, scan, nullptr);
+    for (int q = 0; q < per; q++) { const int f = tid * per + q; if (f < F) { lpre[f] = run; run += cnt[f]; } }
+    __syncthreads();
+#pragma unroll
+    for (int k = 0; k < STAGE_PER_LANE; k++) {
+      if (chunk + tid + k * SORT2_THREADS < cend) {
+        const u32 fk = REC::fine(r[k], fmask, fb);
+        const u32 pos = lpre[fk] + rk[k];
+        spay[pos] = REC::payload(r[k], fb);
+        skey[pos] = (unsigned short)fk;
+      }
+    }
+    __syncthreads();
+    const u32 m = cend - chunk;
+    for (u32 j = tid; j < m; j += SORT2_THREADS) {
+      const u32 f = skey[j];
+      entries[gbase[f] + (j - lpre[f])] = spay[j];
+    }
+    __syncthreads();
+    for (int f = tid; f < F; f += SORT2_THREADS) gbase[f] += cnt[f];
+    __syncthreads();
+  }
+}
+template <class REC>
 __global__ __launch_bounds__(SORT2_THREADS) void k_fine_scatter(const typename REC::T* __restrict__ tmp, const u32* __restrict__ binbase, int nwg, int F,
                                                                  int S, int fb, const u32* __restrict__ finebase, u32* __restrict__ offsets,
                                                                  u32* __restrict__ entries, size_t nbuckets, int bins, u32 cap, const u32* __restrict__ bucket_tot,
-                                                                 u32* __restrict__ bucket_cur) {
+                                                                 u32* __restrict__ bucket_cur, bool over_only) {
   extern __shared__ u32 lds_fs[];
   u32* gbase = lds_fs;
   u32* cnt = gbase + F;
@@ -669,11 +719,20 @@
   u32* spay = scan + SORT2_THREADS;
   unsigned short* skey = reinterpret_cast<unsigned short*>(spay + STAGE_CAP);
   const int tid = threadIdx.x;
-  const FineSlice p = fine_plan(binbase, nwg, bins, S, cap, scan, gbase);
-  __syncthreads();
-  if (blockIdx.x == 0 && tid == 0) offsets[nbuckets] = bucket_tot ? binbase[(size_t)bins * nwg] : finebase[(size_t)F * gridDim.x];
+  if (over_only) {
+    if (tid == 0) scan[0] = 0;
+    __syncthreads();
+    if (tid < bins && binbase[(size_t)(tid + 1) * nwg] - binbase[(size_t)tid * nwg] > cap) scan[0] = 1;
+    __syncthreads();
+    const bool any = scan[0] != 0;
+    __syncthreads();
+    if (!any) return;
+  }
+  const FineSlice p = fine_plan(binbase, nwg, bins, S, cap, scan, gbase, over_only);
+  __syncthreads();
+  if (!over_only && blockIdx.x == 0 && tid == 0) offsets[nbuckets] = bucket_tot ? binbase[(size_t)bins * nwg] : finebase[(size_t)F * gridDim.x];
   if (!p.active) return;
-  const size_t hbase = (size_t)F * (blockIdx.x - (u32)p.s);
+  const size_t hbase = (size_t)F * p.first;
   if (bucket_tot) {
     const int per2 = (F + SORT2_THREADS - 1) / SORT2_THREADS;
     u32 local = 0;
@@ -683,7 +742,7 @@
       const int f = tid * per2 + q;
       if (f < F) {
         const u32 v = cnt[f];
-        const u32 mine = finebase[hbase + (size_t)f * p.Sb + p.s];
+        const u32 mine = finebase[fine_hist_index(F, p.first, f, (u32)p.Sb, (u32)p.s)];
         gbase[f] = run + (mine ? atomicAdd(&bucket_cur[(size_t)p.bin * F + f], mine) : 0u);
         if (p.s == 0) offsets[(size_t)p.bin * F + f] = run;
         run += v;
@@ -697,47 +756,43 @@
       if (p.s == 0) offsets[(size_t)p.bin * F + f] = base;
     }
   }
-  const u32 lo = p.lo, hi = p.hi;
+  fine_rounds<REC>(tmp, p.lo, p.hi, F, fb, gbase, cnt, lpre, scan, spay, skey, entries);
+}
+template <class REC>
+__global__ __launch_bounds__(SORT2_THREADS) void k_fine_one(const typename REC::T* __restrict__ tmp, const u32* __restrict__ binbase, int nwg, int F, int fb,
+                                                             u32* __restrict__ finehist, u32* __restrict__ offsets, u32* __restrict__ entries, size_t nbuckets,
+                                                             int bins, u32 cap, u32* __restrict__ bucket_tot, u32* __restrict__ sort_ctr) {
+  extern __shared__ u32 lds_fs[];
+  u32* gbase = lds_fs;
+  u32* cnt = gbase + F;
+  u32* lpre = cnt + F;
+  u32* scan = lpre + F;
+  u32* spay = scan + SORT2_THREADS;
+  unsigned short* skey = reinterpret_cast<unsigned short*>(spay + STAGE_CAP);
+  const int tid = threadIdx.x;
+  const FineSlice p = fine_plan(binbase, nwg, bins, 1, cap, scan, gbase);
+  __syncthreads();
+  if (blockIdx.x == 0 && tid == 0) offsets[nbuckets] = binbase[(size_t)bins * nwg];
+  if (sort_ctr && blockIdx.x == gridDim.x - 1) for (int i = tid; i < 2 * SORT_CTR_BINS; i += SORT2_THREADS) sort_ctr[i] = 0;
+  if (!p.active) return;
+  fine_histogram<REC>(tmp, p.lo, p.hi, F, fb, cnt);
+  if (fine_role(true, (u32)p.Sb) == FINE_SLICE) {
+    for (int f = tid; f < F; f += SORT2_THREADS) {
+      const u32 v = cnt[f];
+      finehist[fine_hist_index(F, p.first, f, (u32)p.Sb, (u32)p.s)] = v;
+      if (v) atomicAdd(&bucket_tot[(size_t)p.bin * F + f], v);
+    }
+    return;
+  }
   const int per = (F + SORT2_THREADS - 1) / SORT2_THREADS;
-  for (u32 chunk = lo; chunk < hi; chunk += STAGE_CAP) {
-    const u32 cend = (hi - chunk > (u32)STAGE_CAP) ? chunk + STAGE_CAP : hi;
-    for (int f = tid; f < F; f += SORT2_THREADS) cnt[f] = 0;
-    __syncthreads();
-    typename REC::T r[STAGE_PER_LANE];
-    u32 rk[STAGE_PER_LANE];
-    const u32 fmask = (u32)F - 1u;
-#pragma unroll
-    for (int k = 0; k < STAGE_PER_LANE; k++) {
-      const u32 e = chunk + tid + k * SORT2_THREADS;
-      if (e < cend) r[k] = tmp[e];
-    }
-#pragma unroll
-    for (int k = 0; k < STAGE_PER_LANE; k++) rk[k] = (chunk + tid + k * SORT2_THREADS < cend) ? counter_inc_agg(cnt, REC::fine(r[k], fmask, fb)) : 0u;
-    __syncthreads();
-    u32 local = 0;
-    for (int q = 0; q < per; q++) { const int f = tid * per + q; if (f < F) local += cnt[f]; }
-    u32 run = block_excl_scan<SORT2_THREADS>(local, scan, nullptr);
-    for (int q = 0; q < per; q++) { const int f = tid * per + q; if (f < F) { lpre[f] = run; run += cnt[f]; } }
-    __syncthreads();
-#pragma unroll
-    for (int k = 0; k < STAGE_PER_LANE; k++) {
-      if (chunk + tid + k * SORT2_THREADS < cend) {
-        const u32 fk = REC::fine(r[k], fmask, fb);
-        const u32 pos = lpre[fk] + rk[k];
-        spay[pos] = REC::payload(r[k], fb);
-        skey[pos] = (unsigned short)fk;
-      }
-    }
-    __syncthreads();
-    const u32 m = cend - chunk;
-    for (u32 j = tid; j < m; j += SORT2_THREADS) {
-      const u32 f = skey[j];
-      entries[gbase[f] + (j - lpre[f])] = spay[j];
-    }
-    __syncthreads();
-    for (int f = tid; f < F; f += SORT2_THREADS) gbase[f] += cnt[f];
-    __syncthreads();
-  }
+  const auto cnt_at = [&](int f) { return cnt[f]; };
+  const u32 run0 = p.start + block_excl_scan<SORT2_THREADS>(fine_lane_total(tid, per, F, cnt_at), scan, nullptr);
+  fine_lane_offsets(tid, per, F, run0, cnt_at, [&](int f, u32 run, u32) {
+    gbase[f] = run;
+    offsets[(size_t)p.bin * F + f] = run;
+  });
+  __syncthreads();
+  fine_rounds<REC>(tmp, p.lo, p.hi, F, fb, gbase, cnt, lpre, scan, spay, skey, entries);
 }
 
 __global__ __launch_bounds__(256) void k_scan_local(const u32* __restrict__ in, u32* __restrict__ out, u32* __restrict__ block_sums, size_t n) {
@@ -890,17 +945,14 @@
     __syncthreads();
   }
 }
-__global__ __launch_bounds__(HEAVY_THREADS) void k_seg_combine_heavy(const u32* __restrict__ slots, const u32* __restrict__ offsets,
-                                                                      u32* __restrict__ buckets, u32* __restrict__ heavy, size_t max_heavy) {
-  __shared__ __attribute__((aligned(16))) u32 sh[HEAVY_QUADS * 32];
-  __shared__ u32 last_arrival;
-  const u32 count = heavy[0];
+__device__ __forceinline__ void seg_heavy_work(u32 blk, u32 nblk, u32 count, const u32* __restrict__ slots, const u32* __restrict__ offsets,
+                                               u32* __restrict__ buckets, u32* __restrict__ heavy, size_t max_heavy, u32* sh, u32* last_arrival) {
   if (count == 0) return;
   const u32 seg = heavy[1];
   const int lane = threadIdx.x & 3, quad = threadIdx.x >> 2;
   const u32* list = heavy + HEAVY_HDR;
-  if (2 * count > gridDim.x) {
-    for (u32 h = blockIdx.x; h < count; h += gridDim.x) {
+  if (2 * count > nblk) {
+    for (u32 h = blk; h < count; h += nblk) {
       const size_t b = list[2 * h];
       const u32 o0 = offsets[b], o1 = list[2 * h + 1];
       const size_t s0 = (size_t)(o0 / seg) + b, s1 = (size_t)((o1 - 1) / seg) + b;
@@ -912,8 +964,8 @@
     }
     return;
   }
-  const u32 G = gridDim.x / count;
-  const u32 h = blockIdx.x / G, part = blockIdx.x % G;
+  const u32 G = nblk / count;
+  const u32 h = blk / G, part = blk % G;
   if (h >= count) return;
   u32* scratch = heavy + heavy_list_words(max_heavy);
   const size_t b = list[2 * h];
@@ -937,16 +989,35 @@
   if (quad == 0) xyzz_gstore_quad(scratch, (size_t)h * G + part, xyzz_gload_quad(sh, 0, lane), lane);
   __threadfence();
   __syncthreads();
-  if (threadIdx.x == 0) last_arrival = (atomicAdd(&heavy[2 + h], 1u) == G - 1) ? 1u : 0u;
-  __syncthreads();
-  if (!last_arrival) return;
+  if (threadIdx.x == 0) *last_arrival = (atomicAdd(&heavy[2 + h], 1u) == G - 1) ? 1u : 0u;
+  __syncthreads();
+  if (!*last_arrival) return;
   __threadfence();
   acc = xyzz_inf();
   for (u32 q = quad; q < G; q += HEAVY_QUADS) acc = xyzz_add_quad(acc, xyzz_gload_quad(scratch, (size_t)h * G + q, lane), lane);
   heavy_tree(sh, acc, quad, lane);
   if (quad == 0) xyzz_gstore_quad(buckets, b, xyzz_gload_quad(sh, 0, lane), lane);
 }
-
+__device__ __forceinline__ void seg_heavy_wg(u32 blk, u32 nblk, const u32* __restrict__ slots, const u32* __restrict__ offsets, u32* __restrict__ buckets,
+                                             u32* __restrict__ heavy, size_t max_heavy) {
+  __shared__ __attribute__((aligned(16))) u32 sh[HEAVY_QUADS * 32];
+  __shared__ u32 last_arrival;
+  const u32 count = heavy[0];
+  seg_heavy_work(blk, nblk, count, slots, offsets, buckets, heavy, max_heavy, sh, &last_arrival);
+  __syncthreads();
+  if (threadIdx.x == 0) {
+    __threadfence();
+    last_arrival = (atomicAdd(&heavy[HEAVY_DONE_AT], 1u) == nblk - 1) ? 1u : 0u;
+  }
+  __syncthreads();
+  if (!last_arrival) return;
+  if (count) for (int i = threadIdx.x; i < HEAVY_GRID / 2; i += HEAVY_THREADS) heavy[2 + i] = 0;
+  if (threadIdx.x == 0) { heavy[0] = 0; heavy[HEAVY_DONE_AT] = 0; }
+}
+__global__ __launch_bounds__(HEAVY_THREADS) void k_seg_combine_heavy(const u32* __restrict__ slots, const u32* __restrict__ offsets,
+                                                                      u32* __restrict__ buckets, u32* __restrict__ heavy, size_t max_heavy) {
+  seg_heavy_wg(blockIdx.x, gridDim.x, slots, offsets, buckets, heavy, max_heavy);
+}
 __device__ __forceinline__ void halve_op(u32* __restrict__ buf, int lgB, int t, size_t id, int lane) {
   const int lgh = lgB - t - 1;
   const size_t a = id >> lgh, j = id & (((size_t)1 << lgh) - 1);
@@ -1281,18 +1352,31 @@
 #undef MZK_DIRECT
   const u32* bounds = a.bin_tot ? (const u32*)a.bin_start : (const u32*)a.binhist;
   const int bstride = a.bin_tot ? 1 : P.nwg;
+  const size_t fine_lds = ((size_t)3 * P.F + SORT2_THREADS + STAGE_CAP) * 4 + (size_t)STAGE_CAP * 2;
+  if (P.F <= STAGE_F_MAX) {
+    bool& staged_attr = ctx().attr_done[sizeof(R) == 4 ? ATTR_FINE_SCATTER4 : ATTR_FINE_SCATTER8];
+    if (!staged_attr) {
+      MZK_HIP(hipFuncSetAttribute((const void*)k_fine_scatter<REC>, hipFuncAttributeMaxDynamicSharedMemorySize, 160 * 1024));
+      MZK_HIP(hipFuncSetAttribute((const void*)k_fine_one<REC>, hipFuncAttributeMaxDynamicSharedMemorySize, 160 * 1024));
+      staged_attr = true;
+    }
+  }
+  if (P.fine_one) {
+    hipLaunchKernelGGL((k_fine_one<REC>), dim3(P.fine_wgs), dim3(SORT2_THREADS), fine_lds, s, (const R*)a.tmp, bounds, bstride, P.F, P.fb, a.finehist,
+                       a.offsets, a.entries, P.NBtot, (int)bins, P.slice_cap, a.bucket_tot, a.bin_tot);
+    hipLaunchKernelGGL((k_fine_scatter<REC>), dim3(P.fine_over_wgs), dim3(SORT2_THREADS), fine_lds, s, (const R*)a.tmp, bounds, bstride, P.F,
+                       P.S, P.fb, (const u32*)a.finehist, a.offsets, a.entries, P.NBtot, (int)bins, P.slice_cap, (const u32*)a.bucket_tot, a.bucket_cur,
+                       true);
+    MZK_HIP(hipGetLastError());
+    return MZK_OK;
+  }
   hipLaunchKernelGGL((k_fine_count<REC>), dim3(P.fine_wgs), dim3(SORT2_THREADS), 0, s, (const R*)a.tmp, bounds, bstride, P.F, P.S,
                      P.fb, a.finehist, (int)bins, P.slice_cap, a.bucket_tot);
   if (!P.fine_free) MZK_TRY(launch_exclusive_scan((const u32*)a.finehist, a.finehist, P.own.n_fine, a.scan3, s));
   if (P.F <= STAGE_F_MAX) {
-    const size_t lds = ((size_t)3 * P.F + SORT2_THREADS + STAGE_CAP) * 4 + (size_t)STAGE_CAP * 2;
-    bool& staged_attr = ctx().attr_done[sizeof(R) == 4 ? ATTR_FINE_SCATTER4 : ATTR_FINE_SCATTER8];
-    if (!staged_attr) {
-      MZK_HIP(hipFuncSetAttribute((const void*)k_fine_scatter<REC>, hipFuncAttributeMaxDynamicSharedMemorySize, 160 * 1024));
-      staged_attr = true;
-    }
-    hipLaunchKernelGGL((k_fine_scatter<REC>), dim3(P.fine_wgs), dim3(SORT2_THREADS), lds, s, (const R*)a.tmp, bounds, bstride, P.F,
-                       P.S, P.fb, (const u32*)a.finehist, a.offsets, a.entries, P.NBtot, (int)bins, P.slice_cap, (const u32*)a.bucket_tot, a.bucket_cur);
+    hipLaunchKernelGGL((k_fine_scatter<REC>), dim3(P.fine_wgs), dim3(SORT2_THREADS), fine_lds, s, (const R*)a.tmp, bounds, bstride, P.F,
+                       P.S, P.fb, (const u32*)a.finehist, a.offsets, a.entries, P.NBtot, (int)bins, P.slice_cap, (const u32*)a.bucket_tot, a.bucket_cur,
+                       false);
   } else {
     hipLaunchKernelGGL((k_fine_scatter_direct<REC>), dim3(P.fine_wgs), dim3(SORT2_THREADS), 0, s, (const R*)a.tmp, bounds, bstride,
                        P.F, P.S, P.fb, (const u32*)a.finehist, a.offsets, a.entries, P.NBtot, (int)bins, P.slice_cap);
@@ -1320,8 +1404,12 @@
       {WS_MSM_CURSOR, P.ws.cursor, &ranks, 0}, {WS_MSM_ENTRIES, P.ws.entries, &entries, P.alloc.E}, {WS_MSM_SCAN, P.ws.scan, &scan, 0},
       {WS_MSM_BUCKETS, P.ws.buckets, &buckets, P.NB * 32}, {WS_MSM_SLOTS, P.ws.slots, &slots, P.slot_region_words},
       {WS_MSM_WGHIST, P.ws.wghist, &wghist, 0}, {WS_MSM_OUT, P.ws.out, &wsum, 0}};
+  const u32* hdr_was_clean = ctx().msm_hdr_clean;
+  const u32* hdr_now_clean = nullptr;
+  ctx().msm_hdr_clean = nullptr;
   for (const auto& r : req)
     if (r.bytes) { MZK_TRY(ws_get(r.slot, r.bytes, (void**)r.p)); *r.p += (cc ? cc->k : 0) * r.words; }
+  if (ctx().msm_hdr_gen != ctx().ws_alloc_gen) hdr_was_clean = nullptr;
   const u32* pts = (pm ? pm : (const u32*)d_points) + i0 * 16;
   bool prepared = false;
   auto prepare = [&]() -> int {
@@ -1355,7 +1443,7 @@
   } else {
     u32* heavy = slots + P.nslots * SLOT_WORDS;
     prof_begin(s, MZK_PH_MSM_SORT);
-    MZK_HIP(hipMemsetAsync(heavy, 0, (size_t)HEAVY_HDR * 4, s));
+    if (!hdr_was_clean || hdr_was_clean != heavy) MZK_HIP(hipMemsetAsync(heavy, 0, (size_t)HEAVY_HDR * 4, s));
     if (P.path == MsmPath::TwoLevel) {
       u32* finehist = wghist + P.alloc.n_coarse + 1;
       const SortBufs sb{(const u32*)d_scalars, wghist, ranks, finehist, scan + scan_scratch_words(P.alloc.n_coarse) + 2, offsets, entries,
@@ -1408,9 +1496,11 @@
     MZK_HIP(hipGetLastError());
     prof_end(s, MZK_PH_MSM_SEG_COMBINE);
     if (cc) return MZK_OK;
+    if (P.path == MsmPath::TwoLevel && P.fine_one) hdr_now_clean = heavy;
   }
   MZK_TRY(reduce_bucket_sets(buckets, P.lgB, P.red_windows, P.one_set, P.horner_c, wsum, (u32*)d_out, out_partial_xyzz, s));
   MZK_HIP(hipGetLastError());
+  ctx().msm_hdr_clean = hdr_now_clean, ctx().msm_hdr_gen = ctx().ws_alloc_gen;
   return MZK_OK;
 }
 
@@ -1601,6 +1691,7 @@
     MZK_TRY(ws_get(WS_MSM_SCAN, scan_scratch_words(ncnt) * 4, (void**)&scan_tmp));
     MZK_TRY(ws_get(WS_MSM_BUCKETS, NBtot * 128, (void**)&buckets));
     MZK_TRY(ws_get(WS_MSM_SLOTS, nslots * SLOT_WORDS * 4 + heavy_words * 4, (void**)&slots));
+    ctx().msm_hdr_clean = nullptr;
     compact = offs;
     u32* tails = nullptr;
     if (nch > 1) MZK_TRY(ws_get(WS_MSM_OFFSETS, (NBtot + 1) * 4, (void**)&compact));
@@ -1790,6 +1881,7 @@
     if (parts > (size_t)DIRECT_FINISH_PARTS) for (groups = 2; groups * groups < parts; groups++) {}
     u32 *slots, *scratch;
     MZK_TRY(ws_get(WS_MSM_SLOTS, cnt * (parts + groups) * DIRECT_THREADS * SLOT_WORDS * 4, (void**)&slots));
+    ctx().msm_hdr_clean = nullptr;
     MZK_TRY(ws_get(WS_MSM_BUCKETS, cnt * 128, (void**)&scratch));
     const u32* sc = (const u32*)d_scalars + first * stride_elems * 8;
     const unsigned nwg = (unsigned)(cnt * parts);
diff --git a/myzkp_amd/csrc/mzk_msm_plan.h b/myzkp_amd/csrc/mzk_msm_plan.h
--- a/myzkp_amd/csrc/mzk_msm_plan.h
+++ b/myzkp_amd/csrc/mzk_msm_plan.h
@@ -53,6 +53,7 @@
 constexpr int COARSE_PER_WG = 4096;
 constexpr int FINE_MAX = 8192;
 constexpr int STAGE_F_MAX = 2048;
+constexpr size_t FINE_ONE_MAX = 49152;
 constexpr size_t SMALL_MAX_N = 4097;
 constexpr size_t SMALL_MAX_BUCKETS = 8192;
 constexpr int SCAN_ITEMS = 8;
@@ -64,6 +65,7 @@
 }
 constexpr uint32_t HEAVY_SLOTS = 32;
 constexpr int HEAVY_GRID = 512;
+constexpr int HEAVY_DONE_AT = 2 + HEAVY_GRID - 1;
 constexpr int SORT_CTR_BINS = 1024;
 constexpr int SORT_CTR_AT = 2 + HEAVY_GRID;
 constexpr int HEAVY_HDR = SORT_CTR_AT + 2 * SORT_CTR_BINS;
@@ -80,6 +82,7 @@
   int per_fine = 0;
   int sort_scan_free = 3;
   int combine_wide_min_log = 17;
+  int fine_one = 1;
 };
 
 enum class MsmPath { SmallScan, SmallSort, TwoLevel, LdsOnePass, Atomic };
@@ -97,9 +100,10 @@
   MsmPath path = MsmPath::SmallSort;
   int cl = 0, F = 0, fb = 0, key_shift = 0, S = 0, nwg = 0;
   uint32_t fine_mask = 0, slice_cap = 0;
-  unsigned fine_wgs = 0;
+  unsigned fine_wgs = 0, fine_over_wgs = 0;
   size_t per_wg = 0;
   bool compact = false, coarse_free = false, fine_free = false, scatter_staged = false;
+  bool fine_one = false;
   int coarse_c = 0;
   uint32_t seg = 0, t_max = 0;
   size_t T = 0, nslots = 0, max_heavy = 0, slot_region_words = 0;
@@ -201,22 +205,25 @@
   P.fine_mask = (uint32_t)P.F - 1u;
   while ((1 << P.fb) < P.F) P.fb++;
   P.nwg = (int)((n + COARSE_PER_WG - 1) / COARSE_PER_WG);
+  P.compact = ref_max <= ((size_t)1 << (31 - P.fb));
+  P.coarse_free = (kn.sort_scan_free & 1) != 0 && cbins <= (size_t)SORT_CTR_BINS;
+  P.fine_free = (kn.sort_scan_free & 2) != 0 && P.F <= STAGE_F_MAX;
+  P.coarse_c = (plain_merged && (L.c == 16 || L.c == 17 || L.c == 20)) ? L.c : 0;
+  P.scatter_staged = P.coarse_c != 0;
+  const size_t bin_nom = (E_max + cbins - 1) / cbins;
+  P.fine_one = kn.fine_one != 0 && P.coarse_free && P.fine_free && P.scatter_staged && bin_nom <= FINE_ONE_MAX;
   const size_t per_fine = kn.per_fine > 0 ? (size_t)kn.per_fine : (P.F >= 4096 ? 131072 : P.F >= 2048 ? 65536 : (L.glv ? 16384 : 32768));
   const size_t S = (E_max / cbins + per_fine - 1) / per_fine;
-  P.S = S < 2 ? 2 : S > 64 ? 64 : (int)S;
+  P.S = P.fine_one ? 1 : S < 2 ? 2 : S > 64 ? 64 : (int)S;
   const size_t slice_nom = (E_max + cbins * (size_t)P.S - 1) / (cbins * (size_t)P.S);
   P.slice_cap = (uint32_t)(slice_nom + slice_nom / 2 + 1);
   P.fine_wgs = (unsigned)(cbins * (size_t)P.S + (E_max + P.slice_cap - 1) / P.slice_cap + 1);
+  P.fine_over_wgs = P.fine_one ? (unsigned)(2 * (E_max / P.slice_cap) + 1) : 0u;
   P.own.n_coarse = cbins * P.nwg;
   P.own.n_fine = (size_t)P.F * P.fine_wgs;
   const size_t slice_nom_a = (E_alloc + cbins * (size_t)64 - 1) / (cbins * (size_t)64);
   P.alloc.n_coarse = chunks ? cbins * ((n_alloc + COARSE_PER_WG - 1) / COARSE_PER_WG) : P.own.n_coarse;
   P.alloc.n_fine = chunks ? (size_t)P.F * (cbins * 64 + (E_alloc + slice_nom_a) / (slice_nom_a + slice_nom_a / 2 + 1) + 2) : P.own.n_fine;
-  P.compact = ref_max <= ((size_t)1 << (31 - P.fb));
-  P.coarse_free = (kn.sort_scan_free & 1) != 0 && cbins <= (size_t)SORT_CTR_BINS;
-  P.fine_free = (kn.sort_scan_free & 2) != 0 && P.F <= STAGE_F_MAX;
-  P.coarse_c = (plain_merged && (L.c == 16 || L.c == 17 || L.c == 20)) ? L.c : 0;
-  P.scatter_staged = P.coarse_c != 0;
   return msm_sized(P, regions);
 }
 
@@ -285,6 +292,60 @@
   flush(b);
 }
 
+enum FineRole { FINE_IDLE = 0,
+                FINE_OWNER = 1,
+                FINE_SLICE = 2 };
+MZK_HD uint32_t fine_bin_slices(uint32_t len, uint32_t cap, uint32_t min_slices) {
+  const uint32_t s = len / cap + (len % cap != 0 ? 1u : 0u);
+  return s < min_slices ? min_slices : s;
+}
+MZK_HD uint32_t fine_over_slices(uint32_t slices) { return slices > 1 ? slices : 0u; }
+MZK_HD void fine_slice_span(uint32_t start, uint32_t len, uint32_t s, uint32_t slices, uint32_t* lo, uint32_t* hi) {
+  *lo = start + (uint32_t)((uint64_t)len * s / slices);
+  *hi = start + (uint32_t)((uint64_t)len * (s + 1) / slices);
+}
+MZK_HD int fine_role(bool one_pass, uint32_t slices) { return (one_pass && slices == 1) ? FINE_OWNER : FINE_SLICE; }
+struct FineSlice {
+  int bin, s, Sb;
+  uint32_t lo, hi, start;
+  uint32_t first;
+  bool active;
+};
+MZK_HD bool fine_slice_is_mine(uint32_t w, uint32_t before, uint32_t mine) { return before <= w && w - before < mine; }
+MZK_HD FineSlice fine_slice_make(uint32_t bin, uint32_t s, uint32_t slices, uint32_t start, uint32_t len, uint32_t first) {
+  FineSlice r;
+  r.active = true, r.bin = (int)bin, r.s = (int)s, r.Sb = (int)slices, r.start = start, r.first = first;
+  fine_slice_span(start, len, s, slices, &r.lo, &r.hi);
+  return r;
+}
+template <class BinStart>
+MZK_HD FineSlice fine_plan_at(uint32_t w, int bins, BinStart bin_start_at, uint32_t cap, uint32_t min_slices, bool over_only) {
+  uint32_t first = 0, before = 0;
+  for (int b = 0; b < bins; b++) {
+    const uint32_t start = bin_start_at(b), len = bin_start_at(b + 1) - start;
+    const uint32_t slices = fine_bin_slices(len, cap, min_slices), mine = over_only ? fine_over_slices(slices) : slices;
+    if (fine_slice_is_mine(w, before, mine)) return fine_slice_make((uint32_t)b, w - before, slices, start, len, first);
+    first += slices, before += mine;
+  }
+  FineSlice none{};
+  none.active = false;
+  return none;
+}
+template <class Cnt>
+MZK_HD uint32_t fine_lane_total(int tid, int per, int F, Cnt cnt_at) {
+  uint32_t t = 0;
+  for (int q = 0; q < per; q++) { const int f = tid * per + q; if (f < F) t += cnt_at(f); }
+  return t;
+}
+template <class Cnt, class Emit>
+MZK_HD void fine_lane_offsets(int tid, int per, int F, uint32_t run, Cnt cnt_at, Emit emit) {
+  for (int q = 0; q < per; q++) {
+    const int f = tid * per + q;
+    if (f < F) { const uint32_t v = cnt_at(f); emit(f, run, v); run += v; }
+  }
+}
+MZK_HD size_t fine_hist_index(int F, uint32_t first, int f, uint32_t slices, uint32_t s) { return (size_t)F * first + (size_t)f * slices + s; }
+
 static inline bool msm_chunkable(size_t n_total, int point_kind, size_t table_stride, const MsmKnobs& kn) {
   if (n_total < ((size_t)1 << 18)) return false;
   const MsmPlan P = msm_plan(n_total, n_total, n_total, point_kind, table_stride, 256, 1, kn);
```

Measured after the change: 762.7 million pairs/s (median of 4 runs). Within noise of the previous version (-0.5%).
